# Sunefei/PathNet

Measured on AMD Instinct MI355X. Metric: paths aggregated/sec (PAGG fwd+bwd, one training step incl. on-GPU MERW sampling + Adam), higher is better.
Workload: dtype f32; 1 GPU; Cora-shaped synthetic (configs[1]): N=2708 F=1433 C=7 hid=128 path_num=40 path_len=4, 1299 masked nodes = 51960 paths/step, PathNet_homo, dropout 0.7, Adam; nodes=2708, parallelism=node-shard x1

## Files before the change

include/pathnet_hip.h:

```cpp
#ifndef PATHNET_HIP_H_
#define PATHNET_HIP_H_

#include <stdint.h>

#ifdef __cplusplus
extern "C" {
#endif

#define PN_ABI_VERSION 12

#define PN_OK 0
#define PN_ERR_ARG (-1)
#define PN_ERR_IO (-2)
#define PN_ERR_FORMAT (-3)
#define PN_ERR_HIP (-4)
#define PN_ERR_EMPTY_TABLE (-5)
#define PN_ERR_NOMEM (-6)
#define PN_ERR_CAPACITY (-7)

int pn_abi_version(void);
const char *pn_last_error(void);

typedef struct pn_device_info {
    char name[128];
    char arch[64];
    int32_t compute_units;
    int32_t lds_bytes_per_block;
    int64_t hbm_bytes;
    int32_t clock_khz;
} pn_device_info;
int pn_device_query(pn_device_info *out);

typedef struct pn_context pn_context;
int pn_context_create(pn_context **out);
int pn_context_destroy(pn_context *ctx);
int pn_context_set_knob(pn_context *ctx, const char *name, int32_t value);
int pn_context_get_knob(const pn_context *ctx, const char *name, int32_t *value);

typedef struct pn_step_state {
    int64_t epoch;
    uint64_t seed;
    int64_t adam_step;
    int64_t reserved;
} pn_step_state;
int pn_step_state_advance(pn_step_state *dev_state, void *stream);

int pn_clock_probe(double *mhz, void *stream);


int pn_edges_read_text(const char *path, int32_t *n, int64_t *m, int32_t *u, int32_t *v, double *p, int64_t cap);

int pn_pairs_read_text(const char *path, int32_t *n, int64_t *m, int32_t *u, int32_t *v, int64_t cap);

int pn_uniform_build(int32_t n, int64_t m, const int32_t *u, const int32_t *v, int64_t *off, int32_t *packed,
                     int32_t *src, int32_t *nbr, int64_t cap, int64_t *total);

int pn_alias_build(int32_t n, int64_t m, const int32_t *u, const int32_t *v, const double *p, int64_t *off,
                   int32_t *A, int32_t *B, double *S, uint32_t *thr, int64_t cap, int64_t *total);

int pn_hops_dense(int32_t n, int64_t m, const int32_t *u, const int32_t *v, int32_t seq_len, uint8_t *dis);

int pn_csr_build(int32_t n, int64_t m, const int32_t *u, const int32_t *v, int32_t reverse, int64_t *off,
                 int32_t *adj, int64_t cap, int64_t *count);

int pn_glibc_draws(uint32_t seed, uint64_t first, int64_t count, int32_t *out);


#define PN_DRAW_GLIBC_REPLAY 0
#define PN_DRAW_PHILOX 1

typedef struct pn_sampler_tables {
    int32_t n;
    int64_t total;
    const int64_t *off;
    const int32_t *triples;
    const uint8_t *dis;
    const int64_t *adj_off;
    const int32_t *adj;
    const int64_t *radj_off;
    const int32_t *radj;
    int32_t draws_per_step;
    const uint32_t *node_ref;
} pn_sampler_tables;

int pn_node_ref_pack(int32_t n, const int64_t *off, uint32_t *ref);

int pn_alias_pack(int64_t total, const int32_t *A, const int32_t *B, const uint32_t *thr, int32_t *dst);

int pn_tables_workspace_bytes(int32_t n, int64_t m, int64_t *bytes);

int pn_alias_build_device(int32_t n, int64_t m, const int32_t *u, const int32_t *v, const double *p, int64_t *off,
                          int32_t *triples, uint32_t *node_ref, double *S, int64_t cap, int64_t *total, void *workspace,
                          int64_t workspace_bytes, void *stream);

int pn_csr_build_device(int32_t n, int64_t m, const int32_t *u, const int32_t *v, int32_t reverse, int64_t *off,
                        int32_t *adj, int64_t cap, int64_t *count, void *workspace, int64_t workspace_bytes, void *stream);

int pn_hops_dense_device(int32_t n, const int64_t *off, const int32_t *adj, int32_t seq_len, uint8_t *dis, void *stream);

int pn_sample_workspace_bytes(int32_t W, int32_t L, int32_t draw_source, int64_t epoch_count, int32_t node_count,
                              int64_t *bytes);

int pn_sample_paths(pn_context *ctx, const pn_sampler_tables *tables, int32_t W, int32_t L, int32_t draw_source, uint64_t seed,
                    int64_t epoch_begin, int64_t epoch_count, int32_t node_begin, int32_t node_count, int32_t *ids,
                    uint8_t *codes, void *workspace, int64_t workspace_bytes, int32_t *status_flag,
                    const pn_step_state *step_state ,
                    const int32_t *node_list , void *stream);

typedef struct pn_path_report {
    int64_t out_of_range;
    int64_t non_edges;
    int64_t far;
    int64_t first_bad;
} pn_path_report;

int pn_path_codes_workspace_bytes(const pn_sampler_tables *tables, int32_t W, int32_t L, int32_t rows, int64_t *bytes);
int pn_path_codes(pn_context *ctx, const pn_sampler_tables *tables, int32_t W, int32_t L, int32_t rows,
                  const int32_t *ids , const int32_t *sources ,
                  uint8_t *codes , pn_path_report *report ,
                  void *workspace, int64_t workspace_bytes, void *stream);

#define PN_BIAS_MAX_TRIALS 64
int pn_bias_thresholds(double p, double q, uint64_t thr[3]);
int pn_sample_paths_biased_workspace_bytes(const pn_sampler_tables *tables, int32_t W, int32_t L, int64_t epoch_count,
                                           int32_t node_count, int64_t *bytes);
int pn_sample_paths_biased(pn_context *ctx, const pn_sampler_tables *tables, int32_t W, int32_t L, uint64_t seed,
                           int64_t epoch_begin, int64_t epoch_count, int32_t node_begin, int32_t node_count, double p,
                           double q, int32_t *ids, uint8_t *codes, int64_t *exhausted , void *workspace,
                           int64_t workspace_bytes, int32_t *status_flag, const pn_step_state *step_state,
                           const int32_t *node_list, void *stream);

int pn_census_lists_workspace_bytes(int32_t n, int64_t m, int64_t *bytes);
int pn_census_lists(pn_context *ctx, int32_t n, int64_t m, const int32_t *u, const int32_t *v, int64_t *off, int32_t *adj,
                    void *workspace, int64_t workspace_bytes, void *stream);

int pn_pattern_census_workspace_bytes(int32_t n, int32_t num_symbols, int32_t walk_len, int64_t *bytes);
int pn_pattern_census(pn_context *ctx, int32_t n, const int64_t *off, const int32_t *adj,
                      const uint8_t *symbols , int32_t num_symbols, int32_t walk_len,
                      int64_t *counts , int64_t *labels , void *workspace,
                      int64_t workspace_bytes, void *stream);

typedef struct pn_walk_stats_out {
    int64_t *step_code;
    int64_t *label_pairs;
    int64_t *unlabeled;
    int64_t *stay;
    int64_t *back;
    int64_t *distinct_hist;
    int32_t *unique_paths;
    int32_t *cover;
    int64_t *visits;
    int64_t *counters;
} pn_walk_stats_out;

int pn_walk_stats_workspace_bytes(int32_t n, int32_t W, int32_t L, int64_t rows, int32_t C, int64_t *bytes);
int pn_walk_stats(pn_context *ctx, int32_t n, int32_t W, int32_t L, int64_t rows,
                  const int32_t *ids , const uint8_t *codes ,
                  const int32_t *sources , const int32_t *labels , int32_t C,
                  int32_t accumulate, const pn_walk_stats_out *out, void *workspace, int64_t workspace_bytes,
                  void *stream);

typedef struct pn_path_prob_out {
    int64_t *num;
    int64_t *mass;
    uint8_t *cls;
    int64_t *counters;
} pn_path_prob_out;

int pn_path_prob_workspace_bytes(const pn_sampler_tables *tables, int32_t W, int32_t L, int64_t rows, int32_t second_order,
                                 int64_t *bytes);
int pn_path_prob(pn_context *ctx, const pn_sampler_tables *tables, int32_t W, int32_t L, int64_t rows,
                 const int32_t *ids , int32_t second_order, const pn_path_prob_out *out,
                 void *workspace, int64_t workspace_bytes, void *stream);

int pn_paths_write_text(const char *path, const int32_t *ids, const uint8_t *codes, int64_t npaths, int32_t L,
                        int32_t append);
int pn_paths_read_text(const char *path, int32_t L, int32_t *ids, uint8_t *codes, int64_t cap, int64_t *npaths);

int pn_paths_write_bin(const char *path, const int32_t *ids, const uint8_t *codes, int64_t npaths, int32_t L);
int pn_paths_read_bin(const char *path, int32_t *L_out, int32_t *ids, uint8_t *codes, int64_t cap, int64_t *npaths);

#define PN_VARIANT_HETERO 0
#define PN_VARIANT_HOMO 1
#define PN_VARIANT_PAGG 2

typedef struct pn_pagg_shape {
    int32_t variant;
    int32_t N, F, H, C;
    int32_t S, W, L;
    int32_t S_total, group_begin;
    int32_t batch_groups;
    int32_t cell;
    int32_t deterministic;
    int32_t compact;
    int32_t seq_math;
} pn_pagg_shape;
#define PN_SEQ_MATH_DEFAULT 0
#define PN_SEQ_MATH_BF16X3 1
#define PN_SEQ_MATH_F16X2 2
#define PN_COMPACT_AUTO 0
#define PN_COMPACT_ON 1
#define PN_COMPACT_OFF 2
#define PN_CELL_DEFAULT 0
#define PN_CELL_LSTM 1
#define PN_CELL_RNN 2
#define PN_CELL_GRU 3
#define PN_CELL_MEAN 4
#define PN_CELL_SUM 5

typedef struct pn_pagg_args {
    pn_pagg_shape shape;
    const float *X;
    const int32_t *ids;
    const uint8_t *codes;
    const int32_t *sel;
    const float *fc0_w, *fc0_b;
    const float *bank_w, *bank_b;
    const float *w_ih, *w_hh;
    const float *b_ih, *b_hh;
    const float *att_w, *att_b;
    const float *fc2_w, *fc2_b;
    float p_seq, p_cls;
    uint64_t seed;
    const float *mask_seq;
    const float *mask_cls;
    float *out;
    void *workspace;
    int64_t workspace_bytes;
    const float *g_out;
    float *g_X;
    float *g_fc0_w, *g_fc0_b, *g_bank_w, *g_bank_b, *g_w_ih, *g_w_hh, *g_b_ih, *g_b_hh, *g_att_w, *g_att_b,
        *g_fc2_w, *g_fc2_b;
    const float *Xh_in;
    float *g_Xh;
    void *Xh_ready;
    void *g_Xh_ready;
    int32_t no_save;
    int32_t reuse_tables;
    int32_t index_rows_local;
    const pn_step_state *step_state;
    float *out_embed;
    float *out_path_weight;
    float *out_path_state;
    const float *g_embed;
} pn_pagg_args;

int pn_pagg_workspace_bytes(const pn_pagg_shape *shape, int64_t *bytes);
int pn_pagg_shape_info(const pn_pagg_shape *shape, int64_t out[4]);
typedef struct pn_seq_range {
    uint32_t x_bits;
    int32_t x_esum;
    uint32_t x_cnt;
    uint32_t w_ih_bits, w_hh_bits, dg_bits;
} pn_seq_range;
int pn_pagg_range_offset(const pn_pagg_shape *shape, int64_t *offset);
int pn_pagg_paths_stream(pn_context *ctx, const pn_pagg_shape *shape, void *stream, void **out);
int pn_pagg_forward(pn_context *ctx, const pn_pagg_args *args, void *stream);
int pn_pagg_backward(pn_context *ctx, const pn_pagg_args *args, void *stream);
int pn_pagg_train_step(pn_context *ctx, const pn_pagg_args *args, const int64_t *target, float grad_scale, float *loss,
                       void *stream);

int pn_pagg_gather(pn_context *ctx, const pn_pagg_shape *shape, const float *table , const int32_t *ids,
                   const uint8_t *codes, float *rows , void *stream);

int pn_gemm_f32(const float *A, int64_t sAm, int64_t sAk, const float *B, int64_t sBn, int64_t sBk, float *C,
                int64_t ldc, const float *bias, int32_t M, int32_t N, int32_t K, int32_t relu, void *stream);

#define PN_LINEAR_SPLIT_MAX 8
int pn_linear_forward(pn_context *ctx, const float *X, const float *W, const float *b, int32_t rows, int32_t in_f, int32_t out_f,
                      int32_t relu, float *Y, void *workspace, int64_t workspace_bytes, void *stream);

#define PN_LINEAR_BWD_SPLIT_MAX 32
int pn_linear_backward(pn_context *ctx, const float *dY, const float *gate, const float *X, const float *W, int32_t rows, int32_t in_f,
                       int32_t out_f, float *g_W, float *g_b, float *g_X, void *workspace, int64_t workspace_bytes, void *stream);

int pn_merw_workspace_bytes(int32_t n, int64_t *bytes);
int pn_merw_probabilities(int32_t n, int64_t nnz, const int64_t *row_off, const int32_t *col, const double *val,
                          double *p, double *psi, double *lambda, int32_t max_iter, double tol, int32_t *iters,
                          void *workspace, int64_t workspace_bytes, void *stream);

int pn_cross_entropy(const float *logits, const int64_t *target, int32_t rows, int32_t classes, float *loss,
                     float *g_logits, void *stream);

#define PN_ADAM_MAX_TENSORS 32
typedef struct pn_adam_tensor {
    float *param;
    const float *grad;
    float *exp_avg;
    float *exp_avg_sq;
    int64_t count;
} pn_adam_tensor;
int pn_adam_step(const pn_adam_tensor *tensors, int32_t n_tensors, float lr, float beta1, float beta2, float eps,
                 float weight_decay, int64_t step, const pn_step_state *step_state ,
                 void *stream);
int pn_adam_step_advance(const pn_adam_tensor *tensors, int32_t n_tensors, float lr, float beta1, float beta2, float eps,
                         float weight_decay, pn_step_state *step_state , void *stream);

int pn_pagg_debug_offsets(const pn_pagg_shape *shape, int64_t out[4]);

int pn_profile_configure(pn_context *ctx, int32_t mode, int32_t stage);
int pn_profile_stage_count(void);
const char *pn_profile_stage_name(int32_t stage);
int pn_profile_read(pn_context *ctx, double *ms_sum, int64_t *count);

#ifdef __cplusplus
}
#endif
#endif
```

pathnet_amd/_lib.py:

```python
import ctypes
import os

HERE = os.path.dirname(os.path.abspath(__file__))
LIB_PATH = os.environ.get("PN_LIB_PATH", os.path.join(HERE, "csrc", "libpathnet_hip.so"))

PN_OK = 0
PN_ERR_ARG, PN_ERR_IO, PN_ERR_FORMAT, PN_ERR_HIP, PN_ERR_EMPTY_TABLE, PN_ERR_NOMEM, PN_ERR_CAPACITY = (
    -1, -2, -3, -4, -5, -6, -7)
DRAW_GLIBC_REPLAY, DRAW_PHILOX = 0, 1
ABI_VERSION = 12
VARIANT_HETERO, VARIANT_HOMO, VARIANT_PAGG = 0, 1, 2
CELL_DEFAULT, CELL_LSTM, CELL_RNN, CELL_GRU, CELL_MEAN, CELL_SUM = 0, 1, 2, 3, 4, 5
SEQ_MATH_DEFAULT, SEQ_MATH_BF16X3, SEQ_MATH_F16X2 = 0, 1, 2
COMPACT_AUTO, COMPACT_ON, COMPACT_OFF = 0, 1, 2
LINEAR_SPLIT_MAX = 8
LINEAR_BWD_SPLIT_MAX = 32

c_i32p = ctypes.POINTER(ctypes.c_int32)
c_i64p = ctypes.POINTER(ctypes.c_int64)
c_u32p = ctypes.POINTER(ctypes.c_uint32)
c_u8p = ctypes.POINTER(ctypes.c_uint8)
c_f64p = ctypes.POINTER(ctypes.c_double)
vp = ctypes.c_void_p


class PnError(RuntimeError):
    def __init__(self, code, msg):
        super().__init__("libpathnet_hip error %d: %s" % (code, msg))
        self.code = code


class DeviceInfo(ctypes.Structure):
    _fields_ = [("name", ctypes.c_char * 128), ("arch", ctypes.c_char * 64), ("compute_units", ctypes.c_int32),
                ("lds_bytes_per_block", ctypes.c_int32), ("hbm_bytes", ctypes.c_int64), ("clock_khz", ctypes.c_int32)]


class SamplerTables(ctypes.Structure):
    _fields_ = [("n", ctypes.c_int32), ("total", ctypes.c_int64), ("off", vp), ("triples", vp), ("dis", vp),
                ("adj_off", vp), ("adj", vp), ("radj_off", vp), ("radj", vp), ("draws_per_step", ctypes.c_int32),
                ("node_ref", vp)]


class PaggShape(ctypes.Structure):
    _fields_ = [("variant", ctypes.c_int32), ("N", ctypes.c_int32), ("F", ctypes.c_int32), ("H", ctypes.c_int32),
                ("C", ctypes.c_int32), ("S", ctypes.c_int32), ("W", ctypes.c_int32), ("L", ctypes.c_int32),
                ("S_total", ctypes.c_int32), ("group_begin", ctypes.c_int32), ("batch_groups", ctypes.c_int32),
                ("cell", ctypes.c_int32), ("deterministic", ctypes.c_int32), ("compact", ctypes.c_int32),
                ("seq_math", ctypes.c_int32)]


class PaggArgs(ctypes.Structure):
    _fields_ = ([("shape", PaggShape), ("X", vp), ("ids", vp), ("codes", vp), ("sel", vp)] +
                [(k, vp) for k in ("fc0_w", "fc0_b", "bank_w", "bank_b", "w_ih", "w_hh", "b_ih", "b_hh", "att_w",
                                   "att_b", "fc2_w", "fc2_b")] +
                [("p_seq", ctypes.c_float), ("p_cls", ctypes.c_float), ("seed", ctypes.c_uint64), ("mask_seq", vp),
                 ("mask_cls", vp), ("out", vp), ("workspace", vp), ("workspace_bytes", ctypes.c_int64),
                 ("g_out", vp), ("g_X", vp)] +
                [("g_" + k, vp) for k in ("fc0_w", "fc0_b", "bank_w", "bank_b", "w_ih", "w_hh", "b_ih", "b_hh", "att_w",
                                          "att_b", "fc2_w", "fc2_b")] +
                [("Xh_in", vp), ("g_Xh", vp), ("Xh_ready", vp), ("g_Xh_ready", vp), ("no_save", ctypes.c_int32),
                 ("reuse_tables", ctypes.c_int32),
                 ("index_rows_local", ctypes.c_int32), ("step_state", vp),
                 ("out_embed", vp), ("out_path_weight", vp), ("out_path_state", vp), ("g_embed", vp)])


class WalkStatsOut(ctypes.Structure):
    FIELDS = ("step_code", "label_pairs", "unlabeled", "stay", "back", "distinct_hist", "unique_paths", "cover", "visits",
              "counters")
    _fields_ = [(k, vp) for k in FIELDS]


class PathProbOut(ctypes.Structure):
    FIELDS = ("num", "mass", "cls", "counters")
    _fields_ = [(k, vp) for k in FIELDS]


class AdamTensor(ctypes.Structure):
    _fields_ = [("param", ctypes.c_void_p), ("grad", ctypes.c_void_p), ("exp_avg", ctypes.c_void_p),
                ("exp_avg_sq", ctypes.c_void_p), ("count", ctypes.c_int64)]


SIGNATURES = {
    "pn_abi_version": (ctypes.c_int, []),
    "pn_last_error": (ctypes.c_char_p, []),
    "pn_device_query": (ctypes.c_int, [ctypes.POINTER(DeviceInfo)]),
    "pn_context_create": (ctypes.c_int, [ctypes.POINTER(vp)]),
    "pn_context_destroy": (ctypes.c_int, [vp]),
    "pn_context_set_knob": (ctypes.c_int, [vp, ctypes.c_char_p, ctypes.c_int32]),
    "pn_context_get_knob": (ctypes.c_int, [vp, ctypes.c_char_p, c_i32p]),
    "pn_clock_probe": (ctypes.c_int, [c_f64p, vp]),
    "pn_step_state_advance": (ctypes.c_int, [vp, vp]),
    "pn_edges_read_text": (ctypes.c_int, [ctypes.c_char_p, c_i32p, c_i64p, c_i32p, c_i32p, c_f64p, ctypes.c_int64]),
    "pn_pairs_read_text": (ctypes.c_int, [ctypes.c_char_p, c_i32p, c_i64p, c_i32p, c_i32p, ctypes.c_int64]),
    "pn_uniform_build": (ctypes.c_int, [ctypes.c_int32, ctypes.c_int64, c_i32p, c_i32p, c_i64p, c_i32p, c_i32p, c_i32p,
                                        ctypes.c_int64, c_i64p]),
    "pn_alias_build": (ctypes.c_int, [ctypes.c_int32, ctypes.c_int64, c_i32p, c_i32p, c_f64p, c_i64p, c_i32p, c_i32p,
                                      c_f64p, c_u32p, ctypes.c_int64, c_i64p]),
    "pn_alias_pack": (ctypes.c_int, [ctypes.c_int64, c_i32p, c_i32p, c_u32p, c_i32p]),
    "pn_node_ref_pack": (ctypes.c_int, [ctypes.c_int32, c_i64p, c_u32p]),
    "pn_hops_dense": (ctypes.c_int, [ctypes.c_int32, ctypes.c_int64, c_i32p, c_i32p, ctypes.c_int32, c_u8p]),
    "pn_csr_build": (ctypes.c_int, [ctypes.c_int32, ctypes.c_int64, c_i32p, c_i32p, ctypes.c_int32, c_i64p, c_i32p,
                                    ctypes.c_int64, c_i64p]),
    "pn_glibc_draws": (ctypes.c_int, [ctypes.c_uint32, ctypes.c_uint64, ctypes.c_int64, c_i32p]),
    "pn_tables_workspace_bytes": (ctypes.c_int, [ctypes.c_int32, ctypes.c_int64, c_i64p]),
    "pn_alias_build_device": (ctypes.c_int, [ctypes.c_int32, ctypes.c_int64, vp, vp, vp, vp, vp, vp, vp, ctypes.c_int64,
                                             c_i64p, vp, ctypes.c_int64, vp]),
    "pn_csr_build_device": (ctypes.c_int, [ctypes.c_int32, ctypes.c_int64, vp, vp, ctypes.c_int32, vp, vp,
                                           ctypes.c_int64, c_i64p, vp, ctypes.c_int64, vp]),
    "pn_hops_dense_device": (ctypes.c_int, [ctypes.c_int32, vp, vp, ctypes.c_int32, vp, vp]),
    "pn_sample_workspace_bytes": (ctypes.c_int, [ctypes.c_int32, ctypes.c_int32, ctypes.c_int32, ctypes.c_int64,
                                                 ctypes.c_int32, c_i64p]),
    "pn_sample_paths": (ctypes.c_int, [vp, ctypes.POINTER(SamplerTables), ctypes.c_int32, ctypes.c_int32, ctypes.c_int32,
                                       ctypes.c_uint64, ctypes.c_int64, ctypes.c_int64, ctypes.c_int32, ctypes.c_int32,
                                       vp, vp, vp, ctypes.c_int64, vp, vp, vp, vp]),
    "pn_path_codes_workspace_bytes": (ctypes.c_int, [ctypes.POINTER(SamplerTables), ctypes.c_int32, ctypes.c_int32,
                                                     ctypes.c_int32, c_i64p]),
    "pn_path_codes": (ctypes.c_int, [vp, ctypes.POINTER(SamplerTables), ctypes.c_int32, ctypes.c_int32, ctypes.c_int32, vp, vp,
                                     vp, vp, vp, ctypes.c_int64, vp]),
    "pn_bias_thresholds": (ctypes.c_int, [ctypes.c_double, ctypes.c_double, ctypes.POINTER(ctypes.c_uint64)]),
    "pn_sample_paths_biased_workspace_bytes": (ctypes.c_int, [ctypes.POINTER(SamplerTables), ctypes.c_int32, ctypes.c_int32,
                                                              ctypes.c_int64, ctypes.c_int32, c_i64p]),
    "pn_sample_paths_biased": (ctypes.c_int, [vp, ctypes.POINTER(SamplerTables), ctypes.c_int32, ctypes.c_int32,
                                              ctypes.c_uint64, ctypes.c_int64, ctypes.c_int64, ctypes.c_int32,
                                              ctypes.c_int32, ctypes.c_double, ctypes.c_double, vp, vp, vp, vp,
                                              ctypes.c_int64, vp, vp, vp, vp]),
    "pn_census_lists_workspace_bytes": (ctypes.c_int, [ctypes.c_int32, ctypes.c_int64, c_i64p]),
    "pn_census_lists": (ctypes.c_int, [vp, ctypes.c_int32, ctypes.c_int64, vp, vp, vp, vp, vp, ctypes.c_int64, vp]),
    "pn_pattern_census_workspace_bytes": (ctypes.c_int, [ctypes.c_int32, ctypes.c_int32, ctypes.c_int32, c_i64p]),
    "pn_pattern_census": (ctypes.c_int, [vp, ctypes.c_int32, vp, vp, vp, ctypes.c_int32, ctypes.c_int32, vp, vp, vp,
                                         ctypes.c_int64, vp]),
    "pn_walk_stats_workspace_bytes": (ctypes.c_int, [ctypes.c_int32, ctypes.c_int32, ctypes.c_int32, ctypes.c_int64,
                                                     ctypes.c_int32, c_i64p]),
    "pn_walk_stats": (ctypes.c_int, [vp, ctypes.c_int32, ctypes.c_int32, ctypes.c_int32, ctypes.c_int64, vp, vp, vp, vp,
                                     ctypes.c_int32, ctypes.c_int32, ctypes.POINTER(WalkStatsOut), vp, ctypes.c_int64, vp]),
    "pn_path_prob_workspace_bytes": (ctypes.c_int, [ctypes.POINTER(SamplerTables), ctypes.c_int32, ctypes.c_int32,
                                                    ctypes.c_int64, ctypes.c_int32, c_i64p]),
    "pn_path_prob": (ctypes.c_int, [vp, ctypes.POINTER(SamplerTables), ctypes.c_int32, ctypes.c_int32, ctypes.c_int64, vp,
                                    ctypes.c_int32, ctypes.POINTER(PathProbOut), vp, ctypes.c_int64, vp]),
    "pn_paths_write_text": (ctypes.c_int, [ctypes.c_char_p, c_i32p, c_u8p, ctypes.c_int64, ctypes.c_int32,
                                           ctypes.c_int32]),
    "pn_paths_read_text": (ctypes.c_int, [ctypes.c_char_p, ctypes.c_int32, c_i32p, c_u8p, ctypes.c_int64, c_i64p]),
    "pn_paths_write_bin": (ctypes.c_int, [ctypes.c_char_p, c_i32p, c_u8p, ctypes.c_int64, ctypes.c_int32]),
    "pn_paths_read_bin": (ctypes.c_int, [ctypes.c_char_p, c_i32p, c_i32p, c_u8p, ctypes.c_int64, c_i64p]),
    "pn_pagg_workspace_bytes": (ctypes.c_int, [ctypes.POINTER(PaggShape), c_i64p]),
    "pn_pagg_shape_info": (ctypes.c_int, [ctypes.POINTER(PaggShape), c_i64p]),
    "pn_pagg_forward": (ctypes.c_int, [vp, ctypes.POINTER(PaggArgs), vp]),
    "pn_pagg_backward": (ctypes.c_int, [vp, ctypes.POINTER(PaggArgs), vp]),
    "pn_pagg_gather": (ctypes.c_int, [vp, ctypes.POINTER(PaggShape), vp, vp, vp, vp, vp]),
    "pn_gemm_f32": (ctypes.c_int, [vp, ctypes.c_int64, ctypes.c_int64, vp, ctypes.c_int64, ctypes.c_int64, vp,
                                   ctypes.c_int64, vp, ctypes.c_int32, ctypes.c_int32, ctypes.c_int32, ctypes.c_int32,
                                   vp]),
    "pn_profile_configure": (ctypes.c_int, [vp, ctypes.c_int32, ctypes.c_int32]),
    "pn_profile_stage_count": (ctypes.c_int, []),
    "pn_profile_stage_name": (ctypes.c_char_p, [ctypes.c_int32]),
    "pn_profile_read": (ctypes.c_int, [vp, c_f64p, c_i64p]),
    "pn_linear_forward": (ctypes.c_int, [vp, vp, vp, vp, ctypes.c_int32, ctypes.c_int32, ctypes.c_int32, ctypes.c_int32, vp,
                                         vp, ctypes.c_int64, vp]),
    "pn_linear_backward": (ctypes.c_int, [vp, vp, vp, vp, vp, ctypes.c_int32, ctypes.c_int32, ctypes.c_int32, vp, vp,
                                          vp, vp, ctypes.c_int64, vp]),
    "pn_pagg_train_step": (ctypes.c_int, [vp, ctypes.POINTER(PaggArgs), vp, ctypes.c_float, vp, vp]),
    "pn_pagg_debug_offsets": (ctypes.c_int, [ctypes.POINTER(PaggShape), c_i64p]),
    "pn_pagg_range_offset": (ctypes.c_int, [ctypes.POINTER(PaggShape), c_i64p]),
    "pn_pagg_paths_stream": (ctypes.c_int, [vp, ctypes.POINTER(PaggShape), vp, ctypes.POINTER(ctypes.c_void_p)]),
    "pn_merw_workspace_bytes": (ctypes.c_int, [ctypes.c_int32, c_i64p]),
    "pn_merw_probabilities": (ctypes.c_int, [ctypes.c_int32, ctypes.c_int64, vp, vp, vp, vp, vp, c_f64p, ctypes.c_int32,
                                             ctypes.c_double, c_i32p, vp, ctypes.c_int64, vp]),
    "pn_cross_entropy": (ctypes.c_int, [vp, vp, ctypes.c_int32, ctypes.c_int32, vp, vp, vp]),
    "pn_adam_step": (ctypes.c_int, [ctypes.POINTER(AdamTensor), ctypes.c_int32, ctypes.c_float, ctypes.c_float,
                                    ctypes.c_float, ctypes.c_float, ctypes.c_float, ctypes.c_int64, vp, vp]),
    "pn_adam_step_advance": (ctypes.c_int, [ctypes.POINTER(AdamTensor), ctypes.c_int32, ctypes.c_float, ctypes.c_float,
                                            ctypes.c_float, ctypes.c_float, ctypes.c_float, vp, vp]),
}

_lib = None


def load():
    global _lib
    if _lib is None:
        if not os.path.exists(LIB_PATH):
            raise ImportError("pathnet_amd: %s is missing -- build the HIP extension first "
                              "(python -c 'import __graft_entry__ as g; g.build()'); there is no CPU fallback"
                              % LIB_PATH)
        lib = ctypes.CDLL(LIB_PATH)
        for name, (res, args) in SIGNATURES.items():
            fn = getattr(lib, name)
            fn.restype = res
            fn.argtypes = args
        if lib.pn_abi_version() != ABI_VERSION:
            raise ImportError("libpathnet_hip.so ABI version mismatch")
        _lib = lib
    return _lib


_contexts = {}


def context(device):
    import torch
    dev = torch.device(device)
    idx = dev.index if dev.index is not None else torch.cuda.current_device()
    ctx = _contexts.get(idx)
    if ctx is None:
        lib = load()
        h = vp()
        with torch.cuda.device(idx):
            check(lib.pn_context_create(ctypes.byref(h)))
        ctx = _contexts[idx] = vp(h.value)
        if len(_contexts) == 1:
            import atexit
            atexit.register(_destroy_contexts)
    return ctx


def set_knob(name, value, device="cuda"):
    old = get_knob(name, device)
    check(load().pn_context_set_knob(context(device), name.encode(), int(value)))
    return old


def get_knob(name, device="cuda"):
    v = ctypes.c_int32()
    check(load().pn_context_get_knob(context(device), name.encode(), ctypes.byref(v)))
    return v.value


def _destroy_contexts():
    if _lib is None:
        return
    for h in _contexts.values():
        try:
            _lib.pn_context_destroy(h)
        except Exception:
            pass
    _contexts.clear()


def stream_ptr(device):
    import torch
    return vp(torch.cuda.current_stream(device).cuda_stream)


def check(rc):
    if rc != PN_OK:
        raise PnError(rc, load().pn_last_error().decode(errors="replace"))


def ptr(t):
    if t is None:
        return None
    if hasattr(t, "data_ptr"):
        return ctypes.c_void_p(t.data_ptr())
    return ctypes.c_void_p(t.ctypes.data)


def np_ptr(a, ctype):
    return a.ctypes.data_as(ctypes.POINTER(ctype))
```

pathnet_amd/csrc/pn_context.hip:

```cpp
#include <hip/hip_runtime.h>

#include <cstdlib>
#include <cstring>
#include <map>
#include <new>
#include <tuple>
#include <vector>

#include "pn_internal.h"

struct pn_context {
    int device = 0;
    hipStream_t side = nullptr;
    hipEvent_t fork = nullptr, join = nullptr;
    int prof_mode = 0, prof_stage = -1;
    struct Rec {
        int stage;
        hipEvent_t a, b;
    };
    std::vector<Rec> recs;
    std::vector<hipEvent_t> free_events;
    std::map<const void *, int> lds_attr;
    std::map<std::tuple<const void *, size_t, int>, int> slots;
    int cus = 0;
    pn::Knobs knobs;
};

namespace {

__global__ void warm_kernel() {}

__global__ void step_state_advance_kernel(pn_step_state *s) {
    if (threadIdx.x != 0 || blockIdx.x != 0) return;
    s->epoch += 1;
    s->adam_step += 1;
    uint64_t z = (s->seed += 0x9E3779B97F4A7C15ull);
    z = (z ^ (z >> 30)) * 0xBF58476D1CE4E5B9ull;
    z = (z ^ (z >> 27)) * 0x94D049BB133111EBull;
    s->seed = z ^ (z >> 31);
}

__global__ void clock_probe_kernel(long long spin_ticks, long long *out) {
    const long long w0 = wall_clock64();
    const long long c0 = (long long)__builtin_readcyclecounter();
    long long w1 = w0;
    while (w1 - w0 < spin_ticks) {
        __builtin_amdgcn_s_sleep(8);
        w1 = wall_clock64();
    }
    const long long c1 = (long long)__builtin_readcyclecounter();
    out[0] = c1 - c0;
    out[1] = w1 - w0;
}

hipEvent_t take_event(pn_context *ctx) {
    if (!ctx->free_events.empty()) {
        hipEvent_t e = ctx->free_events.back();
        ctx->free_events.pop_back();
        return e;
    }
    hipEvent_t e = nullptr;
    (void)hipEventCreateWithFlags(&e, ctx->knobs.event_dev ? hipEventDisableSystemFence : hipEventDefault);
    return e;
}

}

namespace {

struct KnobName {
    const char *name;
    int pn::Knobs::*field;
};
const KnobName kKnobs[] = {{"PN_NODE_GEMM3", &pn::Knobs::node_gemm3}, {"PN_EVAL_ZW", &pn::Knobs::eval_zw},
                           {"PN_POOL_STEP", &pn::Knobs::pool_step}, {"PN_EVENT_DEVICE_SCOPE", &pn::Knobs::event_dev},
                           {"PN_NODE_RGRAD", &pn::Knobs::node_rgrad}, {"PN_SAMPLER_STAGE", &pn::Knobs::sampler_stage},
                           {"PN_SEQ4", &pn::Knobs::seq4}, {"PN_SEQH_TAIL", &pn::Knobs::seqh_tail}};

}

namespace pn {

const Knobs &knobs_of(const pn_context *ctx) {
    static const Knobs defaults;
    return ctx ? ctx->knobs : defaults;
}

bool profiling_every_stage(const pn_context *ctx) { return ctx && ctx->prof_mode == 1; }

int resident_slots(pn_context *ctx, const void *kernel, int threads, size_t lds_bytes, int *slots, int *cus) {
    if (ctx) {
        auto it = ctx->slots.find(std::make_tuple(kernel, lds_bytes, threads));
        if (it != ctx->slots.end() && ctx->cus > 0) {
            *slots = it->second * ctx->cus;
            *cus = ctx->cus;
            return PN_OK;
        }
    }
    int dev = 0, n_cu = 0, per_cu = 0;
    PN_CHECK_HIP(hipGetDevice(&dev));
    PN_CHECK_HIP(hipDeviceGetAttribute(&n_cu, hipDeviceAttributeMultiprocessorCount, dev));
    PN_CHECK_HIP(hipOccupancyMaxActiveBlocksPerMultiprocessor(&per_cu, kernel, threads, lds_bytes));
    if (ctx) {
        ctx->slots[std::make_tuple(kernel, lds_bytes, threads)] = per_cu;
        ctx->cus = n_cu;
    }
    *slots = per_cu * n_cu;
    *cus = n_cu;
    return PN_OK;
}

int context_check_device(const pn_context *ctx) {
    if (!ctx) return PN_OK;
    int dev = -1;
    PN_CHECK_HIP(hipGetDevice(&dev));
    if (dev != ctx->device)
        PN_FAIL(PN_ERR_ARG, "pn_context belongs to device %d, the current device is %d", ctx->device, dev);
    return PN_OK;
}

int ensure_dynamic_lds(pn_context *ctx, const void *kernel, int bytes) {
    if (ctx) {
        auto it = ctx->lds_attr.find(kernel);
        if (it != ctx->lds_attr.end() && it->second >= bytes) return PN_OK;
    }
    PN_CHECK_HIP(hipFuncSetAttribute(kernel, hipFuncAttributeMaxDynamicSharedMemorySize, bytes));
    if (ctx) ctx->lds_attr[kernel] = bytes;
    return PN_OK;
}

void *context_side_stream(pn_context *ctx) { return ctx ? (void *)ctx->side : nullptr; }
void *context_fork(pn_context *ctx, void *stream) {
    if (!ctx || !ctx->side) return nullptr;
    if (hipEventRecord(ctx->fork, (hipStream_t)stream) != hipSuccess) return nullptr;
    if (hipStreamWaitEvent(ctx->side, ctx->fork, 0) != hipSuccess) return nullptr;
    return ctx->side;
}
int context_record_join(pn_context *ctx) {
    PN_CHECK_HIP(hipEventRecord(ctx->join, ctx->side));
    return PN_OK;
}
int context_join(pn_context *ctx, void *stream) {
    PN_CHECK_HIP(hipStreamWaitEvent((hipStream_t)stream, ctx->join, 0));
    return PN_OK;
}
int context_wait_side(pn_context *ctx, void *stream) {
    if (!ctx || !ctx->side || (hipStream_t)stream == ctx->side) return PN_OK;
    hipStreamCaptureStatus cs = hipStreamCaptureStatusNone, ss = hipStreamCaptureStatusNone;
    PN_CHECK_HIP(hipStreamIsCapturing((hipStream_t)stream, &cs));
    PN_CHECK_HIP(hipStreamIsCapturing(ctx->side, &ss));
    if ((cs == hipStreamCaptureStatusActive) != (ss == hipStreamCaptureStatusActive)) return PN_OK;
    if (int rc = context_record_join(ctx)) return rc;
    return context_join(ctx, stream);
}

StageTimer::StageTimer(pn_context *ctx_, int stage, void *stream_) : ctx(ctx_), slot(-1), stream(stream_) {
    if (!ctx || ctx->prof_mode == 0 || (ctx->prof_mode == 2 && stage != ctx->prof_stage)) return;
    pn_context::Rec r{stage, take_event(ctx), take_event(ctx)};
    (void)hipEventRecord(r.a, (hipStream_t)stream);
    slot = (int)ctx->recs.size();
    ctx->recs.push_back(r);
}
StageTimer::~StageTimer() {
    if (slot >= 0) (void)hipEventRecord(ctx->recs[(size_t)slot].b, (hipStream_t)stream);
}

}

extern "C" {

int pn_context_create(pn_context **out) try {
    if (!out) PN_FAIL(PN_ERR_ARG, "pn_context_create: null");
    *out = nullptr;
    pn_context *c = new (std::nothrow) pn_context();
    if (!c) PN_FAIL(PN_ERR_NOMEM, "pn_context_create: out of memory");
    auto fail = [&](hipError_t e, const char *what) {
        pn::set_error("%s failed: %s", what, hipGetErrorString(e));
        (void)pn_context_destroy(c);
        return PN_ERR_HIP;
    };
    for (const KnobName &k : kKnobs)
        if (const char *v = std::getenv(k.name)) c->knobs.*(k.field) = std::atoi(v);
    hipError_t e = hipGetDevice(&c->device);
    if (e != hipSuccess) return fail(e, "hipGetDevice");
    if ((e = hipStreamCreateWithFlags(&c->side, hipStreamNonBlocking)) != hipSuccess) return fail(e, "hipStreamCreate");
    const unsigned ev_flags = hipEventDisableTiming | (c->knobs.event_dev ? hipEventDisableSystemFence : 0u);
    if ((e = hipEventCreateWithFlags(&c->fork, ev_flags)) != hipSuccess) return fail(e, "hipEventCreate");
    if ((e = hipEventCreateWithFlags(&c->join, ev_flags)) != hipSuccess) return fail(e, "hipEventCreate");
    hipLaunchKernelGGL(warm_kernel, dim3(1), dim3(64), 0, c->side);
    if ((e = hipGetLastError()) != hipSuccess) return fail(e, "first launch on the context's stream");
    *out = c;
    return PN_OK;
} catch (...) {
    PN_FAIL(PN_ERR_NOMEM, "pn_context_create: exception");
}

int pn_context_destroy(pn_context *c) {
    if (!c) return PN_OK;
    int rc = PN_OK;
    if (c->side) {
        if (hipStreamSynchronize(c->side) != hipSuccess) rc = PN_ERR_HIP;
        (void)hipStreamDestroy(c->side);
    }
    if (c->fork) (void)hipEventDestroy(c->fork);
    if (c->join) (void)hipEventDestroy(c->join);
    for (auto &r : c->recs) {
        (void)hipEventDestroy(r.a);
        (void)hipEventDestroy(r.b);
    }
    for (hipEvent_t e : c->free_events) (void)hipEventDestroy(e);
    delete c;
    if (rc != PN_OK) pn::set_error("pn_context_destroy: the context's stream reported an error");
    return rc;
}

int pn_context_set_knob(pn_context *ctx, const char *name, int32_t value) {
    if (!ctx || !name) PN_FAIL(PN_ERR_ARG, "pn_context_set_knob: null");
    for (const KnobName &k : kKnobs)
        if (std::strcmp(k.name, name) == 0) {
            const bool events_change = k.field == &pn::Knobs::event_dev && (ctx->knobs.event_dev != 0) != (value != 0);
            ctx->knobs.*(k.field) = value;
            if (events_change) {
                PN_CHECK_HIP(hipDeviceSynchronize());
                const unsigned ev_flags = hipEventDisableTiming | (value ? hipEventDisableSystemFence : 0u);
                hipEvent_t fork = nullptr, join = nullptr;
                PN_CHECK_HIP(hipEventCreateWithFlags(&fork, ev_flags));
                PN_CHECK_HIP(hipEventCreateWithFlags(&join, ev_flags));
                (void)hipEventDestroy(ctx->fork);
                (void)hipEventDestroy(ctx->join);
                ctx->fork = fork;
                ctx->join = join;
                for (hipEvent_t e : ctx->free_events) (void)hipEventDestroy(e);
                ctx->free_events.clear();
            }
            return PN_OK;
        }
    PN_FAIL(PN_ERR_ARG, "pn_context_set_knob: no knob named %s", name);
}
int pn_context_get_knob(const pn_context *ctx, const char *name, int32_t *value) {
    if (!name || !value) PN_FAIL(PN_ERR_ARG, "pn_context_get_knob: null");
    for (const KnobName &k : kKnobs)
        if (std::strcmp(k.name, name) == 0) {
            *value = pn::knobs_of(ctx).*(k.field);
            return PN_OK;
        }
    PN_FAIL(PN_ERR_ARG, "pn_context_get_knob: no knob named %s", name);
}

int pn_profile_configure(pn_context *ctx, int32_t mode, int32_t stage) {
    if (!ctx) PN_FAIL(PN_ERR_ARG, "pn_profile_configure: null context");
    if (mode < 0 || mode > 2) PN_FAIL(PN_ERR_ARG, "profile mode %d", mode);
    ctx->prof_mode = mode;
    ctx->prof_stage = stage;
    return PN_OK;
}
int pn_profile_stage_count(void) { return pn::ST_COUNT; }
const char *pn_profile_stage_name(int32_t stage) {
    static const char *const names[pn::ST_COUNT] = {"sampler_glibc_fill", "sampler_walk", "gather",    "fc0",      "bank",
                                                    "plan_pack",          "seq_fwd",      "pool_fwd",  "fc2_grad", "pool_bwd",
                                                    "seq_bwd",            "wgrad",        "bias_grad", "bank_bwd", "fc0_bwd", "zero_fill"};
    return (stage >= 0 && stage < pn::ST_COUNT) ? names[stage] : "?";
}
int pn_profile_read(pn_context *ctx, double *ms_sum, int64_t *count) try {
    if (!ctx || !ms_sum || !count) PN_FAIL(PN_ERR_ARG, "pn_profile_read: null");
    for (auto &r : ctx->recs) {
        PN_CHECK_HIP(hipEventSynchronize(r.b));
        float ms = 0.0f;
        PN_CHECK_HIP(hipEventElapsedTime(&ms, r.a, r.b));
        ms_sum[r.stage] += ms;
        count[r.stage] += 1;
        ctx->free_events.push_back(r.a);
        ctx->free_events.push_back(r.b);
    }
    ctx->recs.clear();
    return PN_OK;
} catch (...) {
    PN_FAIL(PN_ERR_NOMEM, "pn_profile_read: exception");
}

int pn_device_query(pn_device_info *out) {
    if (!out) PN_FAIL(PN_ERR_ARG, "pn_device_query: null");
    int dev = 0;
    PN_CHECK_HIP(hipGetDevice(&dev));
    hipDeviceProp_t prop;
    PN_CHECK_HIP(hipGetDeviceProperties(&prop, dev));
    std::snprintf(out->name, sizeof out->name, "%s", prop.name);
    std::snprintf(out->arch, sizeof out->arch, "%s", prop.gcnArchName);
    out->compute_units = prop.multiProcessorCount;
    out->lds_bytes_per_block = (int32_t)prop.sharedMemPerBlock;
    out->hbm_bytes = (int64_t)prop.totalGlobalMem;
    out->clock_khz = prop.clockRate;
    return PN_OK;
}

int pn_step_state_advance(pn_step_state *dev_state, void *stream_) {
    if (!dev_state) PN_FAIL(PN_ERR_ARG, "pn_step_state_advance: null");
    hipLaunchKernelGGL(step_state_advance_kernel, dim3(1), dim3(64), 0, (hipStream_t)stream_, dev_state);
    PN_CHECK_HIP(hipGetLastError());
    return PN_OK;
}

int pn_clock_probe(double *mhz, void *stream_) {
    if (!mhz) PN_FAIL(PN_ERR_ARG, "pn_clock_probe: null");
    hipStream_t stream = (hipStream_t)stream_;
    long long *buf = nullptr;
    PN_CHECK_HIP(hipHostMalloc(reinterpret_cast<void **>(&buf), 2 * sizeof(long long), hipHostMallocDefault));
    buf[0] = buf[1] = 0;
    hipLaunchKernelGGL(clock_probe_kernel, dim3(1), dim3(64), 0, stream, 200000LL , buf);
    hipError_t e = hipGetLastError();
    if (e == hipSuccess) e = hipStreamSynchronize(stream);
    const long long cyc = buf[0], ticks = buf[1];
    (void)hipHostFree(buf);
    if (e != hipSuccess) PN_FAIL(PN_ERR_HIP, "clock probe failed: %s", hipGetErrorString(e));
    if (ticks <= 0) PN_FAIL(PN_ERR_HIP, "clock probe: the wall clock did not advance");
    *mhz = (double)cyc / (double)ticks * 100.0;
    return PN_OK;
}

}
```

pathnet_amd/csrc/pn_internal.h:

```cpp
#pragma once
#include <cstdarg>
#include <cstdint>
#include <cstdio>

#include "../../include/pathnet_hip.h"

namespace pn {

void set_error(const char *fmt, ...) __attribute__((format(printf, 1, 2)));

#define PN_FAIL(code, ...)          \
    do {                            \
        ::pn::set_error(__VA_ARGS__); \
        return (code);              \
    } while (0)

#define PN_CHECK_HIP(expr)                                                                      \
    do {                                                                                        \
        hipError_t e_ = (expr);                                                                 \
        if (e_ != hipSuccess) PN_FAIL(PN_ERR_HIP, "%s failed: %s", #expr, hipGetErrorString(e_)); \
    } while (0)

struct GlibcPoly {
    uint32_t c[31];
};
struct GlibcState {
    uint32_t s[31];
};
GlibcPoly glibc_poly_one();
GlibcPoly glibc_poly_mul(const GlibcPoly &a, const GlibcPoly &b);
GlibcPoly glibc_poly_xpow(uint64_t d);
GlibcState glibc_apply(const GlibcPoly &p, const GlibcState &st);
GlibcState glibc_seed_state(uint32_t seed);

#ifndef PN_SEQH_TAIL_DEFAULT
#define PN_SEQH_TAIL_DEFAULT 0
#endif
struct Knobs {
    int node_gemm3 = 7;
    int eval_zw = 1;
    int event_dev = 1;
    int pool_step = 1;
    int node_rgrad = 1;
    int sampler_stage = -1;
    int seq4 = 4;
    int seqh_tail = PN_SEQH_TAIL_DEFAULT;
};
const Knobs &knobs_of(const pn_context *ctx);

enum Stage {
    ST_SAMPLER_FILL = 0, ST_SAMPLER_WALK, ST_GATHER, ST_FC0, ST_BANK, ST_PLAN_PACK, ST_SEQ_FWD, ST_POOL_FWD,
    ST_FC2_GRAD, ST_POOL_BWD, ST_SEQ_BWD, ST_WGRAD, ST_BIAS_GRAD, ST_BANK_BWD, ST_FC0_BWD, ST_ZERO_FILL, ST_COUNT
};
bool profiling_every_stage(const pn_context *ctx);
int context_check_device(const pn_context *ctx);
void *context_fork(pn_context *ctx, void *stream);
void *context_side_stream(pn_context *ctx);
int context_record_join(pn_context *ctx);
int context_join(pn_context *ctx, void *stream);
int context_wait_side(pn_context *ctx, void *stream);
int ensure_dynamic_lds(pn_context *ctx, const void *kernel, int bytes);
int resident_slots(pn_context *ctx, const void *kernel, int threads, size_t lds_bytes, int *slots, int *cus);
struct StageTimer {
    StageTimer(pn_context *ctx, int stage, void *stream);
    ~StageTimer();
    pn_context *ctx;
    int slot;
    void *stream;
};

struct ZeroList {
    float *ptr[12];
    unsigned long long count[12];
    int n;
};
struct ZeroFill {
    pn_context *ctx;
    ZeroList zl{};
    int add(float *ptr, size_t count) {
        if (!ptr || !count) return PN_OK;
        if (zl.n >= (int)(sizeof zl.ptr / sizeof zl.ptr[0])) PN_FAIL(PN_ERR_ARG, "internal: zero list overflow");
        zl.ptr[zl.n] = ptr;
        zl.count[zl.n] = count;
        zl.n++;
        return PN_OK;
    }
    int flush(void *stream, bool timed = true);
};

int launch_cross_entropy(const float *logits, const int64_t *target, int rows, int classes, float scale, float *loss,
                         float *g_logits, void *stream, bool overwrite = false);

size_t sort_temp_reserve(int64_t n);
int sort_pairs_i32(void *tmp, size_t tmp_bytes, const int32_t *keys_in, int32_t *keys_out, const int32_t *vals_in,
                   int32_t *vals_out, int64_t n, int key_bits, void *stream);

}
```

pathnet_amd/csrc/pn_pagg.hip:

```cpp
#include <hip/hip_runtime.h>

#include <algorithm>
#include <cstdlib>
#include <cstring>
#include <type_traits>

#include "pn_gemm.h"
#include "pn_internal.h"
#include "pn_kernels.h"
#include "pn_seq.h"

using namespace pn;

namespace {

struct PlanDims {
    int S_total, W, L, N;
    int64_t P_total;
    int64_t row_base;
};
__device__ __forceinline__ void plan_entry(int variant, const int32_t *ids, const uint8_t *codes, const PlanDims &d,
                                           int64_t slot, int t, int64_t &q, int &node, int &code) {
    if (variant == PN_VARIANT_HETERO) {
        const int64_t g = slot / d.W, mem = slot - g * d.W;
        q = mem * d.S_total + g;
        const int64_t r = q * d.L + t;
        node = ids[(r % d.P_total) * d.L + (d.L - 1 - (int)(r / d.P_total))];
    } else {
        q = slot;
        node = ids[(q - d.row_base) * d.L + t];
    }
    code = codes[(q - d.row_base) * d.L + t];
}

__global__ void plan_kernel(int variant, const int32_t *__restrict__ ids, const uint8_t *__restrict__ codes, PlanDims d,
                            int64_t slot_begin, int64_t count, const int32_t *__restrict__ rank, int32_t *__restrict__ rowidx,
                            int32_t *__restrict__ egoidx, int32_t *__restrict__ slotof) {
    const int64_t i = (int64_t)blockIdx.x * blockDim.x + threadIdx.x;
    if (i >= count * d.L) return;
    const int64_t ls = i / d.L;
    const int t = (int)(i - ls * d.L);
    int64_t q;
    int node, code;
    plan_entry(variant, ids, codes, d, slot_begin + ls, t, q, node, code);
    node = min(max(node, 0), d.N - 1);
    code = min(code, d.L - 1);
    const int32_t row = rank ? rank[(int64_t)code * d.N + node] : node * d.L + code;
    rowidx[i] = row;
    if (t == 0) {
        slotof[ls] = (int32_t)q;
        egoidx[ls] = variant == PN_VARIANT_HETERO ? min(max(ids[(q - d.row_base) * d.L], 0), d.N - 1) : row;
    }
}

__global__ void mark_rows_kernel(int variant, const int32_t *__restrict__ ids, const uint8_t *__restrict__ codes, PlanDims d,
                                 int64_t slot_begin, int64_t count, uint8_t *__restrict__ flags) {
    const int64_t i = (int64_t)blockIdx.x * blockDim.x + threadIdx.x;
    if (i >= count * d.L) return;
    const int64_t ls = i / d.L;
    int64_t q;
    int node, code;
    plan_entry(variant, ids, codes, d, slot_begin + ls, (int)(i - ls * d.L), q, node, code);
    flags[(int64_t)min(code, d.L - 1) * d.N + min(max(node, 0), d.N - 1)] = 1;
}
constexpr int SCAN_BLOCK = 256 * 16;
__global__ __launch_bounds__(256) void scan_count_kernel(const uint8_t *__restrict__ flags, int64_t n, int32_t *__restrict__ bsum) {
    __shared__ int red[4];
    const int64_t base = (int64_t)blockIdx.x * SCAN_BLOCK + threadIdx.x * 16;
    int c = 0;
    if (base + 16 <= n) {
        const uint4 v = *reinterpret_cast<const uint4 *>(flags + base);
        c = __popc(v.x) + __popc(v.y) + __popc(v.z) + __popc(v.w);
    } else {
        for (int k = 0; k < 16; k++) c += base + k < n ? flags[base + k] : 0;
    }
    c = (int)wave_sum((float)c);
    if ((threadIdx.x & 63) == 0) red[threadIdx.x >> 6] = c;
    __syncthreads();
    if (threadIdx.x == 0) bsum[blockIdx.x] = red[0] + red[1] + red[2] + red[3];
}
__global__ __launch_bounds__(1024) void scan_blocks_kernel(int32_t *__restrict__ bsum, int nb, int32_t *__restrict__ total) {
    __shared__ int part[1024];
    const int per = (nb + 1023) / 1024, lo = threadIdx.x * per, hi = min(nb, lo + per);
    int s = 0;
    for (int i = lo; i < hi; i++) s += bsum[i];
    part[threadIdx.x] = s;
    __syncthreads();
    if (threadIdx.x == 0) {
        int run = 0;
        for (int i = 0; i < 1024; i++) {
            const int v = part[i];
            part[i] = run;
            run += v;
        }
        *total = run;
    }
    __syncthreads();
    int run = part[threadIdx.x];
    for (int i = lo; i < hi; i++) {
        const int v = bsum[i];
        bsum[i] = run;
        run += v;
    }
}
__global__ __launch_bounds__(256) void scan_rank_kernel(const uint8_t *__restrict__ flags, int64_t n, int N, int L,
                                                        const int32_t *__restrict__ bsum, int32_t *__restrict__ rank,
                                                        int32_t *__restrict__ list, int32_t *__restrict__ seg) {
    __shared__ int wsum[4];
    const int64_t base = (int64_t)blockIdx.x * SCAN_BLOCK + threadIdx.x * 16;
    uint8_t f[16];
    int c = 0;
#pragma unroll
    for (int k = 0; k < 16; k++) {
        f[k] = base + k < n ? flags[base + k] : 0;
        c += f[k];
    }
    const int lane = threadIdx.x & 63, wave = threadIdx.x >> 6;
    int inc = c;
#pragma unroll
    for (int o = 1; o < 64; o <<= 1) {
        const int up = __shfl_up(inc, o, 64);
        if (lane >= o) inc += up;
    }
    if (lane == 63) wsum[wave] = inc;
    __syncthreads();
    int run = bsum[blockIdx.x] + inc - c;
    for (int w = 0; w < wave; w++) run += wsum[w];
#pragma unroll
    for (int k = 0; k < 16; k++) {
        const int64_t i = base + k;
        if (i < n) {
            rank[i] = run;
            const int code = (int)(i / N), node = (int)(i - (int64_t)code * N);
            if (node == 0) seg[code] = run;
            if (f[k]) list[run] = node;
            run += f[k];
        }
    }
}

template <int VEC>
__global__ __launch_bounds__(256) void gather_kernel(int variant, const float *__restrict__ table,
                                                     const int32_t *__restrict__ ids,
                                                     const uint8_t *__restrict__ codes, PlanDims d, int64_t slot_begin,
                                                     int64_t count, int H, float *__restrict__ rows) {
    const int hv = H / VEC;
    const int64_t total = count * d.L * hv;
    for (int64_t i = (int64_t)blockIdx.x * blockDim.x + threadIdx.x; i < total; i += (int64_t)gridDim.x * blockDim.x) {
        const int64_t row = i / hv;
        const int c = (int)(i - row * hv);
        const int64_t ls = row / d.L;
        const int t = (int)(row - ls * d.L);
        int64_t q;
        int node, code;
        plan_entry(variant, ids, codes, d, slot_begin + ls, t, q, node, code);
        node = min(max(node, 0), d.N - 1);
        code = min(code, d.L - 1);
        const int64_t src = ((int64_t)node * d.L + code) * hv + c;
        if (VEC == 4)
            reinterpret_cast<float4 *>(rows)[i] = reinterpret_cast<const float4 *>(table)[src];
        else
            rows[i] = table[src];
    }
}

struct SeqReduceParams {
    const float *Z;
    const int32_t *rowidx;
    const int32_t *slotof;
    float *hn;
    const float *dhn;
    float *dZ;
    int P, L, H;
    int64_t Pmask;
    float scale;
    float p_drop;
    uint64_t seed;
    const pn_step_state *dyn;
    const float *mask;
};

template <bool BACKWARD>
__global__ __launch_bounds__(256) void seq_reduce_kernel(SeqReduceParams p) {
    const int hv = p.H / 4;
    const int64_t i = (int64_t)blockIdx.x * blockDim.x + threadIdx.x;
    if (i >= (int64_t)p.P * hv) return;
    const int q = (int)(i / hv), c4 = (int)(i - (int64_t)q * hv);
    const uint64_t seed = p.dyn ? p.dyn->seed : p.seed;
    const int64_t slot = p.slotof[q];
    float4 acc = make_float4(0.f, 0.f, 0.f, 0.f);
    float4 g = make_float4(0.f, 0.f, 0.f, 0.f);
    if (BACKWARD) {
        g = reinterpret_cast<const float4 *>(p.dhn)[i];
        g.x *= p.scale; g.y *= p.scale; g.z *= p.scale; g.w *= p.scale;
    }
    for (int t = 0; t < p.L; t++) {
        float4 m = make_float4(1.f, 1.f, 1.f, 1.f);
        if (p.mask)
            m = reinterpret_cast<const float4 *>(p.mask)[((int64_t)t * p.Pmask + slot) * hv + c4];
        else if (p.p_drop > 0.0f)
            m = dropout4(seed, ((uint64_t)t * p.Pmask + slot) * hv + c4, 1u, p.p_drop);
        const size_t row = (size_t)(uint32_t)p.rowidx[(int64_t)q * p.L + t];
        if (BACKWARD) {
            float *d = p.dZ + row * p.H + 4 * c4;
            atomicAdd(d + 0, g.x * m.x); atomicAdd(d + 1, g.y * m.y); atomicAdd(d + 2, g.z * m.z); atomicAdd(d + 3, g.w * m.w);
        } else {
            const float4 v = reinterpret_cast<const float4 *>(p.Z)[row * hv + c4];
            acc.x += v.x * m.x; acc.y += v.y * m.y; acc.z += v.z * m.z; acc.w += v.w * m.w;
        }
    }
    if (!BACKWARD) {
        acc.x *= p.scale; acc.y *= p.scale; acc.z *= p.scale; acc.w *= p.scale;
        reinterpret_cast<float4 *>(p.hn)[i] = acc;
    }
}


struct GenParams {
    const float *Z;
    const int32_t *rowidx;
    const int32_t *slotof;
    float *xh;
    float *pre;
    float *saved;
    float *state;
    float *hn;
    float *dh;
    const float *gx;
    float *dZ;
    const float *biasc;
    int P, L, H, G, cell, t;
    int64_t Pmask;
    float p_drop;
    uint64_t seed;
    const pn_step_state *dyn;
    const float *mask;
};

__device__ __forceinline__ float4 gen_mask(const GenParams &p, uint64_t seed, int t, int64_t slot, int c4) {
    const int hv = p.H / 4;
    if (p.mask) return reinterpret_cast<const float4 *>(p.mask)[((int64_t)t * p.Pmask + slot) * hv + c4];
    if (p.p_drop > 0.0f) return dropout4(seed, ((uint64_t)t * p.Pmask + slot) * hv + c4, 1u, p.p_drop);
    return make_float4(1.f, 1.f, 1.f, 1.f);
}

__global__ __launch_bounds__(256) void gen_x_kernel(GenParams p) {
    const int hv = p.H / 4;
    const int64_t i = (int64_t)blockIdx.x * blockDim.x + threadIdx.x;
    if (i >= (int64_t)p.P * hv) return;
    const int q = (int)(i / hv), c4 = (int)(i - (int64_t)q * hv);
    const uint64_t seed = p.dyn ? p.dyn->seed : p.seed;
    const float4 m = gen_mask(p, seed, p.t, p.slotof[q], c4);
    const size_t row = (size_t)(uint32_t)p.rowidx[(int64_t)q * p.L + p.t];
    float4 v = reinterpret_cast<const float4 *>(p.Z)[row * hv + c4];
    v.x *= m.x; v.y *= m.y; v.z *= m.z; v.w *= m.w;
    float4 *dst = reinterpret_cast<float4 *>(p.xh) + ((size_t)q * p.L + p.t) * (2 * hv) + c4;
    dst[0] = v;
    if (p.t == 0) dst[hv] = make_float4(0.f, 0.f, 0.f, 0.f);
}

__global__ __launch_bounds__(256) void gen_cell_fwd_kernel(GenParams p) {
    const int64_t i = (int64_t)blockIdx.x * blockDim.x + threadIdx.x;
    if (i >= (int64_t)p.P * p.H) return;
    const int H = p.H, q = (int)(i / H), j = (int)(i - (int64_t)q * H);
    const float *pre = p.pre + ((size_t)q * p.L + p.t) * ((size_t)p.G * H) + j;
    const int SV = p.G == 4 ? 5 : 1;
    float *sv = p.saved ? p.saved + (((size_t)q * p.L + p.t) * SV) * H + j : nullptr;
    float h;
    if (p.cell == 3) {
        const float rg = sigmoidf_(pre[0]), zg = sigmoidf_(pre[H]), nh = pre[3 * (size_t)H];
        const float ng = tanhf_(pre[2 * (size_t)H] + rg * nh);
        const float hp = p.t > 0 ? p.state[i] : 0.0f;
        h = (1.0f - zg) * ng + zg * hp;
        p.state[i] = h;
        if (sv) { sv[0] = rg; sv[H] = zg; sv[2 * (size_t)H] = ng; sv[3 * (size_t)H] = nh; sv[4 * (size_t)H] = hp; }
    } else if (p.G == 4) {
        const float ig = sigmoidf_(pre[0]), fg = sigmoidf_(pre[H]), gg = tanhf_(pre[2 * (size_t)H]), og = sigmoidf_(pre[3 * (size_t)H]);
        const float c = fg * (p.t > 0 ? p.state[i] : 0.0f) + ig * gg;
        p.state[i] = c;
        h = og * tanhf_(c);
        if (sv) { sv[0] = ig; sv[H] = fg; sv[2 * (size_t)H] = gg; sv[3 * (size_t)H] = og; sv[4 * (size_t)H] = c; }
    } else {
        h = tanhf_(pre[0]);
        if (sv) sv[0] = h;
    }
    if (p.t == p.L - 1)
        p.hn[i] = h;
    else
        p.xh[((size_t)q * p.L + p.t + 1) * (2 * (size_t)H) + H + j] = h;
}

__global__ __launch_bounds__(256) void gen_cell_bwd_kernel(GenParams p) {
    const int64_t i = (int64_t)blockIdx.x * blockDim.x + threadIdx.x;
    if (i >= (int64_t)p.P * p.H) return;
    const int H = p.H, q = (int)(i / H), j = (int)(i - (int64_t)q * H);
    const int SV = p.G == 4 ? 5 : 1;
    const float *sv = p.saved + (((size_t)q * p.L + p.t) * SV) * H + j;
    float *d = p.pre + ((size_t)q * p.L + p.t) * ((size_t)p.G * H) + j;
    const float dhv = p.dh[i];
    if (p.cell == 3) {
        const float rg = sv[0], zg = sv[H], ng = sv[2 * (size_t)H], nh = sv[3 * (size_t)H], hp = sv[4 * (size_t)H];
        const float dnp = dhv * (1.0f - zg) * (1.0f - ng * ng);
        d[0] = dnp * nh * rg * (1.0f - rg);
        d[H] = dhv * (hp - ng) * zg * (1.0f - zg);
        d[2 * (size_t)H] = dnp;
        d[3 * (size_t)H] = dnp * rg;
        p.state[i] = dhv * zg;
    } else if (p.G == 4) {
        const float ig = sv[0], fg = sv[H], gg = sv[2 * (size_t)H], og = sv[3 * (size_t)H], c = sv[4 * (size_t)H];
        const float cprev = p.t > 0 ? sv[-(ptrdiff_t)H] : 0.0f;
        const float tc = tanhf_(c);
        const float dct = (p.t < p.L - 1 ? p.state[i] : 0.0f) + dhv * og * (1.0f - tc * tc);
        d[0] = dct * gg * ig * (1.0f - ig);
// ... 677 lines not shown
        gab += ds;
    }
    PTRACE(9);
    if (!has_att) return;
    float *red = part4;
    if (one_row) {
#pragma unroll
        for (int i = 0; i < HI; i++) {
            const int j = lane + 64 * i;
            if (j < H) red[wave * H + j] = ego_acc[i];
        }
        __syncthreads();
        if (tid < H) atomicAdd(&b.dego[(int64_t)e0 * H + tid], (red[tid] + red[H + tid]) + (red[2 * H + tid] + red[3 * H + tid]));
        __syncthreads();
    }
#pragma unroll
    for (int i = 0; i < HI; i++) {
        const int j = lane + 64 * i;
        if (j < H) {
            red[wave * 2 * H + j] = gaw_h[i];
            red[wave * 2 * H + H + j] = gaw_e[i];
        }
    }
    __syncthreads();
    float *out = b.det_att + (int64_t)g * (2 * H + 4);
    for (int j = tid; j < 2 * H; j += 256) out[j] = red[j] + red[2 * H + j] + red[4 * H + j] + red[6 * H + j];
    if (lane == 0) out[2 * H + wave] = gab;
    PTRACE(10);
}
inline size_t pool_step2_lds_bytes(int MM, int H, int C) { return (size_t)(12 * MM + 8 * H + 2 * H + H + 2 * C + 8) * sizeof(float); }

__global__ __launch_bounds__(1024) void loss_sum_kernel(const float *__restrict__ lossg, int rows, float scale,
                                                        float *__restrict__ loss, int store) {
    __shared__ float part[16];
    float mine = 0.0f;
    for (int r = threadIdx.x; r < rows; r += 1024) mine += lossg[r];
#pragma unroll
    for (int o = 32; o > 0; o >>= 1) mine += __shfl_xor(mine, o, 64);
    if ((threadIdx.x & 63) == 0) part[threadIdx.x >> 6] = mine;
    __syncthreads();
    if (threadIdx.x == 0) {
        float t = 0.0f;
        for (int w = 0; w < 16; w++) t += part[w];
        if (store)
            *loss = t * scale;
        else
            atomicAdd(loss, t * scale);
    }
}

constexpr int DET_CHUNK = 32;
struct DetScatterParams {
    const int32_t *skey, *ssrc;
    int32_t kmask;
    int64_t K, chunk0;
    const float *rows;
    const float *scal, *vec;
    float *dst;
    float *cpart;
    int H;
};

struct DetScatterPair {
    DetScatterParams s[2];
};

template <int PASS>
__global__ __launch_bounds__(256) void det_scatter_kernel(DetScatterPair pp) {
    const DetScatterParams &p = pp.s[blockIdx.y];
    const int hv = p.H / 4, gpb = 256 / hv;
    const int grp = threadIdx.x / hv, ln = threadIdx.x - grp * hv;
    if (grp >= gpb) return;
    const int64_t c = (int64_t)blockIdx.x * gpb + grp, b = c * DET_CHUNK;
    if (b >= p.K) return;
    const int64_t e = min(p.K, b + (int64_t)DET_CHUNK);
    float4 *dst = reinterpret_cast<float4 *>(p.dst);
    float4 *cpart = reinterpret_cast<float4 *>(p.cpart) + p.chunk0 * 2 * hv;
    const int32_t km = p.kmask;
    auto add_to = [&](float4 *d, const float4 &a) {
        float4 v = *d;
        v.x += a.x; v.y += a.y; v.z += a.z; v.w += a.w;
        *d = v;
    };
    if (PASS == 1) {
        const float4 vec = p.rows ? make_float4(0.f, 0.f, 0.f, 0.f) : reinterpret_cast<const float4 *>(p.vec)[ln];
        int key = p.skey[b] & km;
        bool lead = b > 0 && (p.skey[b - 1] & km) == key;
        float4 acc = make_float4(0.f, 0.f, 0.f, 0.f);
        constexpr int DU = 4;
        for (int64_t i0 = b; i0 < e; i0 += DU) {
            int kk[DU];
            float4 vv[DU];
#pragma unroll
            for (int j = 0; j < DU; j++) {
                const int64_t i = min(i0 + j, e - 1);
                kk[j] = p.skey[i] & km;
                const int64_t src = p.ssrc[i];
                if (p.rows) {
                    vv[j] = reinterpret_cast<const float4 *>(p.rows)[src * hv + ln];
                } else {
                    const float sc = p.scal[src];
                    vv[j] = make_float4(sc * vec.x, sc * vec.y, sc * vec.z, sc * vec.w);
                }
            }
#pragma unroll
            for (int j = 0; j < DU; j++) {
                if (i0 + j >= e) break;
                const int k = kk[j];
                if (k != key) {
                    if (lead)
                        cpart[(c * 2 + 0) * hv + ln] = acc;
                    else
                        add_to(dst + (int64_t)key * hv + ln, acc);
                    lead = false;
                    key = k;
                    acc = make_float4(0.f, 0.f, 0.f, 0.f);
                }
                acc.x += vv[j].x; acc.y += vv[j].y; acc.z += vv[j].z; acc.w += vv[j].w;
            }
        }
        const bool cont = e < p.K && (p.skey[e] & km) == key;
        if (lead)
            cpart[(c * 2 + 0) * hv + ln] = acc;
        else if (cont)
            cpart[(c * 2 + 1) * hv + ln] = acc;
        else
            add_to(dst + (int64_t)key * hv + ln, acc);
    } else {
        const int key = p.skey[e - 1] & km;
        if (!(e < p.K && (p.skey[e] & km) == key)) return;
        if ((p.skey[b] & km) == key && b > 0 && (p.skey[b - 1] & km) == key) return;
        float4 acc = cpart[(c * 2 + 1) * hv + ln];
        for (int64_t c2 = c + 1;; c2++) {
            const int64_t e2 = min(p.K, (c2 + 1) * (int64_t)DET_CHUNK);
            const float4 v = cpart[(c2 * 2 + 0) * hv + ln];
            acc.x += v.x; acc.y += v.y; acc.z += v.z; acc.w += v.w;
            if ((p.skey[e2 - 1] & km) != key || !(e2 < p.K && (p.skey[e2] & km) == key)) break;
        }
        add_to(dst + (int64_t)key * hv + ln, acc);
    }
}

struct DetKeys3 {
    const int32_t *keys[3];
    int64_t n[3];
    int32_t hi[3];
    int shift;
};
__global__ __launch_bounds__(256) void det_keys3_kernel(DetKeys3 q, int32_t *__restrict__ keys, int32_t *__restrict__ pos) {
    int64_t i = (int64_t)blockIdx.x * blockDim.x + threadIdx.x;
    const int64_t at = i;
    int seg = 0;
    while (seg < 3 && i >= q.n[seg]) i -= q.n[seg], seg++;
    if (seg >= 3) return;
    keys[at] = min(max(q.keys[seg][i], 0), q.hi[seg]) | (seg << q.shift);
    pos[at] = (int32_t)i;
}

__global__ __launch_bounds__(256) void det_iota_kernel(int32_t *__restrict__ iota, int64_t n) {
    const int64_t i = (int64_t)blockIdx.x * blockDim.x + threadIdx.x;
    if (i < n) iota[i] = (int32_t)i;
}

__global__ __launch_bounds__(1024) void det_att_reduce_kernel(const float *__restrict__ part, int nblk, int H,
                                                              float *__restrict__ g_att_w, float *__restrict__ g_att_b) {
    __shared__ float red[16][64];
    const int lane = threadIdx.x & 63, rg = threadIdx.x >> 6, stride = 2 * H + 4;
    const int col = blockIdx.x * 64 + lane;
    float v = 0.0f;
    if (col < stride) {
        const float *src = part + col;
#pragma unroll 8
        for (int b = rg; b < nblk; b += 16) v += src[(int64_t)b * stride];
    }
    red[rg][lane] = v;
    __syncthreads();
    if (rg != 0) return;
    float t = 0.0f;
#pragma unroll
    for (int r = 0; r < 16; r++) t += red[r][lane];
    if (col < 2 * H) {
        g_att_w[col] += t;
    } else if (col < stride) {
        red[0][lane] = t;
        __builtin_amdgcn_fence(__ATOMIC_RELEASE, "wavefront");
        __builtin_amdgcn_wave_barrier();
        __builtin_amdgcn_fence(__ATOMIC_ACQUIRE, "wavefront");
        if (col == 2 * H) *g_att_b += (red[0][lane] + red[0][lane + 1]) + (red[0][lane + 2] + red[0][lane + 3]);
    }
}

__global__ __launch_bounds__(256) void pad_rows_kernel(const float *__restrict__ in, int64_t R, int F, int F4, float *__restrict__ out) {
    const int q4 = F4 / 4;
    const int64_t i = (int64_t)blockIdx.x * 256 + threadIdx.x;
    if (i >= R * q4) return;
    const int64_t r = i / q4;
    const int c = (int)(i - r * q4) * 4;
    const float *src = in + r * F + c;
    float4 v;
    v.x = src[0];
    v.y = c + 1 < F ? src[1] : 0.0f;
    v.z = c + 2 < F ? src[2] : 0.0f;
    v.w = c + 3 < F ? src[3] : 0.0f;
    reinterpret_cast<float4 *>(out)[i] = v;
}

__global__ __launch_bounds__(256) void zero_kernel(ZeroList z) {
    for (int b = 0; b < z.n; b++) {
        float *p = z.ptr[b];
        const unsigned long long cnt = z.count[b];
        const unsigned long long head = min(cnt, (unsigned long long)((16 - (reinterpret_cast<uintptr_t>(p) & 15)) & 15) / 4);
        const unsigned long long body4 = (cnt - head) / 4;
        float4 *p4 = reinterpret_cast<float4 *>(p + head);
        for (unsigned long long i = (unsigned long long)blockIdx.x * blockDim.x + threadIdx.x; i < body4;
             i += (unsigned long long)gridDim.x * blockDim.x)
            p4[i] = make_float4(0.f, 0.f, 0.f, 0.f);
        if (blockIdx.x == 0) {
            for (unsigned long long i = threadIdx.x; i < head; i += blockDim.x) p[i] = 0.0f;
            for (unsigned long long i = head + body4 * 4 + threadIdx.x; i < cnt; i += blockDim.x) p[i] = 0.0f;
        }
    }
}

enum { CELL_LSTM = 1, CELL_RNN = 2, CELL_GRU = 3, CELL_MEAN = 4, CELL_SUM = 5 };
struct Dims {
    int variant, N, F, H, C, S, W, L, G, SV;
    int cell, Gw;
    int gru;
    bool generic;
    int S_total, group_begin;
    int Sb;
    int nb;
    int64_t P_total;
    bool det;
    bool compact;
    int64_t ZR;
    int math;
};

int make_dims(const pn_pagg_shape &s, Dims &d) {
    if (s.variant < 0 || s.variant > 2) PN_FAIL(PN_ERR_ARG, "unknown variant %d", s.variant);
    if (s.H < 32 || s.H > 1024 || s.H % 32 != 0)
        PN_FAIL(PN_ERR_ARG, "hidden size %d not supported (multiples of 32 up to 1024; fused kernels up to 256)", s.H);
    if (s.N < 1 || s.F < 1 || s.C < 1 || s.S < 0 || s.W < 1 || s.L < 1 || s.L > 64)
        PN_FAIL(PN_ERR_ARG, "bad aggregator shape N=%d F=%d C=%d S=%d W=%d L=%d", s.N, s.F, s.C, s.S, s.W, s.L);
    if (64 * (int64_t)s.W + 48 * s.H > 64 * 1024)
        PN_FAIL(PN_ERR_ARG, "W=%d walks per node exceed the pooling kernels' LDS budget (W <= %d at H=%d)", s.W,
                (64 * 1024 - 48 * s.H) / 64, s.H);
    if (s.variant == PN_VARIANT_PAGG && s.L != 4)
        PN_FAIL(PN_ERR_ARG, "PAGG has exactly four distance layers nei0..nei3 (copy.py:310-313); L=%d", s.L);
    if (s.cell < 0 || s.cell > CELL_SUM) PN_FAIL(PN_ERR_ARG, "unknown cell %d", s.cell);
    const int S_total = s.S_total > 0 ? s.S_total : s.S;
    if (s.group_begin < 0 || (int64_t)s.group_begin + s.S > S_total || s.batch_groups < 0)
        PN_FAIL(PN_ERR_ARG, "bad slice: groups [%d, +%d) of a batch of %d, batch_groups=%d", s.group_begin, s.S,
                S_total, s.batch_groups);
    if ((int64_t)S_total * s.W > 2000000000LL || (int64_t)s.N * s.L > 2000000000LL)
        PN_FAIL(PN_ERR_ARG, "index space exceeds int32 (S_total*W = %lld paths, N*L = %lld rows)",
                (long long)S_total * s.W, (long long)s.N * s.L);
    d.variant = s.variant;
    d.N = s.N, d.F = s.F, d.H = s.H, d.C = s.C, d.S = s.S, d.W = s.W, d.L = s.L;
    d.cell = s.cell ? s.cell : (s.variant == PN_VARIANT_PAGG ? CELL_RNN : CELL_LSTM);
    d.G = d.cell == CELL_RNN ? 1 : (d.cell == CELL_LSTM || d.cell == CELL_GRU) ? 4 : 0;
    d.gru = d.cell == CELL_GRU ? 1 : 0;
    d.Gw = d.gru ? 3 : d.G;
    d.SV = d.G == 4 ? 5 : 1;
    d.generic = s.H > 256 && d.G > 0;
    d.S_total = S_total;
    d.group_begin = s.group_begin;
    d.Sb = (s.batch_groups > 0 && s.batch_groups < s.S) ? s.batch_groups : s.S;
    d.nb = d.Sb > 0 ? (s.S + d.Sb - 1) / d.Sb : 1;
    d.P_total = (int64_t)S_total * s.W;
    d.det = s.deterministic != 0;
    {
        const int64_t steps = (int64_t)(d.variant == PN_VARIANT_HETERO ? S_total : s.S) * s.W * s.L, rows = (int64_t)s.N * s.L;
        if (s.compact < 0 || s.compact > PN_COMPACT_OFF) PN_FAIL(PN_ERR_ARG, "unknown compact mode %d", s.compact);
        d.compact = s.S > 0 && (s.compact == PN_COMPACT_AUTO ? 2 * steps < rows : s.compact == PN_COMPACT_ON);
        d.ZR = d.compact ? std::min(rows, steps) : rows;
    }
    if (s.seq_math < 0 || s.seq_math > PN_SEQ_MATH_F16X2) PN_FAIL(PN_ERR_ARG, "unknown seq_math %d", s.seq_math);
    d.math = (d.G > 0 && !d.generic) ? (s.seq_math == PN_SEQ_MATH_BF16X3 ? PN_SEQ_MATH_BF16X3 : PN_SEQ_MATH_F16X2) : 0;
    if ((int64_t)d.Sb * s.W * s.L > 2000000000LL)
        PN_FAIL(PN_ERR_ARG, "%lld path steps in one micro-batch exceed int32: set batch_groups", (long long)d.Sb * s.W * s.L);
    return PN_OK;
}

#ifndef PN_WGRAD_CUS_SHARED
#define PN_WGRAD_CUS_SHARED 224
#endif
constexpr int WGRAD_CUS_SHARED = PN_WGRAD_CUS_SHARED;
inline size_t xpad_floats(const Dims &d) {
    if (d.F % 4 == 0 || d.N < 2048 || d.det) return 0;
    const size_t f4 = (size_t)(d.F + 3) / 4 * 4, n = (size_t)d.N * f4;
    return n * 4 <= ((size_t)256 << 20) ? n : 0;
}

struct WsLayout {
    size_t Xh, Z, range, wmax;
    size_t Wp, biasc, WpT, wpart, gpart, dZ, dXh;
    size_t rowidx, egoidx, slotof, hn, saved, coef, rawsc, layer1, outb;
    size_t xh, keep, dG, dhn, dl1, gx, gout, bankT, xpad;
    size_t flags, rank, list, seg, bsum;
    size_t dx, keys, iota, skey, stmp, cpart, dsel, dds, datt, dgemm;
    size_t okey, osrc;
    size_t stmp_bytes;
    int wgrad_split, wgrad_tiles;
    size_t total;
};

inline size_t align256(size_t x) { return (x + 255) / 256 * 256; }

WsLayout ws_layout(const Dims &d) {
    WsLayout w{};
    const size_t N = d.N, H = d.H, L = d.L, G = d.G, SV = d.SV, Sb = d.Sb, Pb = (size_t)d.Sb * d.W;
    size_t at = 0;
    auto take = [&](size_t bytes) {
        size_t o = at;
        at = align256(at + bytes);
        return o;
    };
    w.Xh = take(N * H * 4);
    w.Z = take((size_t)d.ZR * H * 4);
    w.range = take(sizeof(SeqRange));
    w.wmax = take(64 * 4);
    w.Wp = take(G * H * 3 * H * 4);
    w.biasc = take(G * H * 4);
    w.WpT = take(G * H * 3 * H * 4);
    {
        const size_t rows = Pb * L, tiles = std::max<size_t>(1, ((G * H + WG_BM - 1) / WG_BM) * ((2 * H + WG_BN - 1) / WG_BN));
        const double wg_flops = 2.0 * (double)rows * (double)(G * H) * (double)(2 * H);
        size_t cus = wg_flops <= 1.2e11 ? WGRAD_CUS_SHARED : 256;
        size_t nz = (cus + tiles - 1) / tiles;
        const size_t max_nz = (rows + 4 * WG_KT - 1) / (4 * WG_KT);
        if (nz > max_nz) nz = max_nz;
        if (nz < 1) nz = 1;
        w.wgrad_split = (int)nz;
        w.wgrad_tiles = (int)tiles;
        w.wpart = take(nz * (G * H * 2 * H + G * H) * 4);
    }
    {
        const int nz = std::max(gemm_split_count(d.N, d.H, d.F), gemm_split_count(d.N, d.H, d.L * d.H));
        w.gpart = take(nz > 1 ? (size_t)nz * N * H * 4 : 0);
    }
    w.dZ = take((size_t)d.ZR * H * 4);
    w.dXh = take(N * H * 4);
    w.rowidx = take(Pb * L * 4);
    w.egoidx = take(Pb * 4);
    w.slotof = take(Pb * 4);
    w.hn = take(Pb * H * 4);
    w.saved = take(Pb * L * SV * H * 4);
    w.coef = take(Pb * 4);
    w.rawsc = take(Pb * 4);
    w.layer1 = take(Sb * 2 * H * 4);
    w.outb = take(Sb * (size_t)d.C * 4);
    w.xh = take(Pb * L * 2 * H * 4);
    w.keep = take(Pb * L * (H / 4));
    w.dG = take(Pb * L * G * H * 4);
    w.dhn = take(Pb * H * 4);
    w.dl1 = take(Sb * 2 * H * 4 + 1024);
    w.gx = take(d.generic ? Pb * 2 * H * 4 : 0);
    w.gout = take(Sb * (size_t)d.C * 4);
    w.datt = take(Sb * (2 * H + 4) * 4);
    w.bankT = take(L * H * H * 4);
    w.xpad = take(xpad_floats(d) * 4);
    w.flags = take(d.compact ? N * L + 16 : 0);
    w.rank = take(d.compact ? N * L * 4 : 0);
    w.list = take(d.compact ? (size_t)d.ZR * 4 : 0);
    w.seg = take(d.compact ? (L + 2) * 4 : 0);
    w.bsum = take(d.compact ? ((N * L + SCAN_BLOCK - 1) / SCAN_BLOCK + 1) * 4 : 0);
    if (d.det) {
        const size_t K = std::max(Pb * L, Sb), C = d.C, F = d.F;
        w.dx = take(Pb * L * H * 4);
        const size_t ord[3] = {Sb, Pb, Pb * L};
        const size_t Kt = ord[0] + ord[1] + ord[2];
        w.keys = take(Kt * 4);
        w.iota = take(K * 4);
        w.skey = take(Kt * 4);
        w.okey = take(Kt * 4);
        w.osrc = take(Kt * 4);
        w.stmp_bytes = sort_temp_reserve((int64_t)Kt);
        w.stmp = take(w.stmp_bytes);
        w.cpart = take((Kt / DET_CHUNK + 4) * 2 * H * 4);
        w.dsel = take(Sb * H * 4);
        w.dds = take(Pb * 4);
        w.dgemm = take(std::max({det_gemm_floats(C, 2 * H), det_gemm_floats(d.compact ? H : L * H, H), det_gemm_floats(H, F)}) * 4);
    }
    w.total = at;
    return w;
}

struct JoinGuard {
    pn_context *ctx;
    hipStream_t stream;
    bool pending = false;
    int mark() {
        if (int rc = context_record_join(ctx)) return rc;
        pending = true;
        return PN_OK;
    }
    int join() {
        if (!pending) return PN_OK;
        pending = false;
        return context_join(ctx, stream);
    }
    ~JoinGuard() { (void)join(); }
};

struct Call {
    pn_context *ctx;
    hipStream_t stream;
    const pn_pagg_args *a;
    Dims d;
    WsLayout w;
    char *ws;
    const float *Xh;
    float *Z;
    template <class T>
    T *at(size_t off) const { return reinterpret_cast<T *>(ws + off); }
    int groups(int b) const { return std::min(d.Sb, d.S - b * d.Sb); }
    int64_t group0(int b) const { return (int64_t)d.group_begin + (int64_t)b * d.Sb; }
    const int32_t *sel(int b) const { return a->sel + (a->index_rows_local ? (int64_t)b * d.Sb : group0(b)); }
};

int resolve_call(Call &c, pn_context *ctx, const pn_pagg_args *a, hipStream_t stream, const char *who) {
    if (!a) PN_FAIL(PN_ERR_ARG, "%s: null args", who);
    if (int rc = context_check_device(ctx)) return rc;
    if (int rc = make_dims(a->shape, c.d)) return rc;
    c.ctx = ctx;
    c.stream = stream;
    c.a = a;
    c.w = ws_layout(c.d);
    if (!a->workspace) PN_FAIL(PN_ERR_ARG, "%s: null workspace", who);
    if (a->workspace_bytes < (int64_t)c.w.total)
        PN_FAIL(PN_ERR_CAPACITY, "aggregator workspace holds %lld bytes, need %lld", (long long)a->workspace_bytes,
                (long long)c.w.total);
    c.ws = reinterpret_cast<char *>(a->workspace);
    c.Xh = a->Xh_in ? a->Xh_in : c.at<const float>(c.w.Xh);
    c.Z = c.at<float>(c.w.Z);
    if (a->index_rows_local && c.d.variant == PN_VARIANT_HETERO && (c.d.group_begin != 0 || c.d.S != c.d.S_total))
        PN_FAIL(PN_ERR_ARG, "%s: the hetero class reads paths of the whole batch (PathNet_run.py:196-197): "
                "index_rows_local needs the whole batch's ids / codes", who);
    return PN_OK;
}

inline PlanDims plan_dims(const Call &c) {
    const Dims &d = c.d;
    return PlanDims{d.S_total, d.W, d.L, d.N, d.P_total, c.a->index_rows_local ? (int64_t)d.group_begin * d.W : 0};
}

int run_plan(const Call &c, hipStream_t s, int b) {
    const Dims &d = c.d;
    const int64_t count = (int64_t)c.groups(b) * d.W, n = count * d.L;
    const PlanDims pd = plan_dims(c);
    hipLaunchKernelGGL(plan_kernel, dim3((unsigned)((n + 255) / 256)), dim3(256), 0, s, d.variant, c.a->ids, c.a->codes,
                       pd, c.group0(b) * d.W, count, d.compact ? c.at<const int32_t>(c.w.rank) : nullptr,
                       c.at<int32_t>(c.w.rowidx), c.at<int32_t>(c.w.egoidx), c.at<int32_t>(c.w.slotof));
    PN_CHECK_HIP(hipGetLastError());
    return PN_OK;
}

int run_compact_rows(const Call &c, hipStream_t s) {
    const Dims &d = c.d;
    const bool het = d.variant == PN_VARIANT_HETERO;
    const int64_t slot0 = het ? 0 : (int64_t)d.group_begin * d.W, count = (int64_t)(het ? d.S_total : d.S) * d.W, n = count * d.L;
    const int64_t rows = (int64_t)d.N * d.L;
    const PlanDims pd = plan_dims(c);
    uint8_t *flags = c.at<uint8_t>(c.w.flags);
    PN_CHECK_HIP(hipMemsetAsync(flags, 0, (size_t)rows, s));
    hipLaunchKernelGGL(mark_rows_kernel, dim3((unsigned)((n + 255) / 256)), dim3(256), 0, s, d.variant, c.a->ids, c.a->codes, pd,
                       slot0, count, flags);
    const int nb = (int)((rows + SCAN_BLOCK - 1) / SCAN_BLOCK);
    int32_t *seg = c.at<int32_t>(c.w.seg), *bsum = c.at<int32_t>(c.w.bsum);
    hipLaunchKernelGGL(scan_count_kernel, dim3(nb), dim3(256), 0, s, flags, rows, bsum);
    hipLaunchKernelGGL(scan_blocks_kernel, dim3(1), dim3(1024), 0, s, bsum, nb, seg + d.L);
    hipLaunchKernelGGL(scan_rank_kernel, dim3(nb), dim3(256), 0, s, flags, rows, d.N, d.L, bsum, c.at<int32_t>(c.w.rank),
                       c.at<int32_t>(c.w.list), seg);
    PN_CHECK_HIP(hipGetLastError());
    return PN_OK;
}

GenParams gen_params(const Call &c, int b) {
    const Dims &d = c.d;
    const pn_pagg_args *a = c.a;
    GenParams gp{};
    gp.Z = c.Z;
    gp.rowidx = c.at<int32_t>(c.w.rowidx);
    gp.slotof = c.at<int32_t>(c.w.slotof);
    gp.xh = c.at<float>(c.w.xh);
    gp.pre = c.at<float>(c.w.dG);
    gp.hn = c.at<float>(c.w.hn);
    gp.gx = c.at<float>(c.w.gx);
    gp.dZ = c.at<float>(c.w.dZ);
    gp.biasc = c.at<float>(c.w.biasc);
    gp.P = c.groups(b) * d.W;
    gp.L = d.L;
    gp.H = d.H;
    gp.G = d.G;
    gp.cell = d.cell;
    gp.Pmask = d.P_total;
    gp.p_drop = a->p_seq;
    gp.seed = a->seed;
    gp.dyn = a->step_state;
    gp.mask = a->mask_seq;
    return gp;
}

int run_seq_fwd_generic(const Call &c, int b, bool save) {
    const Dims &d = c.d;
    GenParams gp = gen_params(c, b);
    gp.saved = save ? c.at<float>(c.w.saved) : nullptr;
    gp.state = c.at<float>(c.w.dhn);
    const int H = d.H, GH = d.G * H, P = gp.P;
    const float *Wcat = c.at<const float>(c.w.Wp);
    const unsigned bx = (unsigned)(((int64_t)P * (H / 4) + 255) / 256), be = (unsigned)(((int64_t)P * H + 255) / 256);
    StageTimer tm(c.ctx, ST_SEQ_FWD, c.stream);
    for (int t = 0; t < d.L; t++) {
        gp.t = t;
        hipLaunchKernelGGL(gen_x_kernel, dim3(bx), dim3(256), 0, c.stream, gp);
        PN_CHECK_HIP(hipGetLastError());
        GemmParams g = gemm_linear_fwd(gp.xh + (size_t)t * 2 * H, (int64_t)d.L * 2 * H, Wcat, 2 * H, gp.pre + (size_t)t * GH,
                                       (int64_t)d.L * GH, P, t == 0 ? H : 2 * H, GH);
        g.bias = gp.biasc;
        if (int rc = launch_gemm3(c.stream, gemm3_of(g))) return rc;
        hipLaunchKernelGGL(gen_cell_fwd_kernel, dim3(be), dim3(256), 0, c.stream, gp);
        PN_CHECK_HIP(hipGetLastError());
    }
    return PN_OK;
}

int run_seq_bwd_generic(const Call &c, int b) {
    const Dims &d = c.d;
    GenParams gp = gen_params(c, b);
    gp.saved = c.at<float>(c.w.saved);
    if (d.det) gp.rowidx = c.at<int32_t>(c.w.iota), gp.dZ = c.at<float>(c.w.dx);
    gp.dh = c.at<float>(c.w.dhn);
    gp.state = c.at<float>(c.w.hn);
    const int H = d.H, GH = d.G * H, P = gp.P;
    const float *WcatT = c.at<const float>(c.w.WpT);
    float *gx = c.at<float>(c.w.gx);
    const unsigned bx = (unsigned)(((int64_t)P * (H / 4) + 255) / 256), be = (unsigned)(((int64_t)P * H + 255) / 256);
    {
        StageTimer tm(c.ctx, ST_SEQ_BWD, c.stream);
        for (int t = d.L - 1; t >= 0; t--) {
            gp.t = t;
            hipLaunchKernelGGL(gen_cell_bwd_kernel, dim3(be), dim3(256), 0, c.stream, gp);
            PN_CHECK_HIP(hipGetLastError());
            const GemmParams g = gemm_linear_fwd(gp.pre + (size_t)t * GH, (int64_t)d.L * GH, WcatT, GH, gx, 2 * H, P, GH,
                                                 t == 0 ? H : 2 * H);
            if (int rc = launch_gemm3(c.stream, gemm3_of(g))) return rc;
            hipLaunchKernelGGL(gen_scatter_kernel, dim3(bx), dim3(256), 0, c.stream, gp);
            PN_CHECK_HIP(hipGetLastError());
        }
    }
    return PN_OK;
}

inline bool bank_epilogue_range(const Call &c) {
    const Dims &d = c.d;
    const pn_pagg_args *a = c.a;
    return d.math == PN_SEQ_MATH_F16X2 && d.G > 0 && !d.generic && !d.compact && a->reuse_tables == 0 && !a->Xh_in &&
           !gemm3_pays(c.ctx, d.N, d.H, d.F, G3_FC0) && !gemm3_pays(c.ctx, d.N, d.L * d.H, d.H, G3_BANK);
}

int run_pack_fwd(const Call &c, hipStream_t s) {
    const Dims &d = c.d;
    if (d.G == 0) return PN_OK;
    if (d.generic) {
        const int64_t n = (int64_t)d.G * d.H * 2 * d.H;
        hipLaunchKernelGGL(gen_pack_kernel, dim3((unsigned)((n + 255) / 256)), dim3(256), 0, s, c.a->w_ih, c.a->w_hh,
                           c.a->b_ih, c.a->b_hh, d.H, d.G, d.gru, c.at<float>(c.w.Wp),
                           c.at<float>(c.w.WpT), c.at<float>(c.w.biasc));
        PN_CHECK_HIP(hipGetLastError());
        return PN_OK;
    }
    if (d.math == PN_SEQ_MATH_F16X2) {
        SeqRange *rg = c.at<SeqRange>(c.w.range);
        return launch_pack_fb(s, c.a->w_ih, c.a->w_hh, c.a->b_ih, c.a->b_hh, d.H, d.G, d.Gw, d.gru,
                              (d.compact || c.a->reuse_tables != 1) && !bank_epilogue_range(c), rg, c.at<void>(c.w.wmax),
                              c.at<void>(c.w.Wp), c.at<float>(c.w.biasc), c.a->no_save ? nullptr : c.at<void>(c.w.WpT));
    }
    return launch_pack_fwd3(s, c.a->w_ih, c.a->w_hh, c.a->b_ih, c.a->b_hh, d.H, d.G, d.gru, c.at<void>(c.w.Wp),
                            c.at<float>(c.w.biasc));
}

int run_seq_reduce(const Call &c, int b, bool backward) {
    const Dims &d = c.d;
    const pn_pagg_args *a = c.a;
    SeqReduceParams rp{};
    rp.Z = c.Z;
    rp.rowidx = c.at<int32_t>(c.w.rowidx);
    rp.slotof = c.at<int32_t>(c.w.slotof);
    rp.hn = c.at<float>(c.w.hn);
    rp.dhn = c.at<float>(c.w.dhn);
    rp.dZ = c.at<float>(c.w.dZ);
    rp.P = c.groups(b) * d.W;
    rp.L = d.L;
    rp.H = d.H;
    rp.Pmask = d.P_total;
    rp.scale = d.cell == CELL_MEAN ? 1.0f / (float)d.L : 1.0f;
    rp.p_drop = a->p_seq;
    rp.seed = a->seed;
    rp.dyn = a->step_state;
    rp.mask = a->mask_seq;
    if (backward && d.det) rp.rowidx = c.at<int32_t>(c.w.iota), rp.dZ = c.at<float>(c.w.dx);
    const int64_t n = (int64_t)rp.P * (d.H / 4);
    StageTimer tm(c.ctx, backward ? ST_SEQ_BWD : ST_SEQ_FWD, c.stream);
    if (backward)
        hipLaunchKernelGGL(seq_reduce_kernel<true>, dim3((unsigned)((n + 255) / 256)), dim3(256), 0, c.stream, rp);
    else
        hipLaunchKernelGGL(seq_reduce_kernel<false>, dim3((unsigned)((n + 255) / 256)), dim3(256), 0, c.stream, rp);
    PN_CHECK_HIP(hipGetLastError());
    return PN_OK;
}

inline bool use_zw(const Call &c) {
    const Dims &d = c.d;
    const pn_pagg_args *a = c.a;
    if (d.math != PN_SEQ_MATH_F16X2 || !a->no_save || a->p_seq > 0.0f || a->mask_seq) return false;
    if (knobs_of(c.ctx).eval_zw == 0) return false;
    const size_t need = (size_t)d.ZR * d.G * d.H * 4, have = (size_t)d.Sb * d.W * d.L * d.SV * d.H * 4;
    return need <= have && need <= ((size_t)2 << 30);
}

inline float seq_xmul(const pn_pagg_args *a) {
    return a->mask_seq ? 16.0f : a->p_seq > 0.0f ? 1.0f / (1.0f - a->p_seq) : 1.0f;
}

int run_seq_fwd(const Call &c, int b, bool save) {
    const Dims &d = c.d;
    const pn_pagg_args *a = c.a;
    if (d.G == 0) return run_seq_reduce(c, b, false);
    if (d.generic) return run_seq_fwd_generic(c, b, save);
    SeqFwdParams sp{};
    sp.Z = c.Z;
    sp.rowidx = c.at<int32_t>(c.w.rowidx);
    sp.slotof = c.at<int32_t>(c.w.slotof);
    sp.Wp = c.at<float>(c.w.Wp);
    sp.biasc = c.at<float>(c.w.biasc);
    sp.hn = c.at<float>(c.w.hn);
    sp.saved = save ? c.at<float>(c.w.saved) : nullptr;
    sp.xh = save ? c.at<float>(c.w.xh) : nullptr;
    sp.keep = (!save || a->mask_seq || !(a->p_seq > 0.0f)) ? nullptr : c.at<uint8_t>(c.w.keep);
    sp.P = c.groups(b) * d.W;
    sp.L = d.L;
    sp.Pmask = d.P_total;
    sp.p_drop = a->p_seq;
    sp.seed = a->seed;
    sp.dyn = a->step_state;
    sp.mask = a->mask_seq;
    StageTimer tm(c.ctx, ST_SEQ_FWD, c.stream);
    if (!save && use_zw(c)) {
        sp.range = c.at<SeqRange>(c.w.range);
        sp.ZW = c.at<const float>(c.w.saved);
        return launch_seq_fwdzw(c.ctx, c.stream, d.H, d.Gw, sp);
    }
    if (d.math == PN_SEQ_MATH_F16X2) {
        sp.range = c.at<SeqRange>(c.w.range);
        sp.xmul = seq_xmul(a);
        return launch_seq_fwdh(c.ctx, c.stream, d.H, d.Gw, sp);
    }
    return launch_seq_fwd3(c.ctx, c.stream, d.H, d.Gw, sp);
}

PoolParams pool_fwd_params(const Call &c, int b, float *out) {
    const Dims &d = c.d;
    const pn_pagg_args *a = c.a;
    const int homo = d.variant == PN_VARIANT_HOMO;
    PoolParams pp{};
    pp.variant = d.variant;
    pp.S = c.groups(b);
    pp.W = d.W;
    pp.H = d.H;
    pp.C = d.C;
    pp.N = d.N;
    pp.goff = c.group0(b);
    pp.hn = c.at<float>(c.w.hn);
    pp.ego_tab = homo ? c.Z : c.Xh;
    pp.egoidx = c.at<int32_t>(c.w.egoidx);
    pp.Xh = c.Xh;
    pp.sel = c.sel(b);
    pp.att_w = a->att_w;
    pp.att_b = a->att_b;
    pp.fc2_w = a->fc2_w;
    pp.fc2_b = a->fc2_b;
    pp.p_drop = a->p_cls;
    pp.seed = a->seed;
    pp.dyn = a->step_state;
    pp.mask = a->mask_cls;
    pp.coef = c.at<float>(c.w.coef);
    pp.rawsc = c.at<float>(c.w.rawsc);
    pp.layer1 = c.at<float>(c.w.layer1);
    pp.out = out;
    return pp;
}
inline size_t pool_fwd_lds_bytes(const Dims &d) { return (size_t)(2 * d.W + 6 * d.H) * sizeof(float); }
int run_pool_fwd(const Call &c, int b, float *out, bool outputs = false) {
    PoolParams pp = pool_fwd_params(c, b, out);
    if (outputs) {
        const pn_pagg_args *a = c.a;
        const int64_t r0 = (int64_t)b * c.d.Sb;
        if (a->out_embed) pp.embed = a->out_embed + r0 * 2 * c.d.H;
        if (a->out_path_weight) pp.path_weight = a->out_path_weight + r0 * c.d.W;
        if (a->out_path_state) pp.path_state = a->out_path_state + r0 * c.d.W * c.d.H;
    }
    StageTimer tm(c.ctx, ST_POOL_FWD, c.stream);
    hipLaunchKernelGGL(pool_fwd_kernel, dim3(pp.S), dim3(256), pool_fwd_lds_bytes(c.d), c.stream, pp);
    PN_CHECK_HIP(hipGetLastError());
    return PN_OK;
}

int check_forward_args(const Call &c, const char *who) {
    const pn_pagg_args *a = c.a;
    const Dims &d = c.d;
    if (!a->ids || !a->codes || !a->sel || !a->bank_w || !a->bank_b || !a->fc2_w || !a->fc2_b || !a->out)
        PN_FAIL(PN_ERR_ARG, "%s: null tensor", who);
    if (d.G > 0 && (!a->w_ih || !a->w_hh || !a->b_ih || !a->b_hh)) PN_FAIL(PN_ERR_ARG, "%s: recurrent weights missing", who);
    if (!a->Xh_in && !a->reuse_tables && (!a->X || !a->fc0_w || !a->fc0_b)) PN_FAIL(PN_ERR_ARG, "%s: X / fc0 missing", who);
    if (d.variant != PN_VARIANT_PAGG && (!a->att_w || !a->att_b)) PN_FAIL(PN_ERR_ARG, "%s: attention weights missing", who);
    if (reinterpret_cast<uintptr_t>(a->out_path_state) % 16 != 0)
        PN_FAIL(PN_ERR_ARG, "%s: out_path_state must be 16-byte aligned", who);
    return PN_OK;
}

int run_tables(const Call &c, JoinGuard &joiner, ZeroFill *zero_fill = nullptr) {
    pn_context *ctx = c.ctx;
    hipStream_t stream = c.stream;
    const pn_pagg_args *a = c.a;
    const Dims &d = c.d;
    const int H = d.H, L = d.L;
    const int homo = d.variant == PN_VARIANT_HOMO;
    const bool epi_range = bank_epilogue_range(c);
    if (d.compact) {
        if (int rc = context_wait_side(ctx, stream)) return rc;
        StageTimer tm(ctx, ST_PLAN_PACK, stream);
        if (int rc = run_compact_rows(c, stream)) return rc;
    }
    hipStream_t pstream = stream;
    if (!profiling_every_stage(ctx))
        if (void *side = context_fork(ctx, stream)) pstream = (hipStream_t)side;
    {
        StageTimer tm(ctx, ST_PLAN_PACK, pstream);
        if (int rc = run_plan(c, pstream, 0)) return rc;
        if (int rc = run_pack_fwd(c, pstream)) return rc;
    }
    if (zero_fill)
        if (int rc = zero_fill->flush(pstream)) return rc;
    if (pstream != stream)
        if (int rc = joiner.mark()) return rc;
    if (!a->reuse_tables) {
        if (!a->Xh_in) {
            StageTimer tm(ctx, ST_FC0, stream);
            GemmParams g = gemm_linear_fwd(a->X, d.F, a->fc0_w, d.F, c.at<float>(c.w.Xh), H, d.N, d.F, H);
            g.bias = a->fc0_b;
            g.relu = homo;
            g.clear_word = epi_range ? &c.at<SeqRange>(c.w.range)->x : nullptr;
            if (gemm3_pays(c.ctx, d.N, H, d.F, G3_FC0)) {
                if (int rc = launch_gemm3(stream, gemm3_of(g))) return rc;
            } else if (int rc = launch_gemm_split(stream, g, c.at<float>(c.w.gpart)))
                return rc;
        }
    }
    if (a->Xh_in && a->Xh_ready) PN_CHECK_HIP(hipStreamWaitEvent(stream, (hipEvent_t)a->Xh_ready, 0));
    if (d.compact) {
        StageTimer tm(ctx, ST_BANK, stream);
        const int mmax = (int)std::min<int64_t>(d.N, d.ZR);
        for (int code = 0; code < L; code++) {
            GemmParams g = gemm_linear_fwd(c.Xh, H, a->bank_w + (size_t)code * H * H, H, c.Z, H, mmax, H, H);
            g.bias = a->bank_b + (size_t)code * H;
            g.relu = homo;
            g.ind = GEMM_IND_A_ROWS;
            g.seg = c.at<const int32_t>(c.w.seg) + code;
            g.list = c.at<const int32_t>(c.w.list);
            if (gemm3_pays(c.ctx, mmax, H, H, G3_BANK)) {
                if (int rc = launch_gemm3(stream, gemm3_of(g), g.ind)) return rc;
            } else if (int rc = launch_gemm(stream, g))
                return rc;
        }
    } else if (a->reuse_tables != 1) {
        StageTimer tm(ctx, ST_BANK, stream);
        GemmParams g = gemm_linear_fwd(c.Xh, H, a->bank_w, H, c.Z, (int64_t)L * H, d.N, H, L * H);
        g.bias = a->bank_b;
        g.relu = homo;
        g.absmax = epi_range ? &c.at<SeqRange>(c.w.range)->x : nullptr;
        if (gemm3_pays(c.ctx, d.N, L * H, H, G3_BANK)) {
            if (int rc = launch_gemm3(stream, gemm3_of(g))) return rc;
        } else if (int rc = launch_gemm(stream, g))
            return rc;
    }
    if (int rc = joiner.join()) return rc;
    if (d.math == PN_SEQ_MATH_F16X2 && (d.compact || a->reuse_tables != 1) && !epi_range) {
        StageTimer tm(ctx, ST_BANK, stream);
        if (int rc = launch_range_rows(stream, c.Z, d.ZR, H, d.compact ? c.at<const int32_t>(c.w.seg) + L : nullptr,
                                       c.at<SeqRange>(c.w.range)))
            return rc;
    }
    if (use_zw(c)) {
        StageTimer tm(ctx, ST_BANK, stream);
        const int GH = d.G * H;
        const int64_t n = (int64_t)GH * 2 * H;
        float *Wcat = c.at<float>(c.w.WpT);
        hipLaunchKernelGGL(gen_pack_kernel, dim3((unsigned)((n + 255) / 256)), dim3(256), 0, stream, a->w_ih, a->w_hh, a->b_ih,
                           a->b_hh, H, d.G, d.gru, Wcat, (float *)nullptr, c.at<float>(c.w.biasc));
        PN_CHECK_HIP(hipGetLastError());
        const int M = (int)d.ZR;
        const bool g3 = H % G3_KT == 0 && (int64_t)((M + G3_BM - 1) / G3_BM) * ((GH + G3_BN - 1) / G3_BN) >= 256;
        GemmParams g = gemm_linear_fwd(c.Z, H, Wcat, 2 * H, c.at<float>(c.w.saved), GH, M, H, GH);
        g.bias = c.at<float>(c.w.biasc);
        if (g3) {
            if (int rc = launch_gemm3(stream, gemm3_of(g))) return rc;
        } else if (int rc = launch_gemm(stream, g))
            return rc;
    }
    return PN_OK;
}

enum { DET_SEL = 0, DET_EGO = 1, DET_ROW = 2 };
struct DetOrder {
    const int32_t *keys;
    int64_t K, max_key;
};
inline DetOrder det_order(const Call &c, int which, int b) {
    const Dims &d = c.d;
    const int64_t Sb = c.groups(b), Pb = Sb * d.W;
    const bool homo = d.variant == PN_VARIANT_HOMO;
    switch (which) {
        case DET_SEL: return DetOrder{c.sel(b), Sb, (int64_t)d.N - 1};
        case DET_EGO: return DetOrder{c.at<const int32_t>(c.w.egoidx), Pb, homo ? d.ZR - 1 : (int64_t)d.N - 1};
        default: return DetOrder{c.at<const int32_t>(c.w.rowidx), Pb * d.L, d.ZR - 1};
    }
}

struct DetSegments {
    DetOrder o[3];
    int64_t n[3], off[3], total, max_key;
    int bits;
};
DetSegments det_segments(const Call &c, int b) {
    const bool has_att = c.d.variant != PN_VARIANT_PAGG;
    DetSegments g{};
    for (int which = 0; which < 3; which++) {
        g.o[which] = det_order(c, which, b);
        g.n[which] = (which == DET_EGO && !has_att) ? 0 : std::max<int64_t>(g.o[which].K, 0);
        g.off[which] = g.total;
        g.total += g.n[which];
        if (g.n[which]) g.max_key = std::max(g.max_key, g.o[which].max_key);
    }
    g.bits = 1;
    while (g.bits < 31 && (g.max_key >> g.bits) != 0) g.bits++;
    return g;
}

int prepare_det_orders(const Call &c, hipStream_t s, int b) {
    const DetSegments g = det_segments(c, b);
    if (g.total <= 0) return PN_OK;
    if (g.bits + 2 > 31)
        PN_FAIL(PN_ERR_ARG, "deterministic mode: %lld table rows leave no room for the scatters' segment bits", (long long)g.max_key + 1);
    DetKeys3 q{};
    for (int which = 0; which < 3; which++) {
        q.keys[which] = g.o[which].keys;
        q.n[which] = g.n[which];
        q.hi[which] = (int32_t)g.o[which].max_key;
    }
    q.shift = g.bits;
    int32_t *ck = c.at<int32_t>(c.w.keys), *pos = c.at<int32_t>(c.w.skey);
    hipLaunchKernelGGL(det_keys3_kernel, dim3((unsigned)((g.total + 255) / 256)), dim3(256), 0, s, q, ck, pos);
    PN_CHECK_HIP(hipGetLastError());
    return sort_pairs_i32(c.at<void>(c.w.stmp), c.w.stmp_bytes, ck, c.at<int32_t>(c.w.okey), pos, c.at<int32_t>(c.w.osrc),
                          g.total, g.bits + 2, s);
}

int fork_det_orders(const Call &c, JoinGuard &joiner, int b) {
    hipStream_t s = c.stream;
    if (!profiling_every_stage(c.ctx))
        if (void *side = context_fork(c.ctx, c.stream)) s = (hipStream_t)side;
    if (int rc = prepare_det_orders(c, s, b)) return rc;
    if (s != c.stream) return joiner.mark();
    return PN_OK;
}

DetScatterParams det_params(const Call &c, int which, int b, const float *rows, const float *scal, const float *vec, float *dst) {
    const DetSegments g = det_segments(c, b);
    const int64_t off = g.off[which];
    return DetScatterParams{c.at<int32_t>(c.w.okey) + off, c.at<int32_t>(c.w.osrc) + off, (int32_t)((1u << g.bits) - 1u),
                            g.n[which], off / DET_CHUNK + which, rows, scal, vec, dst, c.at<float>(c.w.cpart), c.d.H};
}

int run_det_scatters(const Call &c, const DetScatterParams *list, int count) {
    DetScatterPair pp{};
    int64_t kmax = 0;
    for (int i = 0; i < count; i++) pp.s[i] = list[i], kmax = std::max(kmax, list[i].K);
    if (kmax <= 0) return PN_OK;
    const int gpb = 256 / (c.d.H / 4);
    const int64_t chunks = (kmax + DET_CHUNK - 1) / DET_CHUNK;
    const dim3 grid((unsigned)((chunks + gpb - 1) / gpb), (unsigned)count);
    hipLaunchKernelGGL(det_scatter_kernel<1>, grid, dim3(256), 0, c.stream, pp);
    hipLaunchKernelGGL(det_scatter_kernel<2>, grid, dim3(256), 0, c.stream, pp);
    PN_CHECK_HIP(hipGetLastError());
    return PN_OK;
}

int run_det_scatter(const Call &c, int which, int b, const float *rows, const float *scal, const float *vec, float *dst) {
    const DetScatterParams p = det_params(c, which, b, rows, scal, vec, dst);
    return run_det_scatters(c, &p, 1);
}

inline float *grad_xh(const Call &c) { return c.a->Xh_in ? c.a->g_Xh : c.at<float>(c.w.dXh); }

inline hipStream_t fork_if(const Call &c, bool fork) {
    if (fork)
        if (void *side = context_fork(c.ctx, c.stream)) return (hipStream_t)side;
    return c.stream;
}

int run_fc2_grad(const Call &c, int b, JoinGuard &joiner, hipStream_t s, const float *g_out, float *loss, float grad_scale) {
    const Dims &d = c.d;
    const pn_pagg_args *a = c.a;
    const int H = d.H, Sb = c.groups(b);
    if (loss) {
        hipLaunchKernelGGL(loss_sum_kernel, dim3(1), dim3(1024), 0, s, c.at<const float>(c.w.outb), Sb, grad_scale, loss,
                           d.nb == 1 ? 1 : 0);
        PN_CHECK_HIP(hipGetLastError());
    }
    if (g_out) {
        StageTimer tm(c.ctx, ST_FC2_GRAD, s);
        GemmParams g = gemm_weight_grad(g_out, d.C, c.at<float>(c.w.layer1), 2 * H, a->g_fc2_w, 2 * H, Sb, 2 * H, d.C);
        g.rowsum = a->g_fc2_b;
        g.mode = GEMM_ATOMIC;
        if (a->g_fc2_w && d.det) {
            if (int rc = launch_gemm_det(s, g, (Sb + 127) / 128, c.at<float>(c.w.dgemm))) return rc;
        } else if (a->g_fc2_w) {
            if (int rc = launch_gemm(s, g, (Sb + 127) / 128)) return rc;
        } else if (a->g_fc2_b) {
            if (int rc = launch_colsum(s, g_out, nullptr, d.C, Sb, d.C, a->g_fc2_b, d.det)) return rc;
        }
    }
    return s != c.stream ? joiner.mark() : PN_OK;
}

PoolBwdParams pool_bwd_params(const Call &c, int b, const float *g_out) {
    const Dims &d = c.d;
    const pn_pagg_args *a = c.a;
    const int homo = d.variant == PN_VARIANT_HOMO;
    float *dXh = grad_xh(c), *scratch = c.at<float>(c.w.dl1);
    PoolBwdParams pp{};
    pp.variant = d.variant;
    pp.S = c.groups(b);
    pp.W = d.W;
    pp.H = d.H;
    pp.C = d.C;
    pp.N = d.N;
    pp.goff = c.group0(b);
    pp.hn = c.at<float>(c.w.hn);
    pp.ego_tab = homo ? c.Z : c.Xh;
    pp.egoidx = c.at<int32_t>(c.w.egoidx);
    pp.sel = c.sel(b);
    pp.att_w = a->att_w;
    pp.fc2_w = a->fc2_w;
    pp.g_out = g_out;
    pp.coef = c.at<float>(c.w.coef);
    pp.rawsc = c.at<float>(c.w.rawsc);
    pp.p_drop = a->p_cls;
    pp.seed = a->seed;
    pp.dyn = a->step_state;
    pp.mask = a->mask_cls;
    pp.dhn = c.at<float>(c.w.dhn);
    pp.dXh = dXh;
    pp.dego = homo ? c.at<float>(c.w.dZ) : dXh;
    pp.g_att_w = a->g_att_w ? a->g_att_w : scratch;
    pp.g_att_b = a->g_att_b ? a->g_att_b : scratch + 2 * d.H;
    pp.det_att = c.at<float>(c.w.datt);
    if (d.det) {
        pp.det_sel = c.at<float>(c.w.dsel);
        pp.det_ds = c.at<float>(c.w.dds);
    }
    return pp;
}
inline size_t pool_bwd_lds_bytes(const Dims &d) { return (size_t)(4 * (2 * d.W + d.H) + 8 * d.H + 8 * d.W) * sizeof(float); }

int run_pool_step(const Call &c, int b, const PoolBwdParams &pp, const int64_t *target, float grad_scale) {
    const Dims &d = c.d;
    const int H = d.H, Sb = pp.S, knob = knobs_of(c.ctx).pool_step;
    PoolStepParams ps{};
    ps.f = pool_fwd_params(c, b, c.a->out + (size_t)b * d.Sb * d.C);
    ps.b = pp;
    ps.target = target + (size_t)b * d.Sb;
    ps.scale = grad_scale;
    ps.gout = c.at<float>(c.w.gout);
    ps.b.g_out = ps.gout;
    ps.lossg = c.at<float>(c.w.outb);
    const size_t lds_step = std::max(pool_bwd_lds_bytes(d), pool_fwd_lds_bytes(d));
    StageTimer tm(c.ctx, ST_POOL_FWD, c.stream);
    const size_t lds_step2 = pool_step2_lds_bytes(10, H, d.C);
    if (d.W <= 40 && H <= 128 && H >= 32 && lds_step2 <= 64 * 1024 && knob >= 1 && knob != 2) {
        hipLaunchKernelGGL((pool_step2_kernel<10, 2>), dim3(Sb), dim3(256), lds_step2, c.stream, ps);
    } else if (H <= 256) {
        hipLaunchKernelGGL(pool_step_kernel<4>, dim3(Sb), dim3(256), lds_step, c.stream, ps);
    } else {
        if (int rc = ensure_dynamic_lds(c.ctx, reinterpret_cast<const void *>(pool_step_kernel<16>), (int)lds_step)) return rc;
        hipLaunchKernelGGL(pool_step_kernel<16>, dim3(Sb), dim3(256), lds_step, c.stream, ps);
    }
    PN_CHECK_HIP(hipGetLastError());
    return PN_OK;
}

int run_pool_bwd(const Call &c, const PoolBwdParams &pp, bool pool_step) {
    StageTimer tm(c.ctx, ST_POOL_BWD, c.stream);
    if (pool_step) return PN_OK;
    const size_t lds_bytes = pool_bwd_lds_bytes(c.d);
    if (pp.H <= 256) {
        hipLaunchKernelGGL(pool_bwd_wg_kernel<4>, dim3(pp.S), dim3(256), lds_bytes, c.stream, pp);
    } else {
        if (int rc = ensure_dynamic_lds(c.ctx, reinterpret_cast<const void *>(pool_bwd_wg_kernel<16>), (int)lds_bytes)) return rc;
        hipLaunchKernelGGL(pool_bwd_wg_kernel<16>, dim3(pp.S), dim3(256), lds_bytes, c.stream, pp);
    }
    PN_CHECK_HIP(hipGetLastError());
    return PN_OK;
}

int run_att_reduce(const Call &c, JoinGuard &joiner, hipStream_t s, const PoolBwdParams &pp) {
    if (c.d.variant != PN_VARIANT_PAGG) {
        hipLaunchKernelGGL(det_att_reduce_kernel, dim3((2 * pp.H + 4 + 63) / 64), dim3(1024), 0, s, pp.det_att, pp.S, pp.H,
                           pp.g_att_w, pp.g_att_b);
        PN_CHECK_HIP(hipGetLastError());
    }
    return s != c.stream ? joiner.mark() : PN_OK;
}

int run_pool_scatters(const Call &c, int b, const PoolBwdParams &pp) {
    const bool has_att = c.d.variant != PN_VARIANT_PAGG;
    const DetScatterParams two[2] = {det_params(c, DET_SEL, b, pp.det_sel, nullptr, nullptr, pp.dXh),
                                     det_params(c, DET_EGO, b, nullptr, pp.det_ds, c.a->att_w + c.d.H, pp.dego)};
    if (has_att && pp.dego != pp.dXh) return run_det_scatters(c, two, 2);
    if (int rc = run_det_scatters(c, two, 1)) return rc;
    return has_att ? run_det_scatters(c, two + 1, 1) : PN_OK;
}

int run_seq_bwd(const Call &c, int b) {
    const Dims &d = c.d;
    const pn_pagg_args *a = c.a;
    const bool f16 = d.math == PN_SEQ_MATH_F16X2;
    const int64_t Pb = (int64_t)c.groups(b) * d.W;
    float *dZ = c.at<float>(c.w.dZ);
    if (d.det && !f16) PN_CHECK_HIP(hipMemsetAsync(c.at<float>(c.w.dx), 0, (size_t)Pb * d.L * d.H * sizeof(float), c.stream));
    if (d.G == 0) {
        if (int rc = run_seq_reduce(c, b, true)) return rc;
    } else if (d.generic) {
        if (int rc = run_seq_bwd_generic(c, b)) return rc;
    } else {
        StageTimer tm(c.ctx, ST_SEQ_BWD, c.stream);
        SeqBwdParams sp{};
        sp.saved = c.at<float>(c.w.saved);
        sp.keep = (a->mask_seq || !(a->p_seq > 0.0f)) ? nullptr : c.at<const uint8_t>(c.w.keep);
        sp.dhn = c.at<float>(c.w.dhn);
        sp.rowidx = c.at<int32_t>(c.w.rowidx);
        sp.slotof = c.at<int32_t>(c.w.slotof);
        sp.WpT = c.at<float>(c.w.WpT);
        sp.dG = c.at<float>(c.w.dG);
        sp.dZ = dZ;
        sp.P = (int)Pb;
        sp.L = d.L;
        sp.Pmask = d.P_total;
        sp.p_drop = a->p_seq;
        sp.seed = a->seed;
        sp.mask = a->mask_seq;
        sp.merge0 = d.variant != PN_VARIANT_HETERO && !d.det;
        if (d.det) sp.rowidx = c.at<int32_t>(c.w.iota), sp.dZ = c.at<float>(c.w.dx);
        sp.range = c.at<SeqRange>(c.w.range);
        sp.store_dx = d.det && f16;
        if (int rc = f16 ? launch_seq_bwdh(c.ctx, c.stream, d.H, d.Gw, sp) : launch_seq_bwd3(c.ctx, c.stream, d.H, d.Gw, sp))
            return rc;
    }
    if (d.det) {
        StageTimer tm(c.ctx, ST_SEQ_BWD, c.stream);
        return run_det_scatter(c, DET_ROW, b, c.at<float>(c.w.dx), nullptr, nullptr, dZ);
    }
    return PN_OK;
}

int run_wgrad(const Call &c, int b, JoinGuard &joiner) {
    const Dims &d = c.d;
    const pn_pagg_args *a = c.a;
    const int H = d.H, GH = d.G * H;
    const hipStream_t ws = fork_if(c, !profiling_every_stage(c.ctx));
    WgradParams wp{};
    wp.dG = c.at<float>(c.w.dG);
    wp.xh = c.at<const float>(c.w.xh);
    wp.R = (int64_t)c.groups(b) * d.W * d.L;
    wp.GH = GH;
    wp.H2 = 2 * H;
    int nz = c.w.wgrad_split;
    if (a->Xh_in && a->g_Xh_ready) nz = std::min(nz, std::max(1, (WGRAD_CUS_SHARED + c.w.wgrad_tiles - 1) / c.w.wgrad_tiles));
    int64_t rps = (wp.R + nz - 1) / nz;
    rps = (rps + WG_KT - 1) / WG_KT * WG_KT;
    wp.rows_per_split = rps;
    const int64_t ntiles = (wp.R + WG_KT - 1) / WG_KT;
    const int nz_used = (int)(ntiles < nz ? ntiles : nz);
    wp.part_w = c.at<float>(c.w.wpart);
    wp.part_b = wp.part_w + (size_t)nz * GH * 2 * H;
    {
        StageTimer tm(c.ctx, ST_WGRAD, ws);
        int nz_red = nz_used;
        wp.range = c.at<SeqRange>(c.w.range);
        wp.xmul = seq_xmul(a);
        if (d.math == PN_SEQ_MATH_F16X2) {
            const int64_t nt16 = (wp.R + 15) / 16;
            nz_red = (int)(nt16 < nz ? nt16 : nz);
            if (int rc = launch_wgradh(c.ctx, ws, wp, H, nz_red)) return rc;
        } else if (seq4_select(c.ctx, H, d.G, d.L) & SEQ4_WGRAD) {
            const int64_t nt16 = (wp.R + 15) / 16;
            nz_red = (int)(nt16 < nz ? nt16 : nz);
            if (int rc = launch_wgrad4(c.ctx, ws, wp, nz_red)) return rc;
        } else {
            if (int rc = launch_wgrad3(c.ctx, ws, wp, nz_used)) return rc;
        }
        if (int rc = launch_wgrad_reduce(ws, wp.part_w, wp.part_b, nz_red, GH, H, b > 0 ? 1 : 0, d.gru,
                                         a->g_w_ih, a->g_w_hh, a->g_b_ih, a->g_b_hh))
            return rc;
    }
    return ws != c.stream ? joiner.mark() : PN_OK;
}

int run_bank_bwd(const Call &c, float *dXh, const float *dZ) {
    pn_context *ctx = c.ctx;
    hipStream_t stream = c.stream;
    const pn_pagg_args *a = c.a;
    const Dims &d = c.d;
    const int H = d.H, L = d.L;
    const float *Xh = c.Xh, *zgate = d.variant == PN_VARIANT_HOMO ? c.Z : nullptr;
    float *dgemm = d.det ? c.at<float>(c.w.dgemm) : nullptr;
    StageTimer tm(ctx, ST_BANK_BWD, stream);
    if (d.compact) {
        if (a->g_bank_b && !a->g_bank_w) PN_FAIL(PN_ERR_ARG, "pn_pagg_backward: compact rows need g_bank_w with g_bank_b");
        const int mmax = (int)std::min<int64_t>(d.N, d.ZR);
        const int32_t *seg = c.at<const int32_t>(c.w.seg), *list = c.at<const int32_t>(c.w.list);
        const bool g3 = (knobs_of(ctx).node_gemm3 & 8) && gemm3_pays(ctx, mmax, H, H, G3_BANK_DX);
        float *bankT = c.at<float>(c.w.bankT);
        if (g3)
            for (int code = 0; code < L; code++)
                launch_transpose(stream, a->bank_w + (size_t)code * H * H, H, H, bankT + (size_t)code * H * H);
        for (int code = 0; code < L; code++) {
            GemmParams g = g3 ? gemm_linear_fwd(dZ, H, bankT + (size_t)code * H * H, H, dXh, H, mmax, H, H)
                              : gemm_input_grad(dZ, H, a->bank_w + (size_t)code * H * H, H, dXh, H, mmax, H, H);
            g.gateA = zgate;
            g.mode = GEMM_ADD;
            g.ind = GEMM_IND_C_ROWS;
            g.seg = seg + code;
            g.list = list;
            if (g3) {
                if (int rc = launch_gemm3(stream, gemm3_of(g), g.ind)) return rc;
            } else if (int rc = launch_gemm(stream, g))
                return rc;
        }
        if (a->Xh_in && a->g_Xh_ready) PN_CHECK_HIP(hipEventRecord((hipEvent_t)a->g_Xh_ready, stream));
        for (int code = 0; code < L; code++) {
            GemmParams g = gemm_weight_grad(dZ, H, Xh, H, a->g_bank_w ? a->g_bank_w + (size_t)code * H * H : nullptr, H, mmax, H, H);
            g.gateA = zgate;
            g.rowsum = a->g_bank_b ? a->g_bank_b + (size_t)code * H : nullptr;
            g.mode = GEMM_ATOMIC;
            g.ind = GEMM_IND_K;
            g.seg = seg + code;
            g.list = list;
            if (a->g_bank_w && d.det) {
                if (int rc = launch_gemm_det(stream, g, (mmax + 255) / 256, dgemm)) return rc;
            } else if (a->g_bank_w && rgrad_pays(ctx, mmax, H, H)) {
                const RgradParams rp{dZ, zgate, Xh, H, H, mmax, H, H, a->g_bank_w + (size_t)code * H * H, H,
                                     a->g_bank_b ? a->g_bank_b + (size_t)code * H : nullptr, seg + code, list};
                if (int rc = launch_rgrad(ctx, stream, rp)) return rc;
            } else if (a->g_bank_w)
                if (int rc = launch_gemm(stream, g, (mmax + 255) / 256)) return rc;
        }
        return PN_OK;
    }
    if (gemm3_pays(ctx, d.N, H, L * H, G3_BANK_DX)) {
        float *bankT = c.at<float>(c.w.bankT);
        launch_transpose(stream, a->bank_w, L * H, H, bankT);
        GemmParams g = gemm_linear_fwd(dZ, (int64_t)L * H, bankT, (int64_t)L * H, dXh, H, d.N, L * H, H);
        g.gateA = zgate;
        g.mode = GEMM_ADD;
        if (int rc = launch_gemm3(stream, gemm3_of(g))) return rc;
    } else {
        GemmParams g = gemm_input_grad(dZ, (int64_t)L * H, a->bank_w, H, dXh, H, d.N, H, L * H);
        g.gateA = zgate;
        g.mode = GEMM_ADD;
        if (int rc = launch_gemm_split(stream, g, c.at<float>(c.w.gpart))) return rc;
    }
    if (a->Xh_in && a->g_Xh_ready) PN_CHECK_HIP(hipEventRecord((hipEvent_t)a->g_Xh_ready, stream));
    GemmParams g = gemm_weight_grad(dZ, (int64_t)L * H, Xh, H, a->g_bank_w, H, d.N, H, L * H);
    g.gateA = zgate;
    g.rowsum = a->g_bank_b;
    g.mode = GEMM_ATOMIC;
    if (a->g_bank_w && d.det) {
        if (int rc = launch_gemm_det(stream, g, (d.N + 255) / 256, dgemm)) return rc;
    } else if (a->g_bank_w && rgrad_pays(ctx, d.N, L * H, H)) {
        const RgradParams rp{dZ, zgate, Xh, (int64_t)L * H, H, d.N, L * H, H, a->g_bank_w, H, a->g_bank_b, nullptr, nullptr};
        if (int rc = launch_rgrad(ctx, stream, rp)) return rc;
    } else if (a->g_bank_w) {
        if (int rc = launch_gemm(stream, g, (d.N + 255) / 256)) return rc;
    } else if (a->g_bank_b) {
        if (int rc = launch_colsum(stream, dZ, zgate, (int64_t)L * H, d.N, L * H, a->g_bank_b, d.det)) return rc;
    }
    return PN_OK;
}

int run_fc0_bwd(const Call &c, const float *dXh) {
    pn_context *ctx = c.ctx;
    hipStream_t stream = c.stream;
    const pn_pagg_args *a = c.a;
    const Dims &d = c.d;
    const int H = d.H;
    const float *xgate = d.variant == PN_VARIANT_HOMO ? c.Xh : nullptr;
    StageTimer tm(ctx, ST_FC0_BWD, stream);
    GemmParams g = gemm_weight_grad(dXh, H, a->X, d.F, a->g_fc0_w, d.F, d.N, d.F, H);
    g.gateA = xgate;
    g.rowsum = a->g_fc0_b;
    g.mode = GEMM_ATOMIC;
    if (a->g_fc0_w && d.det) {
        if (int rc = launch_gemm_det(stream, g, (d.N + 255) / 256, c.at<float>(c.w.dgemm))) return rc;
    } else if (a->g_fc0_w && d.F % 4 == 0 && rgrad_pays(ctx, d.N, H, d.F)) {
        const RgradParams rp{dXh, xgate, a->X, H, d.F, d.N, H, d.F, a->g_fc0_w, d.F, a->g_fc0_b, nullptr, nullptr};
        if (int rc = launch_rgrad(ctx, stream, rp)) return rc;
    } else if (a->g_fc0_w && xpad_floats(d) > 0 && rgrad_pays(ctx, d.N, H, (d.F + 3) / 4 * 4)) {
        const int F4 = (d.F + 3) / 4 * 4;
        float *Xp = c.at<float>(c.w.xpad);
        const int64_t n4 = (int64_t)d.N * (F4 / 4);
        hipLaunchKernelGGL(pad_rows_kernel, dim3((unsigned)((n4 + 255) / 256)), dim3(256), 0, stream, a->X, (int64_t)d.N, d.F, F4, Xp);
        PN_CHECK_HIP(hipGetLastError());
        const RgradParams rp{dXh, xgate, Xp, H, F4, d.N, H, d.F, a->g_fc0_w, d.F, a->g_fc0_b, nullptr, nullptr};
        if (int rc = launch_rgrad(ctx, stream, rp)) return rc;
    } else if (a->g_fc0_w) {
        if (int rc = launch_gemm(stream, g, (d.N + 255) / 256)) return rc;
    } else if (a->g_fc0_b) {
        if (int rc = launch_colsum(stream, dXh, xgate, H, d.N, H, a->g_fc0_b, d.det)) return rc;
    }
    if (a->g_X) {
        GemmParams gx = gemm_input_grad(dXh, H, a->fc0_w, d.F, a->g_X, d.F, d.N, d.F, H);
        gx.gateA = xgate;
        if (int rc = launch_gemm(stream, gx)) return rc;
    }
    return PN_OK;
}

}

int pn::ZeroFill::flush(void *stream, bool timed) {
    if (!zl.n) return PN_OK;
    StageTimer tm(timed ? ctx : nullptr, ST_ZERO_FILL, stream);
    hipLaunchKernelGGL(zero_kernel, dim3(512), dim3(256), 0, (hipStream_t)stream, zl);
    PN_CHECK_HIP(hipGetLastError());
    zl.n = 0;
    return PN_OK;
}

extern "C" {

int pn_pagg_workspace_bytes(const pn_pagg_shape *shape, int64_t *bytes) {
    if (!shape || !bytes) PN_FAIL(PN_ERR_ARG, "pn_pagg_workspace_bytes: null");
    Dims d;
    if (int rc = make_dims(*shape, d)) return rc;
    *bytes = (int64_t)ws_layout(d).total;
    return PN_OK;
}

int pn_pagg_shape_info(const pn_pagg_shape *shape, int64_t out[4]) {
    if (!shape || !out) PN_FAIL(PN_ERR_ARG, "pn_pagg_shape_info: null");
    Dims d;
    if (int rc = make_dims(*shape, d)) return rc;
    out[0] = d.compact ? 1 : 0;
    out[1] = d.ZR;
    out[2] = d.nb;
    out[3] = d.math;
    return PN_OK;
}

int pn_pagg_paths_stream(pn_context *ctx, const pn_pagg_shape *shape, void *stream, void **out) {
    if (!shape || !out) PN_FAIL(PN_ERR_ARG, "pn_pagg_paths_stream: null");
    Dims d;
    if (int rc = make_dims(*shape, d)) return rc;
    void *side = (ctx && d.nb == 1 && !profiling_every_stage(ctx)) ? context_side_stream(ctx) : nullptr;
    *out = side ? side : stream;
    return PN_OK;
}

int pn_pagg_range_offset(const pn_pagg_shape *shape, int64_t *offset) {
    if (!shape || !offset) PN_FAIL(PN_ERR_ARG, "pn_pagg_range_offset: null");
    Dims d;
    if (int rc = make_dims(*shape, d)) return rc;
    static_assert(sizeof(SeqRange) == sizeof(pn_seq_range), "pn_seq_range is the public face of SeqRange");
    *offset = (d.math == PN_SEQ_MATH_F16X2 && d.G > 0 && !d.generic) ? (int64_t)ws_layout(d).range : -1;
    return PN_OK;
}

int pn_pagg_debug_offsets(const pn_pagg_shape *shape, int64_t out[4]) {
    if (!shape || !out) PN_FAIL(PN_ERR_ARG, "pn_pagg_debug_offsets: null");
    Dims d;
    if (int rc = make_dims(*shape, d)) return rc;
    const WsLayout w = ws_layout(d);
    out[0] = (int64_t)w.Xh;
    out[1] = (int64_t)w.Z;
    out[2] = (int64_t)w.hn;
    out[3] = (int64_t)w.layer1;
    return PN_OK;
}

int pn_pagg_gather(pn_context *ctx, const pn_pagg_shape *shape, const float *table, const int32_t *ids,
                   const uint8_t *codes, float *rows, void *stream_) {
    hipStream_t stream = (hipStream_t)stream_;
    if (!shape || !table || !ids || !codes || !rows) PN_FAIL(PN_ERR_ARG, "pn_pagg_gather: null");
    if (int rc = context_check_device(ctx)) return rc;
    const pn_pagg_shape &s = *shape;
    if (s.S < 0 || s.W < 1 || s.L < 1 || s.H < 1 || s.N < 1) PN_FAIL(PN_ERR_ARG, "pn_pagg_gather: bad shape");
    const int S_total = s.S_total > 0 ? s.S_total : s.S;
    if (s.group_begin < 0 || (int64_t)s.group_begin + s.S > S_total) PN_FAIL(PN_ERR_ARG, "pn_pagg_gather: bad slice");
    const int64_t count = (int64_t)s.S * s.W, rowsn = count * s.L;
    if (rowsn == 0) return PN_OK;
    const bool vec = (s.H % 4 == 0) && ((reinterpret_cast<uintptr_t>(table) | reinterpret_cast<uintptr_t>(rows)) % 16 == 0);
    const int64_t work = rowsn * (vec ? s.H / 4 : s.H);
    const int blocks = (int)std::min<int64_t>((work + 255) / 256, 256 * 32);
    const PlanDims pd{S_total, s.W, s.L, s.N, (int64_t)S_total * s.W, 0};
    const int64_t slot_begin = (int64_t)s.group_begin * s.W;
    StageTimer tm(ctx, ST_GATHER, stream);
    if (vec)
        hipLaunchKernelGGL(gather_kernel<4>, dim3(blocks), dim3(256), 0, stream, s.variant, table, ids, codes, pd,
                           slot_begin, count, s.H, rows);
    else
        hipLaunchKernelGGL(gather_kernel<1>, dim3(blocks), dim3(256), 0, stream, s.variant, table, ids, codes, pd,
                           slot_begin, count, s.H, rows);
    PN_CHECK_HIP(hipGetLastError());
    return PN_OK;
}

int pn_pagg_forward(pn_context *ctx, const pn_pagg_args *a, void *stream_) {
    hipStream_t stream = (hipStream_t)stream_;
    Call c;
    if (int rc = resolve_call(c, ctx, a, stream, "pn_pagg_forward")) return rc;
    const Dims &d = c.d;
    if (int rc = check_forward_args(c, "pn_pagg_forward")) return rc;
    if (d.S == 0) return PN_OK;
    JoinGuard joiner{ctx, stream};
    if (int rc = run_tables(c, joiner)) return rc;
    const bool save = d.nb == 1 && !a->no_save;
    if (save && d.det)
        if (int rc = fork_det_orders(c, joiner, 0)) return rc;
    for (int b = 0; b < d.nb; b++) {
        if (b > 0) {
            StageTimer tm(ctx, ST_PLAN_PACK, stream);
            if (int rc = run_plan(c, stream, b)) return rc;
        }
        if (int rc = run_seq_fwd(c, b, save)) return rc;
        if (int rc = run_pool_fwd(c, b, a->out + (size_t)b * d.Sb * d.C, true)) return rc;
    }
    return PN_OK;
}

static int pagg_backward_impl(pn_context *ctx, const pn_pagg_args *a, void *stream_, const int64_t *target, float grad_scale,
                              float *loss) {
    hipStream_t stream = (hipStream_t)stream_;
    const bool fused = target != nullptr;
    Call c;
    if (int rc = resolve_call(c, ctx, a, stream, fused ? "pn_pagg_train_step" : "pn_pagg_backward")) return rc;
    const Dims &d = c.d;
    if (fused) {
        if (d.S > 0)
            if (int rc = check_forward_args(c, "pn_pagg_train_step")) return rc;
        if (d.nb > 1 || d.S == 0) PN_CHECK_HIP(hipMemsetAsync(loss, 0, sizeof(float), stream));
    }
    if (!a->bank_w || !a->fc2_w || (d.S > 0 && (!a->ids || !a->codes || !a->sel || (!fused && !a->g_out && !a->g_embed))))
        PN_FAIL(PN_ERR_ARG, "pn_pagg_backward: null tensor");
    if (d.G > 0 && (!a->w_ih || !a->w_hh)) PN_FAIL(PN_ERR_ARG, "pn_pagg_backward: recurrent weights missing");
    if (!a->Xh_in && (!a->X || !a->fc0_w)) PN_FAIL(PN_ERR_ARG, "pn_pagg_backward: X / fc0 missing");
    if (a->Xh_in && !a->g_Xh) PN_FAIL(PN_ERR_ARG, "pn_pagg_backward: g_Xh is required with Xh_in");
    if (d.nb > 1 && !fused && ((d.G > 0 && (!a->b_ih || !a->b_hh)) || !a->fc2_b || (d.variant != PN_VARIANT_PAGG && !a->att_b)))
        PN_FAIL(PN_ERR_ARG, "pn_pagg_backward: micro-batches re-run the forward and need every forward tensor");
    const int H = d.H, L = d.L, GwH = d.Gw * H;
    const bool has_att = d.variant != PN_VARIANT_PAGG;
    float *dZ = c.at<float>(c.w.dZ), *dXh = grad_xh(c);
    ZeroFill zf{ctx};
    if (int rc = zf.add(dZ, (size_t)d.ZR * H)) return rc;
    if (int rc = zf.add(dXh, (size_t)d.N * H)) return rc;
    if (int rc = zf.add(a->g_att_w, has_att ? (size_t)2 * H : 0)) return rc;
    if (int rc = zf.add(a->g_att_b, has_att ? 1 : 0)) return rc;
    if (has_att && (!a->g_att_w || !a->g_att_b))
        if (int rc = zf.add(c.at<float>(c.w.dl1), (size_t)2 * H + 1)) return rc;
    if (int rc = zf.add(a->g_fc2_b, (size_t)d.C)) return rc;
    if (int rc = zf.add(a->g_fc2_w, (size_t)d.C * 2 * H)) return rc;
    if (int rc = zf.add(a->g_bank_w, (size_t)L * H * H)) return rc;
    if (int rc = zf.add(a->g_bank_b, (size_t)L * H)) return rc;
    if (!a->Xh_in) {
        if (int rc = zf.add(a->g_fc0_w, (size_t)H * d.F)) return rc;
        if (int rc = zf.add(a->g_fc0_b, (size_t)H)) return rc;
    }
    if (d.S == 0) {
        if (int rc = zf.flush(stream)) return rc;
        if (int rc = zf.add(a->g_w_ih, (size_t)GwH * H)) return rc;
        if (int rc = zf.add(a->g_w_hh, (size_t)GwH * H)) return rc;
        if (int rc = zf.add(a->g_b_ih, (size_t)GwH)) return rc;
        if (int rc = zf.add(a->g_b_hh, (size_t)GwH)) return rc;
        if (int rc = zf.add(a->g_X, (size_t)d.N * d.F)) return rc;
        if (int rc = zf.flush(stream)) return rc;
        if (a->Xh_in && a->g_Xh_ready) PN_CHECK_HIP(hipEventRecord((hipEvent_t)a->g_Xh_ready, stream));
        return PN_OK;
    }
    JoinGuard joiner{ctx, stream};
    if (int rc = fused ? run_tables(c, joiner, &zf) : zf.flush(stream)) return rc;
    const bool side_ok = !profiling_every_stage(ctx) && !d.det;
    const bool pool_step = fused && !d.det && knobs_of(ctx).pool_step != 0;
    if (d.det) {
        const int64_t n = std::max<int64_t>((int64_t)d.Sb * d.W * L, d.Sb);
        hipLaunchKernelGGL(det_iota_kernel, dim3((unsigned)((n + 255) / 256)), dim3(256), 0, stream, c.at<int32_t>(c.w.iota), n);
        PN_CHECK_HIP(hipGetLastError());
    }
    if (d.G > 0 && !d.generic) {
        StageTimer tm(ctx, ST_PLAN_PACK, stream);
        if (d.math != PN_SEQ_MATH_F16X2)
            if (int rc = launch_pack_bwd3(stream, a->w_ih, a->w_hh, H, d.G, d.gru, c.at<void>(c.w.WpT))) return rc;
    }
    const bool wgrad_wanted = d.G > 0 && (a->g_w_ih || a->g_w_hh || a->g_b_ih || a->g_b_hh);
    const bool small_behind_pool = side_ok && wgrad_wanted && ctx != nullptr;
    const bool rerun = fused || d.nb > 1;
    for (int b = 0; b < d.nb; b++) {
        const float *g_out = fused ? c.at<const float>(c.w.gout) : a->g_out ? a->g_out + (size_t)b * d.Sb * d.C : nullptr;
        float *loss_sum = pool_step ? loss : nullptr;
        if (rerun) {
            if (!(fused && b == 0)) {
                StageTimer tm(ctx, ST_PLAN_PACK, stream);
                if (int rc = run_plan(c, stream, b)) return rc;
            }
            if (d.det)
                if (int rc = fork_det_orders(c, joiner, b)) return rc;
            if (int rc = run_seq_fwd(c, b, true)) return rc;
            if (!pool_step) {
                float *out_b = fused ? a->out + (size_t)b * d.Sb * d.C : c.at<float>(c.w.outb);
                if (int rc = run_pool_fwd(c, b, out_b)) return rc;
                if (fused)
                    if (int rc = launch_cross_entropy(out_b, target + (size_t)b * d.Sb, c.groups(b), d.C, grad_scale, loss,
                                                      c.at<float>(c.w.gout), stream, d.nb == 1))
                        return rc;
            }
        }
        PoolBwdParams pp = pool_bwd_params(c, b, g_out);
        if (a->g_embed) pp.g_embed = a->g_embed + (size_t)b * d.Sb * 2 * H;
        if (pool_step)
            if (int rc = run_pool_step(c, b, pp, target, grad_scale)) return rc;
        if (!small_behind_pool)
            if (int rc = run_fc2_grad(c, b, joiner, fork_if(c, side_ok), g_out, loss_sum, grad_scale)) return rc;
        if (int rc = run_pool_bwd(c, pp, pool_step)) return rc;
        const hipStream_t small = fork_if(c, small_behind_pool);
        if (small_behind_pool)
            if (int rc = run_fc2_grad(c, b, joiner, small, g_out, loss_sum, grad_scale)) return rc;
        if (int rc = run_att_reduce(c, joiner, small, pp)) return rc;
        if (d.det) {
            if (rerun)
                if (int rc = joiner.join()) return rc;
            if (int rc = run_pool_scatters(c, b, pp)) return rc;
        }
        if (int rc = run_seq_bwd(c, b)) return rc;
        if (wgrad_wanted)
            if (int rc = run_wgrad(c, b, joiner)) return rc;
        if (b + 1 < d.nb)
            if (int rc = joiner.join()) return rc;
    }
    if (int rc = run_bank_bwd(c, dXh, dZ)) return rc;
    if (a->Xh_in) return PN_OK;
    return run_fc0_bwd(c, dXh);
}

int pn_pagg_backward(pn_context *ctx, const pn_pagg_args *a, void *stream) {
    return pagg_backward_impl(ctx, a, stream, nullptr, 0.0f, nullptr);
}

int pn_pagg_train_step(pn_context *ctx, const pn_pagg_args *a, const int64_t *target, float grad_scale, float *loss,
                       void *stream) {
    if (!a) PN_FAIL(PN_ERR_ARG, "pn_pagg_train_step: null args");
    if (a->out_embed || a->out_path_weight || a->out_path_state || a->g_embed)
        PN_FAIL(PN_ERR_ARG, "pn_pagg_train_step: out_embed / out_path_weight / out_path_state / g_embed are for pn_pagg_forward / "
                            "pn_pagg_backward");
    if (!loss || (a->shape.S > 0 && !target)) PN_FAIL(PN_ERR_ARG, "pn_pagg_train_step: null target / loss");
    if (a->shape.S == 0) {
        PN_CHECK_HIP(hipMemsetAsync(loss, 0, sizeof(float), (hipStream_t)stream));
        return pagg_backward_impl(ctx, a, stream, nullptr, 0.0f, nullptr);
    }
    return pagg_backward_impl(ctx, a, stream, target, grad_scale, loss);
}

}

#ifdef PN_POOL_TRACE
extern "C" int pn_debug_pool_trace(long long *host_out) {
    return hipMemcpyFromSymbol(host_out, HIP_SYMBOL(g_pool_trace), sizeof(long long) * 2048 * 12) == hipSuccess ? 0 : -1;
}
#endif
```

pathnet_amd/modules.py:

```python
import collections
import ctypes
import os

import numpy as np
import torch
import torch.nn as nn

from . import _lib

dropout = 0.7

_VARIANT = {"hetero": _lib.VARIANT_HETERO, "homo": _lib.VARIANT_HOMO, "pagg": _lib.VARIANT_PAGG}
_CELL = {None: _lib.CELL_DEFAULT, "lstm": _lib.CELL_LSTM, "rnn": _lib.CELL_RNN, "gru": _lib.CELL_GRU,
         "mean": _lib.CELL_MEAN, "sum": _lib.CELL_SUM}
_HEAD_PARAMS = ("fc0_w", "fc0_b", "w_ih", "w_hh", "b_ih", "b_hh", "att_w", "att_b", "fc2_w", "fc2_b")


WORKSPACE_BUDGET_BYTES = 48 << 30
MIN_BATCH_BYTES = 8 << 30


def default_budget(device=None):
    try:
        free, _ = torch.cuda.mem_get_info(device)
        return int(min(WORKSPACE_BUDGET_BYTES, max(0.6 * free, MIN_BATCH_BYTES)))
    except Exception:
        return WORKSPACE_BUDGET_BYTES


_SEQ_MATH = {None: _lib.SEQ_MATH_DEFAULT, "": _lib.SEQ_MATH_DEFAULT, "f16x2": _lib.SEQ_MATH_F16X2, "bf16x3": _lib.SEQ_MATH_BF16X3}


def compact_default():
    e = os.environ.get("PN_COMPACT")
    if e is None or e == "":
        return _lib.COMPACT_AUTO
    return _lib.COMPACT_ON if int(e) != 0 else _lib.COMPACT_OFF


RANGE_WINDOW_BITS = 18
RANGE_POLL_EVERY = 16


def seq_math_default():
    e = os.environ.get("PN_SEQ_MATH", "").strip().lower()
    if e not in _SEQ_MATH:
        raise ValueError("PN_SEQ_MATH=%r: f16x2 or bf16x3" % e)
    return _SEQ_MATH[e]


class PaggCall:
    SHAPE_FIELDS = ("variant", "N", "F", "H", "C", "S", "W", "L", "S_total", "group_begin", "batch_groups", "cell",
                    "deterministic", "compact", "seq_math")
    __slots__ = SHAPE_FIELDS + ("p_seq", "p_cls", "seed", "mask_seq", "mask_cls", "step_state", "index_rows_local", "bank_w",
                                "bank_b", "grad", "reuse_tables", "grad_scale", "path_state", "sparse_plan", "workspace",
                                "_shape", "_ws_bytes")

    def __init__(self, variant, N, F, H, C, S, W, L, S_total=0, group_begin=0, batch_groups=0, cell=None, deterministic=False,
                 compact=None, seq_math=None, *, p_seq=0.0, p_cls=0.0, seed=0, mask_seq=None, mask_cls=None, step_state=None,
                 index_rows_local=False, bank_w=None, bank_b=None, grad=True, reuse_tables=0, grad_scale=1.0,
                 path_state=False, sparse_plan=None, workspace=None):
        self.variant, self.N, self.F, self.H, self.C, self.S, self.W, self.L = variant, N, F, H, C, S, W, L
        self.S_total, self.group_begin, self.batch_groups, self.cell = S_total, group_begin, batch_groups, cell
        self.deterministic = bool(deterministic)
        self.compact = compact_default() if compact is None else int(compact)
        self.seq_math = seq_math_default() if seq_math is None else int(seq_math)
        self.p_seq, self.p_cls, self.seed, self.mask_seq, self.mask_cls = p_seq, p_cls, seed, mask_seq, mask_cls
        self.step_state, self.index_rows_local, self.bank_w, self.bank_b = step_state, index_rows_local, bank_w, bank_b
        self.grad, self.reuse_tables, self.grad_scale, self.path_state = grad, reuse_tables, grad_scale, path_state
        self.sparse_plan, self.workspace = sparse_plan, workspace
        self._shape = self._ws_bytes = None

    def get(self, name, default=None):
        return getattr(self, name)
    __getitem__ = get

    def shape(self):
        if self._shape is None:
            self._shape = _lib.PaggShape(_VARIANT[self.variant], self.N, self.F, self.H, self.C, self.S, self.W, self.L,
                                         self.S_total, self.group_begin, self.batch_groups, _CELL[self.cell],
                                         1 if self.deterministic else 0, self.compact, self.seq_math)
        return self._shape

    def set_batch_groups(self, bg):
        self.batch_groups = bg
        self._shape = self._ws_bytes = None
        return self

    def pick_batch_groups(self, budget, device=None):
        return self.set_batch_groups(pick_batch_groups(
            self.variant, self.N, self.F, self.H, self.C, self.S, self.W, self.L, budget, cell=self.cell, device=device,
            deterministic=self.deterministic, S_total=self.S_total, group_begin=self.group_begin, compact=self.compact,
            seq_math=self.seq_math))

    def workspace_bytes(self):
        if self._ws_bytes is None:
            n = ctypes.c_int64(0)
            _lib.check(_lib.load().pn_pagg_workspace_bytes(ctypes.byref(self.shape()), ctypes.byref(n)))
            self._ws_bytes = n.value
        return self._ws_bytes

    def take_workspace(self, dev, have=None):
        need = self.workspace_bytes()
        if have is not None and have.numel() >= need and have.device == dev:
            return have
        return torch.empty(max(need, 1), dtype=torch.uint8, device=dev)

    def args(self, ids, codes, sel, p, X=None, Xh=None):
        a = _lib.PaggArgs()
        a.shape = self.shape()
        if Xh is None:
            a.X, names = X.data_ptr(), _HEAD_PARAMS
        else:
            a.Xh_in, names = Xh.data_ptr(), _HEAD_PARAMS[2:]
        a.ids, a.codes, a.sel = ids.data_ptr(), codes.data_ptr(), sel.data_ptr()
        for k in names:
            if p[k] is not None:
                setattr(a, k, p[k].data_ptr())
        a.bank_w, a.bank_b = self.bank_w.data_ptr(), self.bank_b.data_ptr()
        a.p_seq, a.p_cls, a.seed = self.p_seq, self.p_cls, self.seed
        a.mask_seq = self.mask_seq.data_ptr() if self.mask_seq is not None else None
        a.mask_cls = self.mask_cls.data_ptr() if self.mask_cls is not None else None
        a.step_state = self.step_state.ptr() if self.step_state is not None else None
        a.index_rows_local = 1 if self.index_rows_local else 0
        return a

    def grad_buffers(self, a, p, X=None, flat=False):
        keys = [k for k in _HEAD_PARAMS if getattr(a, k)]
        like = [p[k] for k in keys] + [self.bank_w, self.bank_b]
        buf = None
        if flat:
            sizes = [-(-t.numel() // 4) * 4 for t in like]
            buf = torch.empty(sum(sizes), dtype=torch.float32, device=self.bank_w.device)
            pieces = [v[:t.numel()].view(t.shape) for v, t in zip(buf.split(sizes), like)]
        else:
            pieces = [torch.empty_like(t) for t in like]
        grads = dict(zip(keys + ["bank_w", "bank_b"], pieces))
        for k, g in grads.items():
            setattr(a, "g_" + k, g.data_ptr())
        gX = torch.empty_like(X) if X is not None else None
        a.g_X = gX.data_ptr() if gX is not None else None
        return grads, gX, buf


def _shape(variant, N, F, H, C, S, W, L, S_total=0, group_begin=0, batch_groups=0, cell=None, deterministic=False,
           compact=None, seq_math=None):
    return PaggCall(variant, N, F, H, C, S, W, L, S_total, group_begin, batch_groups, cell, deterministic, compact, seq_math).shape()


def shape_info(sh):
    out = (ctypes.c_int64 * 4)()
    _lib.check(_lib.load().pn_pagg_shape_info(ctypes.byref(sh), out))
    return bool(out[0]), int(out[1]), int(out[2]), int(out[3])


def deterministic_default():
    return torch.are_deterministic_algorithms_enabled() or os.environ.get("PN_DETERMINISTIC", "0") not in ("", "0")


def workspace_bytes(variant, N, F, H, C, S, W, L, S_total=0, group_begin=0, batch_groups=0, cell=None, deterministic=False,
                    compact=None, seq_math=None):
    return PaggCall(variant, N, F, H, C, S, W, L, S_total, group_begin, batch_groups, cell, deterministic, compact, seq_math).workspace_bytes()


def pick_batch_groups(variant, N, F, H, C, S, W, L, budget=None, cell=None, device=None, deterministic=False,
                      S_total=0, group_begin=0, compact=None, seq_math=None):
    call = PaggCall(variant, N, F, H, C, S, W, L, S_total, group_begin, 0, cell, deterministic, compact, seq_math)

    def ws(bg):
        return call.set_batch_groups(bg).workspace_bytes()
    need = ws(0) if S > 1 else 0
    floor = MIN_BATCH_BYTES if budget is None else 0
    if budget is None:
        if need <= MIN_BATCH_BYTES:
            return 0
        budget = default_budget(device)
    budget = int(budget)
    if S <= 1 or need <= budget:
        return 0
    step = min(1024, S - 1)
    w1 = ws(1)
    per_group = max((ws(1 + step) - w1) // step, 1) if step > 0 else max(need, 1)
    fixed = w1 - per_group
    avail = max(budget - fixed, floor)
    bg = int(max(1, min(S, avail // per_group if avail > 0 else 1)))
    if floor == 0:
        while bg > 1 and ws(bg) > budget:
            bg = max(1, min(bg - 1, int(bg * 0.98)))
        for _ in range(16):
            if bg >= S or ws(bg + 1) > budget:
                break
            bg += 1
    return bg


def _split_params(params, L):
    p = dict(zip(_HEAD_PARAMS, params[:10]))
    p["bank_ws"], p["bank_bs"] = params[10:10 + L], params[10 + L:10 + 2 * L]
    return p


def _grad_tuple(grads, L):
    return tuple(grads.get(k) for k in _HEAD_PARAMS) + tuple(grads["bank_w"][d] for d in range(L)) + tuple(
        grads["bank_b"][d] for d in range(L))


def _begin(call, ids, codes, sel, p, X=None, Xh=None):
    dev = ids.device
    out = torch.empty((call.S, call.C), dtype=torch.float32, device=dev)
    ws = call.take_workspace(dev, call.workspace)
    a = call.args(ids, codes, sel, p, X=X, Xh=Xh)
    a.out = out.data_ptr()
    a.workspace, a.workspace_bytes = ws.data_ptr(), ws.numel()
    return a, out, ws


class _PaggFunction(torch.autograd.Function):

    @staticmethod
    def _forward(ctx, call, X, ids, codes, sel, params, encode_out=None):
        p = _split_params(params, call.L)
        dev = X.device
        with torch.cuda.device(dev):
            a, out, ws = _begin(call, ids, codes, sel, p, X=X)
            a.no_save = 0 if call.grad else 1
            a.reuse_tables = int(call.reuse_tables or 0)
            if encode_out is not None:
                a.out_embed, a.out_path_weight = encode_out[0].data_ptr(), encode_out[1].data_ptr()
                a.out_path_state = encode_out[2].data_ptr() if encode_out[2] is not None else None
            if call.S > 0:
                _lib.check(_lib.load().pn_pagg_forward(_lib.context(dev), ctypes.byref(a), _lib.stream_ptr(dev)))
        ctx.call, ctx.ws = call, ws
        ctx.present = [t is not None for t in params]
        ctx.save_for_backward(X, ids, codes, sel, *[t for t in params if t is not None])
        return out

    @staticmethod
    def forward(ctx, call, X, ids, codes, sel, *params):
        return _PaggFunction._forward(ctx, call, X, ids, codes, sel, params)

    @staticmethod
    def backward(ctx, g_out):
        return _PaggFunction._backward(ctx, g_out, None)

    @staticmethod
    def _backward(ctx, g_out, g_embed):
        call = ctx.call
        saved = list(ctx.saved_tensors)
        X, ids, codes, sel = saved[:4]
        it = iter(saved[4:])
        params = [next(it) if pres else None for pres in ctx.present]
        p = _split_params(params, call.L)
        dev = X.device
        with torch.cuda.device(dev):
            g_out = g_out.contiguous().float() if g_out is not None else None
            g_embed = g_embed.contiguous().float() if g_embed is not None else None
            a = call.args(ids, codes, sel, p, X=X)
            grads, gX, _ = call.grad_buffers(a, p, X if ctx.needs_input_grad[1] else None)
            a.workspace, a.workspace_bytes = ctx.ws.data_ptr(), ctx.ws.numel()
            a.g_out = g_out.data_ptr() if g_out is not None else None
            a.g_embed = g_embed.data_ptr() if g_embed is not None else None
            if call.S > 0:
                _lib.check(_lib.load().pn_pagg_backward(_lib.context(dev), ctypes.byref(a), _lib.stream_ptr(dev)))
            else:
                for g in list(grads.values()) + [gX] * (gX is not None):
                    g.zero_()
        return (None, gX, None, None, None) + _grad_tuple(grads, call.L)


class _PaggEncodeFunction(torch.autograd.Function):

    @staticmethod
    def forward(ctx, call, X, ids, codes, sel, *params):
        S, W, H, dev = call.S, call.W, call.H, X.device
        with torch.cuda.device(dev):
            emb = torch.empty((S, 2 * H), dtype=torch.float32, device=dev)
            pw = torch.empty((S, W), dtype=torch.float32, device=dev)
            ps = torch.empty((S, W, H), dtype=torch.float32, device=dev) if call.path_state else None
        out = _PaggFunction._forward(ctx, call, X, ids, codes, sel, params, encode_out=(emb, pw, ps))
        ctx.mark_non_differentiable(*[t for t in (pw, ps) if t is not None])
        ctx.set_materialize_grads(False)
        return (out, emb, pw) if ps is None else (out, emb, pw, ps)

    @staticmethod
    def backward(ctx, g_out, g_embed, *_unused):
        if g_out is None and g_embed is None:
            return (None,) * (5 + len(ctx.present))
        return _PaggFunction._backward(ctx, g_out, g_embed)


class _PaggLossFunction(torch.autograd.Function):

    @staticmethod
    def forward(ctx, call, X, ids, codes, sel, target, *params):
        p = _split_params(params, call.L)
        dev = X.device
        with torch.cuda.device(dev):
            a, out, _ = _begin(call, ids, codes, sel, p, X=X)
            loss = (torch.empty if call.S > 0 else torch.zeros)((), dtype=torch.float32, device=dev)
            grads, gX, flat = call.grad_buffers(a, p, X if ctx.needs_input_grad[1] else None, flat=True)
            target = target.to(device=dev, dtype=torch.int64).contiguous()
            if call.S > 0:
                _lib.check(_lib.load().pn_pagg_train_step(_lib.context(dev), ctypes.byref(a), target.data_ptr(),
                                                          float(call.grad_scale), loss.data_ptr(), _lib.stream_ptr(dev)))
            else:
                flat.zero_()
                if gX is not None:
                    gX.zero_()
        ctx.grads = (gX,) + _grad_tuple(grads, call.L)
        ctx.flat = flat
        ctx.mark_non_differentiable(out)
        ctx.set_materialize_grads(False)
        return loss, out

    @staticmethod
    @torch.autograd.function.once_differentiable
    def backward(ctx, g_loss, _g_out):
        grads, flat = ctx.grads, ctx.flat
        ctx.grads = ctx.flat = None
        if grads is None:
            raise RuntimeError("forward_loss: the gradients were handed out already (backward twice)")
        from . import optim
        if g_loss is None:
            return (None,) * (6 + len(grads) - 1)
        one = optim._UNIT.get(g_loss.device)
        if one is None or g_loss.data_ptr() != one.data_ptr():
            flat.mul_(g_loss)
            if grads[0] is not None:
                grads[0].mul_(g_loss)
        return (None, grads[0], None, None, None, None) + tuple(grads[1:])


def _as_index_tensors(neis, layer_type, indices, num_w, walk_len, device, n_nodes=None):
    if isinstance(indices, np.ndarray):
        if indices.dtype == np.bool_:
            sel = torch.from_numpy(np.flatnonzero(indices).astype(np.int32))
        elif np.issubdtype(indices.dtype, np.integer):
            sel = torch.from_numpy(np.ascontiguousarray(indices).reshape(-1).astype(np.int32))
        else:
            raise TypeError("indices: bool mask or integer node ids expected, got numpy %s" % indices.dtype)
    else:
        idx = torch.as_tensor(indices)
        if idx.dtype == torch.bool:
            sel = torch.nonzero(idx, as_tuple=False).flatten().to(torch.int32)
        elif not idx.dtype.is_floating_point and not idx.dtype.is_complex:
            sel = idx.flatten().to(torch.int32)
        else:
            raise TypeError("indices: bool mask or integer node ids expected, got %s" % idx.dtype)
    S = int(sel.numel())
    ids = torch.as_tensor(neis)
    codes = torch.as_tensor(layer_type)
    if ids.numel() != S * num_w * walk_len or codes.numel() != S * num_w * walk_len:
        raise ValueError("neis / layer_type hold %d / %d entries, %d masked nodes x %d paths x %d steps = %d expected"
                         % (ids.numel(), codes.numel(), S, num_w, walk_len, S * num_w * walk_len))
    if n_nodes is not None and S and sel.device.type == "cpu":
        lo, hi = int(sel.min()), int(sel.max())
        if lo < 0 or hi >= n_nodes:
            raise IndexError("indices name node %d, the feature matrix has %d rows" % (lo if lo < 0 else hi, n_nodes))
    if ids.dtype != torch.int32:
        ids = ids.to(torch.int32)
    if codes.dtype != torch.uint8:
        codes = codes.to(torch.uint8)
    ids = ids.reshape(S, num_w, walk_len).to(device, non_blocking=True).contiguous()
    codes = codes.reshape(S, num_w, walk_len).to(device, non_blocking=True).contiguous()
    return ids, codes, sel.to(device, non_blocking=True).contiguous(), S


Encoded = collections.namedtuple("Encoded", ("logits", "embedding", "path_weight", "path_state"))


def _explicit_masks(ms, mc, H, Hk, seq_math, check_range=True):
    if ms is None and mc is None:
        return None, None
    if Hk != H:
        P = torch.nn.functional.pad
        ms = P(ms, (0, Hk - H)).contiguous() if ms is not None else None
        mc = P(mc.view(mc.shape[0], 2, H), (0, Hk - H)).reshape(mc.shape[0], 2 * Hk).contiguous() if mc is not None else None
    if ms is not None and check_range and seq_math != _lib.SEQ_MATH_BF16X3 and float(ms.abs().max()) > 16.0:
        raise ValueError("explicit sequence masks must satisfy |m| <= 16 with seq_math f16x2 (include/pathnet_hip.h); "
                         "use seq_math='bf16x3' for others")
    return ms, mc


class _Aggregator(nn.Module):
    variant = None

    def _common_init(self, feature_length, hidden_size, out_size, dropout_p, cell=None):
        _lib.load()
        if cell not in _CELL:
            raise ValueError("cell must be one of %s" % sorted(k for k in _CELL if k))
        self.cell = cell
        self.feature_length, self.hidden_size, self.out_size = feature_length, hidden_size, out_size
        self._dropout = dropout_p
        self._ws_eval = None
        self._ws_tables = None
        self.step_state = None
        self.workspace_budget = None
        self.deterministic = None
        self.seq_math = None
        self.range_guard = True
        self._range_wide = False
        self._range_calls = 0
        self._range_pending = None
        self.range_spread_bits = None
        self._mask_seq = None
        self._mask_cls = None
        self._bank_flat = (None, None)

    def dropout_p(self):
        return float(dropout if self._dropout is None else self._dropout)

    def set_dropout(self, p):
        self._dropout = p

    def _bank_layers(self):
        raise NotImplementedError

    def _tables_key(self, X, L):
        lins = [self.fc0] + list(self._bank_layers())
        return (X.data_ptr(), tuple(X.shape), int(X._version), int(L),
                tuple(int(t._version) for l in lins for t in (l.weight, l.bias)))

    def _make_cell(self, default):
        kind = self.cell or default
        H = self.hidden_size
        if kind == "lstm":
            self.LSTM = nn.LSTM(H, H)
        elif kind == "rnn":
            self.RNN = nn.RNN(H, H)
        elif kind == "gru":
            self.GRU = nn.GRU(H, H)
        self._cell_kind = kind

    def _cell(self):
        return {"lstm": getattr(self, "LSTM", None), "rnn": getattr(self, "RNN", None),
                "gru": getattr(self, "GRU", None)}.get(self._cell_kind)

    def _bank(self):
        lins = self._bank_layers()
        H = self.hidden_size
        fw, fb = self._bank_flat
        ok = (fw is not None and fw.device == lins[0].weight.device and
              all(l.weight.data_ptr() == fw.data_ptr() + d * H * H * 4 and l.bias.data_ptr() == fb.data_ptr() + d * H * 4
                  for d, l in enumerate(lins)))
        if not ok:
            with torch.no_grad():
                fw = torch.stack([l.weight.detach() for l in lins]).contiguous()
                fb = torch.stack([l.bias.detach() for l in lins]).contiguous()
                for d, l in enumerate(lins):
                    l.weight.data = fw[d]
                    l.bias.data = fb[d]
            self._bank_flat = (fw, fb)
        return fw, fb, [l.weight for l in lins], [l.bias for l in lins]

    def _padded_param_inputs(self, Hk):
        H, G = self.hidden_size, {"lstm": 4, "rnn": 1, "gru": 3}.get(self._cell_kind, 0)
        pad = Hk - H
        P = torch.nn.functional.pad

        def rows(w):
            return P(w, (0, 0) * (w.dim() - 1) + (0, pad))

        def gates(w):
            if w.dim() == 2:
                return P(w.view(G, H, H), (0, pad, 0, pad)).reshape(G * Hk, Hk)
            return P(w.view(G, H), (0, pad)).reshape(G * Hk)

        def halves(w):
            return P(w.view(w.shape[0], 2, H), (0, pad)).reshape(w.shape[0], 2 * Hk)
        lins = self._bank_layers()
        ws = [P(l.weight, (0, pad, 0, pad)) for l in lins]
        bs = [P(l.bias, (0, pad)) for l in lins]
        cell = self._cell()
        att = getattr(self, "attw", None)
        rec = tuple(gates(t) for t in (cell.weight_ih_l0, cell.weight_hh_l0, cell.bias_ih_l0, cell.bias_hh_l0)) \
            if cell is not None else (None,) * 4
        head = (rows(self.fc0.weight), P(self.fc0.bias, (0, pad))) + rec + (
            halves(att.weight) if att is not None else None, att.bias if att is not None else None,
            halves(self.fc2.weight), self.fc2.bias)
        with torch.no_grad():
            fw, fb = torch.stack([w.detach() for w in ws]).contiguous(), torch.stack([b.detach() for b in bs]).contiguous()
        return fw, fb, head + tuple(ws) + tuple(bs)

    def _param_inputs(self):
        fw, fb, ws, bs = self._bank()
        cell = self._cell()
        att = getattr(self, "attw", None)
        rec = (cell.weight_ih_l0, cell.weight_hh_l0, cell.bias_ih_l0, cell.bias_hh_l0) if cell is not None else (None,) * 4
        head = (self.fc0.weight, self.fc0.bias) + rec + (
                att.weight if att is not None else None, att.bias if att is not None else None,
                self.fc2.weight, self.fc2.bias)
        return fw, fb, head + tuple(ws) + tuple(bs)

    def forward_loss(self, X, neis, num_w, walk_len, indices, layer_type, target, indxx=None, grad_scale=None, fused=None):
        return self._run(X, neis, num_w, walk_len, indices, layer_type, target=target, grad_scale=grad_scale, fused=fused)

    def forward(self, X, neis, num_w, walk_len, indices, layer_type, indxx=None, reuse_tables=False, group_slice=None):
        return self._run(X, neis, num_w, walk_len, indices, layer_type, reuse_tables=reuse_tables, group_slice=group_slice)

    def encode(self, X, neis, num_w, walk_len, indices, layer_type, indxx=None, *, path_state=False, group_slice=None,
               reuse_tables=False, seed=None):
        res = self._run(X, neis, num_w, walk_len, indices, layer_type, reuse_tables=reuse_tables, group_slice=group_slice,
                        seed=seed, _encode=bool(path_state))
        logits, emb, pw = res[:3]
        ps = res[3] if path_state else None
        H = self.hidden_size
        Hk = emb.shape[1] // 2
        if Hk != H:
            S = emb.shape[0]
            emb = emb.view(S, 2, Hk)[:, :, :H].reshape(S, 2 * H)
            ps = ps[:, :, :H].contiguous() if ps is not None else None
        return Encoded(logits, emb, pw, ps)

    def paths_stream(self):
        cur = torch.cuda.current_stream()
        last = getattr(self, "_last_shape", None)
        if last is None or self.step_state is not None:
            prev = getattr(self, "_paths_stream_prev", None)
            if prev is not None and prev.cuda_stream != cur.cuda_stream:
                cur.wait_stream(prev)
            self._paths_stream_prev = cur
            return cur
        shape, dev = last
        out = ctypes.c_void_p()
        with torch.cuda.device(dev):
            cur = torch.cuda.current_stream(dev)
            _lib.check(_lib.load().pn_pagg_paths_stream(_lib.context(dev), ctypes.byref(shape), _lib.stream_ptr(dev), ctypes.byref(out)))
        new = cur if (not out.value or out.value == cur.cuda_stream) else torch.cuda.ExternalStream(out.value, device=dev)
        prev = getattr(self, "_paths_stream_prev", None)
        if prev is not None and prev.cuda_stream != new.cuda_stream:
            new.wait_stream(prev)
            new.wait_stream(cur)
        self._paths_stream_prev = new
        return new

    def _range_eval(self, rec):
        x_bits, esum, cnt = int(rec[0]) & 0xFFFFFFFF, int(rec[1]), int(rec[2]) & 0xFFFFFFFF
        if cnt > 0 and x_bits:
            self.range_spread_bits = ((x_bits >> 23) & 255) - esum / cnt
            if self.range_spread_bits > RANGE_WINDOW_BITS and not self._range_wide:
                self._range_wide = True
                import warnings
                warnings.warn("pathnet_amd: the distance-bank rows span %.1f bits between their largest value and the typical row "
                              "(window of the fp16 x 2 recurrent kernels: %d); this module now runs seq_math='bf16x3'"
                              % (self.range_spread_bits, RANGE_WINDOW_BITS))

    def _range_poll(self):
        if self._range_pending is not None and self._range_pending[1].query():
            rec, _ = self._range_pending
            self._range_pending = None
            self._range_eval(rec)

    def _range_read(self, call, ws, sync):
        off = ctypes.c_int64(-1)
        _lib.check(_lib.load().pn_pagg_range_offset(ctypes.byref(call.shape()), ctypes.byref(off)))
        if ws is None or off.value < 0:
            return
        rec = torch.empty(6, dtype=torch.int32, pin_memory=True)
        rec.copy_(ws[off.value:off.value + 24].view(torch.int32), non_blocking=True)
        ev = torch.cuda.Event()
        ev.record()
        if sync:
            ev.synchronize()
            self._range_eval(rec)
        else:
            self._range_pending = (rec, ev)

    def _call_modes(self):
        return (deterministic_default() if self.deterministic is None else bool(self.deterministic), compact_default(),
                seq_math_default() if self.seq_math is None else _SEQ_MATH[self.seq_math])

    def _run(self, X, neis, num_w, walk_len, indices, layer_type, reuse_tables=False, group_slice=None, target=None,
             grad_scale=None, fused=None, batch_position=None, seed=None, _math=None, _encode=None):
        dev = X.device
        if dev.type != "cuda":
            raise RuntimeError("pathnet_amd aggregators run on the GPU only (X is on %s); no CPU fallback" % dev)
        X = X.contiguous().float()
        ids, codes, sel, S = _as_index_tensors(neis, layer_type, indices, num_w, walk_len, dev, n_nodes=X.shape[0])
        H, L = self.hidden_size, int(walk_len)
        Hk = -(-H // 32) * 32
        fw, fb, params = self._param_inputs() if Hk == H else self._padded_param_inputs(Hk)
        training = self.training
        p = self.dropout_p() if training else 0.0
        det, compact, math = self._call_modes()
        if _math is not None:
            math = _math
        guard = (_math is None and self.seq_math is None and self.range_guard and math != _lib.SEQ_MATH_BF16X3 and
                 self.step_state is None)
        if guard:
            self._range_poll()
            if self._range_wide:
                math, guard = _lib.SEQ_MATH_BF16X3, False
        draws = p > 0 and self.step_state is None
        seed = (int(seed) if seed is not None else int(torch.randint(0, 2 ** 62, (1,)).item())) if draws else 0
        S_total = begin = 0
        if batch_position is not None:
            if self.variant == "hetero" or group_slice is not None:
                raise ValueError("batch_position: homo / PAGG classes, without group_slice")
            S_total, begin = int(batch_position[0]), int(batch_position[1])
            if begin < 0 or begin + S > S_total:
                raise ValueError("batch_position (%d, %d): %d rows do not fit" % (S_total, begin, S))
        if group_slice is not None:
            begin, count = int(group_slice[0]), int(group_slice[1])
            if begin < 0 or count < 0 or begin + count > S:
                raise ValueError("group_slice (%d, %d) outside the batch of %d masked nodes" % (begin, count, S))
            S_total, S = S, count
        if len(params) != 10 + 2 * L:
            raise ValueError("walk_len=%d but the module has %d distance layers" % (L, (len(params) - 10) // 2))
        ms, mc = _explicit_masks(self._mask_seq, self._mask_cls, H, Hk, math) if training else (None, None)
        p_drop = p if ms is None and mc is None else 0.0
        grad = torch.is_grad_enabled()
        call = PaggCall(self.variant, X.shape[0], X.shape[1], Hk, self.out_size, S, int(num_w), L, S_total, begin, 0,
                        self._cell_kind, det, compact, math, p_seq=p_drop, p_cls=p_drop, seed=seed, mask_seq=ms, mask_cls=mc,
                        step_state=self.step_state, index_rows_local=batch_position is not None, bank_w=fw, bank_b=fb,
                        grad=grad, path_state=bool(_encode))
        call.pick_batch_groups(self.workspace_budget, dev)
        self._last_shape = (call.shape(), dev)
        if not grad:
            ws = call.take_workspace(dev, self._ws_eval)
            fits = ws is self._ws_eval
            key = self._tables_key(X, L)
            compact_now = shape_info(call.shape())[0]
            have_key, have_dense = self._ws_tables if self._ws_tables is not None else (None, False)
            if reuse_tables and fits and have_key == key:
                call.reuse_tables = 1 if (have_dense and not compact_now) else 2
            call.workspace = self._ws_eval = ws
            self._ws_tables = (key, not compact_now) if S > 0 else None
        elif reuse_tables:
            raise RuntimeError("reuse_tables is for no-grad (inference) forwards")
        else:
            call.workspace = call.take_workspace(dev)
            self._ws_tables = None
        if target is not None:
            if not grad:
                raise RuntimeError("forward_loss computes gradients: call it with grad enabled")
            target = torch.as_tensor(target)
            if target.numel() != S:
                raise ValueError("target holds %d classes, the batch has %d masked nodes" % (target.numel(), S))
            call.grad_scale = (1.0 / max(S, 1)) if grad_scale is None else float(grad_scale)
            target = target.reshape(-1)
            if fused is None:
                fused = call.batch_groups > 0
            if fused:
                res = _PaggLossFunction.apply(call, X, ids, codes, sel, target, *params)
            else:
                from . import optim
                out = _PaggFunction.apply(call, X, ids, codes, sel, *params)
                loss = optim.CrossEntropyLoss()(out, target.to(device=dev, dtype=torch.int64))
                if grad_scale is not None:
                    loss = loss * (float(grad_scale) * max(S, 1))
                res = (loss, out)
        elif _encode is not None:
            res = _PaggEncodeFunction.apply(call, X, ids, codes, sel, *params)
        else:
            res = _PaggFunction.apply(call, X, ids, codes, sel, *params)
        if guard and S > 0:
            first = self._range_calls == 0
            self._range_calls += 1
            if first or (self._range_calls % RANGE_POLL_EVERY == 0 and self._range_pending is None):
                self._range_read(call, call.workspace, sync=first)
                if first and self._range_wide:
                    return self._run(X, neis, num_w, walk_len, indices, layer_type, reuse_tables=False, group_slice=group_slice,
                                     target=target, grad_scale=grad_scale, fused=fused, batch_position=batch_position,
                                     seed=seed, _math=_lib.SEQ_MATH_BF16X3, _encode=_encode)
        return res


class PathNet(_Aggregator):
    variant = "hetero"

    def __init__(self, feature_length, hidden_size, out_size, wl, dropout=None, cell=None, **kwargs):
        super().__init__()
        self._common_init(feature_length, hidden_size, out_size, dropout, cell)
        self.fc0 = nn.Linear(feature_length, hidden_size)
        self._make_cell("lstm")
        self.fc2 = nn.Linear(2 * hidden_size, out_size)
        self.nets = nn.ModuleList([nn.Linear(hidden_size, hidden_size) for _ in range(wl)])
        self.attw = nn.Linear(2 * hidden_size, 1)
        self.Lrelu = nn.LeakyReLU()

    def _bank_layers(self):
        return list(self.nets)


class PathNet_homo(PathNet):
    variant = "homo"

    def __init__(self, feature_length, hidden_size, out_size, wl, dropout=None, cell=None, **kwargs):
        super().__init__(feature_length, hidden_size, out_size, wl, dropout=dropout, cell=cell, **kwargs)
        nn.init.xavier_uniform_(self.fc0.weight)
        nn.init.xavier_uniform_(self.fc2.weight)


class PAGG(_Aggregator):
    variant = "pagg"

    def __init__(self, feature_length, hidden_size, out_size, node_num, dropout=0.9, cell=None, **kwargs):
        super().__init__()
        self._common_init(feature_length, hidden_size, out_size, dropout, cell)
        self.node_num = node_num
        self.fc0 = nn.Linear(feature_length, hidden_size)
        self._make_cell("rnn")
        self.fc2 = nn.Linear(2 * hidden_size, out_size)
        self.nei0 = nn.Linear(hidden_size, hidden_size)
        self.nei1 = nn.Linear(hidden_size, hidden_size)
        self.nei2 = nn.Linear(hidden_size, hidden_size)
        self.nei3 = nn.Linear(hidden_size, hidden_size)
        for lin in (self.fc0, self.fc2, self.nei0, self.nei1, self.nei2, self.nei3):
            nn.init.xavier_uniform_(lin.weight)

    def _bank_layers(self):
        return [self.nei0, self.nei1, self.nei2, self.nei3]
```

Baseline: 61.54 million paths/s.

## Use sparse CSR/CSC features for fc0 forward and weight gradient

Adds a sparse feature path. The feature matrix X is scanned once into CSR and CSC form, and the result is cached per tensor version. The fc0 forward becomes an SpMM against a transposed weight, and the fc0 weight gradient becomes a sparse product, so the dense N×F×H GEMMs are skipped for bag-of-words style inputs such as Cora-shaped features. In auto mode it needs N≥2048 and density ≤1/64, and the sparse structure is reused across steps, keyed on the data pointer and version, which is a legitimate preprocessing cache for a constant input. It adds a per-step weight transpose and one-time host-synchronising scans, and it is slower if the features are not actually sparse.

```diff
diff --git a/include/pathnet_hip.h b/include/pathnet_hip.h
--- a/include/pathnet_hip.h
+++ b/include/pathnet_hip.h
@@ -260,6 +260,22 @@
 int pn_pagg_train_step(pn_context *ctx, const pn_pagg_args *args, const int64_t *target, float grad_scale, float *loss,
                        void *stream);
 
+typedef struct pn_sparse_features {
+    int64_t nnz;
+    int32_t *row_off;
+    int32_t *col;
+    float *val;
+    int32_t *col_off;
+    int32_t *row;
+    float *valc;
+} pn_sparse_features;
+int pn_sparse_count(pn_context *ctx, const float *X, int32_t N, int32_t F, int32_t *row_off, int32_t *col_off, void *stream);
+int pn_sparse_fill(pn_context *ctx, const float *X, int32_t N, int32_t F, const pn_sparse_features *features, void *stream);
+int pn_pagg_forward_sparse(pn_context *ctx, const pn_pagg_args *args, const pn_sparse_features *features, void *stream);
+int pn_pagg_backward_sparse(pn_context *ctx, const pn_pagg_args *args, const pn_sparse_features *features, void *stream);
+int pn_pagg_train_step_sparse(pn_context *ctx, const pn_pagg_args *args, const pn_sparse_features *features,
+                              const int64_t *target, float grad_scale, float *loss, void *stream);
+
 int pn_pagg_gather(pn_context *ctx, const pn_pagg_shape *shape, const float *table , const int32_t *ids,
                    const uint8_t *codes, float *rows , void *stream);
 
diff --git a/pathnet_amd/_lib.py b/pathnet_amd/_lib.py
--- a/pathnet_amd/_lib.py
+++ b/pathnet_amd/_lib.py
@@ -62,6 +62,10 @@
                  ("reuse_tables", ctypes.c_int32),
                  ("index_rows_local", ctypes.c_int32), ("step_state", vp),
                  ("out_embed", vp), ("out_path_weight", vp), ("out_path_state", vp), ("g_embed", vp)])
+
+
+class SparseFeatures(ctypes.Structure):
+    _fields_ = [("nnz", ctypes.c_int64), ("row_off", vp), ("col", vp), ("val", vp), ("col_off", vp), ("row", vp), ("valc", vp)]
 
 
 class WalkStatsOut(ctypes.Structure):
@@ -159,6 +163,12 @@
     "pn_linear_backward": (ctypes.c_int, [vp, vp, vp, vp, vp, ctypes.c_int32, ctypes.c_int32, ctypes.c_int32, vp, vp,
                                           vp, vp, ctypes.c_int64, vp]),
     "pn_pagg_train_step": (ctypes.c_int, [vp, ctypes.POINTER(PaggArgs), vp, ctypes.c_float, vp, vp]),
+    "pn_sparse_count": (ctypes.c_int, [vp, vp, ctypes.c_int32, ctypes.c_int32, vp, vp, vp]),
+    "pn_sparse_fill": (ctypes.c_int, [vp, vp, ctypes.c_int32, ctypes.c_int32, ctypes.POINTER(SparseFeatures), vp]),
+    "pn_pagg_forward_sparse": (ctypes.c_int, [vp, ctypes.POINTER(PaggArgs), ctypes.POINTER(SparseFeatures), vp]),
+    "pn_pagg_backward_sparse": (ctypes.c_int, [vp, ctypes.POINTER(PaggArgs), ctypes.POINTER(SparseFeatures), vp]),
+    "pn_pagg_train_step_sparse": (ctypes.c_int, [vp, ctypes.POINTER(PaggArgs), ctypes.POINTER(SparseFeatures), vp,
+                                                 ctypes.c_float, vp, vp]),
     "pn_pagg_debug_offsets": (ctypes.c_int, [ctypes.POINTER(PaggShape), c_i64p]),
     "pn_pagg_range_offset": (ctypes.c_int, [ctypes.POINTER(PaggShape), c_i64p]),
     "pn_pagg_paths_stream": (ctypes.c_int, [vp, ctypes.POINTER(PaggShape), vp, ctypes.POINTER(ctypes.c_void_p)]),
diff --git a/pathnet_amd/csrc/pn_context.hip b/pathnet_amd/csrc/pn_context.hip
--- a/pathnet_amd/csrc/pn_context.hip
+++ b/pathnet_amd/csrc/pn_context.hip
@@ -75,7 +75,8 @@
 const KnobName kKnobs[] = {{"PN_NODE_GEMM3", &pn::Knobs::node_gemm3}, {"PN_EVAL_ZW", &pn::Knobs::eval_zw},
                            {"PN_POOL_STEP", &pn::Knobs::pool_step}, {"PN_EVENT_DEVICE_SCOPE", &pn::Knobs::event_dev},
                            {"PN_NODE_RGRAD", &pn::Knobs::node_rgrad}, {"PN_SAMPLER_STAGE", &pn::Knobs::sampler_stage},
-                           {"PN_SEQ4", &pn::Knobs::seq4}, {"PN_SEQH_TAIL", &pn::Knobs::seqh_tail}};
+                           {"PN_SEQ4", &pn::Knobs::seq4}, {"PN_SEQH_TAIL", &pn::Knobs::seqh_tail},
+                           {"PN_FC0_SPARSE", &pn::Knobs::fc0_sparse}};
 
 }
 
diff --git a/pathnet_amd/csrc/pn_internal.h b/pathnet_amd/csrc/pn_internal.h
--- a/pathnet_amd/csrc/pn_internal.h
+++ b/pathnet_amd/csrc/pn_internal.h
@@ -45,6 +45,7 @@
     int sampler_stage = -1;
     int seq4 = 4;
     int seqh_tail = PN_SEQH_TAIL_DEFAULT;
+    int fc0_sparse = 1;
 };
 const Knobs &knobs_of(const pn_context *ctx);
 
diff --git a/pathnet_amd/csrc/pn_pagg.hip b/pathnet_amd/csrc/pn_pagg.hip
--- a/pathnet_amd/csrc/pn_pagg.hip
+++ b/pathnet_amd/csrc/pn_pagg.hip
@@ -9,6 +9,7 @@
 #include "pn_internal.h"
 #include "pn_kernels.h"
 #include "pn_seq.h"
+#include "pn_sparse.h"
 
 using namespace pn;
 
@@ -1292,6 +1293,7 @@
     size_t flags, rank, list, seg, bsum;
     size_t dx, keys, iota, skey, stmp, cpart, dsel, dds, datt, dgemm;
     size_t okey, osrc;
+    size_t w0t;
     size_t stmp_bytes;
     int wgrad_split, wgrad_tiles;
     size_t total;
@@ -1374,6 +1376,7 @@
         w.dds = take(Pb * 4);
         w.dgemm = take(std::max({det_gemm_floats(C, 2 * H), det_gemm_floats(d.compact ? H : L * H, H), det_gemm_floats(H, F)}) * 4);
     }
+    w.w0t = take(d.H <= 256 ? (size_t)d.F * H * 4 : 0);
     w.total = at;
     return w;
 }
@@ -1404,6 +1407,7 @@
     char *ws;
     const float *Xh;
     float *Z;
+    const pn_sparse_features *sp;
     template <class T>
     T *at(size_t off) const { return reinterpret_cast<T *>(ws + off); }
     int groups(int b) const { return std::min(d.Sb, d.S - b * d.Sb); }
@@ -1411,7 +1415,8 @@
     const int32_t *sel(int b) const { return a->sel + (a->index_rows_local ? (int64_t)b * d.Sb : group0(b)); }
 };
 
-int resolve_call(Call &c, pn_context *ctx, const pn_pagg_args *a, hipStream_t stream, const char *who) {
+int resolve_call(Call &c, pn_context *ctx, const pn_pagg_args *a, hipStream_t stream, const char *who,
+                 const pn_sparse_features *sp = nullptr) {
     if (!a) PN_FAIL(PN_ERR_ARG, "%s: null args", who);
     if (int rc = context_check_device(ctx)) return rc;
     if (int rc = make_dims(a->shape, c.d)) return rc;
@@ -1426,6 +1431,7 @@
     c.ws = reinterpret_cast<char *>(a->workspace);
     c.Xh = a->Xh_in ? a->Xh_in : c.at<const float>(c.w.Xh);
     c.Z = c.at<float>(c.w.Z);
+    c.sp = (sp && !a->Xh_in && c.d.H <= 256 && (int64_t)c.d.N * c.d.F <= SPARSE_MAX_ELEMS && knobs_of(ctx).fc0_sparse != 0) ? sp : nullptr;
     if (a->index_rows_local && c.d.variant == PN_VARIANT_HETERO && (c.d.group_begin != 0 || c.d.S != c.d.S_total))
         PN_FAIL(PN_ERR_ARG, "%s: the hetero class reads paths of the whole batch (PathNet_run.py:196-197): "
                 "index_rows_local needs the whole batch's ids / codes", who);
@@ -1743,7 +1749,11 @@
             g.bias = a->fc0_b;
             g.relu = homo;
             g.clear_word = epi_range ? &c.at<SeqRange>(c.w.range)->x : nullptr;
-            if (gemm3_pays(c.ctx, d.N, H, d.F, G3_FC0)) {
+            if (c.sp) {
+                float *W0T = c.at<float>(c.w.w0t);
+                if (int rc = launch_transpose(stream, a->fc0_w, H, d.F, W0T)) return rc;
+                if (int rc = launch_sparse_fc0_fwd(stream, *c.sp, d.N, H, W0T, g.bias, g.relu, g.clear_word, g.C)) return rc;
+            } else if (gemm3_pays(c.ctx, d.N, H, d.F, G3_FC0)) {
                 if (int rc = launch_gemm3(stream, gemm3_of(g))) return rc;
             } else if (int rc = launch_gemm_split(stream, g, c.at<float>(c.w.gpart)))
                 return rc;
@@ -2203,7 +2213,11 @@
     g.gateA = xgate;
     g.rowsum = a->g_fc0_b;
     g.mode = GEMM_ATOMIC;
-    if (a->g_fc0_w && d.det) {
+    if (a->g_fc0_w && c.sp) {
+        if (int rc = launch_sparse_fc0_wgrad(stream, *c.sp, d.N, d.F, H, dXh, xgate, a->g_fc0_w, d.det ? nullptr : a->g_fc0_b)) return rc;
+        if (a->g_fc0_b && d.det)
+            if (int rc = launch_colsum(stream, dXh, xgate, H, d.N, H, a->g_fc0_b, true)) return rc;
+    } else if (a->g_fc0_w && d.det) {
         if (int rc = launch_gemm_det(stream, g, (d.N + 255) / 256, c.at<float>(c.w.dgemm))) return rc;
     } else if (a->g_fc0_w && d.F % 4 == 0 && rgrad_pays(ctx, d.N, H, d.F)) {
         const RgradParams rp{dXh, xgate, a->X, H, d.F, d.N, H, d.F, a->g_fc0_w, d.F, a->g_fc0_b, nullptr, nullptr};
@@ -2318,10 +2332,14 @@
     return PN_OK;
 }
 
-int pn_pagg_forward(pn_context *ctx, const pn_pagg_args *a, void *stream_) {
+int pn_pagg_forward(pn_context *ctx, const pn_pagg_args *a, void *stream) {
+    return pn_pagg_forward_sparse(ctx, a, nullptr, stream);
+}
+
+int pn_pagg_forward_sparse(pn_context *ctx, const pn_pagg_args *a, const pn_sparse_features *sp, void *stream_) {
     hipStream_t stream = (hipStream_t)stream_;
     Call c;
-    if (int rc = resolve_call(c, ctx, a, stream, "pn_pagg_forward")) return rc;
+    if (int rc = resolve_call(c, ctx, a, stream, "pn_pagg_forward", sp)) return rc;
     const Dims &d = c.d;
     if (int rc = check_forward_args(c, "pn_pagg_forward")) return rc;
     if (d.S == 0) return PN_OK;
@@ -2342,11 +2360,11 @@
 }
 
 static int pagg_backward_impl(pn_context *ctx, const pn_pagg_args *a, void *stream_, const int64_t *target, float grad_scale,
-                              float *loss) {
+                              float *loss, const pn_sparse_features *sp) {
     hipStream_t stream = (hipStream_t)stream_;
     const bool fused = target != nullptr;
     Call c;
-    if (int rc = resolve_call(c, ctx, a, stream, fused ? "pn_pagg_train_step" : "pn_pagg_backward")) return rc;
+    if (int rc = resolve_call(c, ctx, a, stream, fused ? "pn_pagg_train_step" : "pn_pagg_backward", sp)) return rc;
     const Dims &d = c.d;
     if (fused) {
         if (d.S > 0)
@@ -2454,11 +2472,20 @@
 }
 
 int pn_pagg_backward(pn_context *ctx, const pn_pagg_args *a, void *stream) {
-    return pagg_backward_impl(ctx, a, stream, nullptr, 0.0f, nullptr);
+    return pagg_backward_impl(ctx, a, stream, nullptr, 0.0f, nullptr, nullptr);
+}
+
+int pn_pagg_backward_sparse(pn_context *ctx, const pn_pagg_args *a, const pn_sparse_features *sp, void *stream) {
+    return pagg_backward_impl(ctx, a, stream, nullptr, 0.0f, nullptr, sp);
 }
 
 int pn_pagg_train_step(pn_context *ctx, const pn_pagg_args *a, const int64_t *target, float grad_scale, float *loss,
                        void *stream) {
+    return pn_pagg_train_step_sparse(ctx, a, nullptr, target, grad_scale, loss, stream);
+}
+
+int pn_pagg_train_step_sparse(pn_context *ctx, const pn_pagg_args *a, const pn_sparse_features *sp, const int64_t *target,
+                              float grad_scale, float *loss, void *stream) {
     if (!a) PN_FAIL(PN_ERR_ARG, "pn_pagg_train_step: null args");
     if (a->out_embed || a->out_path_weight || a->out_path_state || a->g_embed)
         PN_FAIL(PN_ERR_ARG, "pn_pagg_train_step: out_embed / out_path_weight / out_path_state / g_embed are for pn_pagg_forward / "
@@ -2466,9 +2493,9 @@
     if (!loss || (a->shape.S > 0 && !target)) PN_FAIL(PN_ERR_ARG, "pn_pagg_train_step: null target / loss");
     if (a->shape.S == 0) {
         PN_CHECK_HIP(hipMemsetAsync(loss, 0, sizeof(float), (hipStream_t)stream));
-        return pagg_backward_impl(ctx, a, stream, nullptr, 0.0f, nullptr);
-    }
-    return pagg_backward_impl(ctx, a, stream, target, grad_scale, loss);
+        return pagg_backward_impl(ctx, a, stream, nullptr, 0.0f, nullptr, sp);
+    }
+    return pagg_backward_impl(ctx, a, stream, target, grad_scale, loss, sp);
 }
 
 }
diff --git a/pathnet_amd/csrc/pn_sparse.h b/pathnet_amd/csrc/pn_sparse.h
--- /dev/null
+++ b/pathnet_amd/csrc/pn_sparse.h
@@ -0,0 +1,17 @@
+#pragma once
+#include <hip/hip_runtime.h>
+
+#include <cstdint>
+
+#include "pn_internal.h"
+
+namespace pn {
+
+constexpr int64_t SPARSE_MAX_ELEMS = (int64_t)1 << 28;
+
+int launch_sparse_fc0_fwd(hipStream_t stream, const pn_sparse_features &sp, int N, int H, const float *W0T, const float *bias,
+                          int relu, uint32_t *clear_word, float *Xh);
+int launch_sparse_fc0_wgrad(hipStream_t stream, const pn_sparse_features &sp, int N, int F, int H, const float *dXh,
+                            const float *gate, float *g_w, float *g_b);
+
+}
diff --git a/pathnet_amd/csrc/pn_sparse.hip b/pathnet_amd/csrc/pn_sparse.hip
--- /dev/null
+++ b/pathnet_amd/csrc/pn_sparse.hip
@@ -0,0 +1,332 @@
+#include <hip/hip_runtime.h>
+
+#include "pn_sparse.h"
+
+namespace pn {
+namespace {
+
+__device__ __forceinline__ int wave_bcast(int v, int lane) { return __builtin_amdgcn_readlane(v, lane); }
+__device__ __forceinline__ float wave_bcast(float v, int lane) {
+    return __int_as_float(__builtin_amdgcn_readlane(__float_as_int(v), lane));
+}
+
+__global__ __launch_bounds__(256) void sp_count_rows_kernel(const float *__restrict__ X, int N, int F, int32_t *__restrict__ row_off) {
+    const int lane = threadIdx.x & 63;
+    const int n = blockIdx.x * 4 + (threadIdx.x >> 6);
+    if (n >= N) return;
+    const float *x = X + (int64_t)n * F;
+    int cnt = 0;
+    for (int f = lane; f < F; f += 64) cnt += x[f] != 0.0f ? 1 : 0;
+    for (int o = 32; o > 0; o >>= 1) cnt += __shfl_xor(cnt, o);
+    if (lane == 0) row_off[n + 1] = cnt;
+}
+
+__global__ __launch_bounds__(64) void sp_count_cols_kernel(const float *__restrict__ X, int N, int F, int32_t *__restrict__ col_off) {
+    const int f = blockIdx.x * 64 + threadIdx.x;
+    if (f >= F) return;
+    const float *x = X + f;
+    int cnt = 0;
+#pragma unroll 8
+    for (int n = 0; n < N; n++) cnt += x[(int64_t)n * F] != 0.0f ? 1 : 0;
+    col_off[f + 1] = cnt;
+}
+
+__global__ __launch_bounds__(1024) void sp_scan_kernel(int32_t *__restrict__ off_a, int na, int32_t *__restrict__ off_b, int nb) {
+    __shared__ int wsum[16];
+    int32_t *off = blockIdx.x == 0 ? off_a : off_b;
+    const int n = blockIdx.x == 0 ? na : nb;
+    const int tid = threadIdx.x, lane = tid & 63, wave = tid >> 6;
+    int carry = 0;
+    for (int base = 0; base < n; base += 4096) {
+        const int i = base + tid * 4;
+        int v[4];
+#pragma unroll
+        for (int u = 0; u < 4; u++) v[u] = i + u < n ? off[1 + i + u] : 0;
+        const int t = v[0] + v[1] + v[2] + v[3];
+        int incl = t;
+        for (int o = 1; o < 64; o <<= 1) {
+            const int up = __shfl_up(incl, o);
+            if (lane >= o) incl += up;
+        }
+        if (lane == 63) wsum[wave] = incl;
+        __syncthreads();
+        int before = 0, total = 0;
+        for (int w = 0; w < 16; w++) {
+            const int s = wsum[w];
+            if (w < wave) before += s;
+            total += s;
+        }
+        int run = carry + before + incl - t;
+#pragma unroll
+        for (int u = 0; u < 4; u++) {
+            run += v[u];
+            if (i + u < n) off[1 + i + u] = run;
+        }
+        carry += total;
+        __syncthreads();
+    }
+    if (tid == 0) off[0] = 0;
+}
+
+__global__ __launch_bounds__(256) void sp_fill_rows_kernel(const float *__restrict__ X, int N, int F, const int32_t *__restrict__ row_off,
+                                                            int32_t *__restrict__ col, float *__restrict__ val) {
+    const int lane = threadIdx.x & 63;
+    const int n = blockIdx.x * 4 + (threadIdx.x >> 6);
+    if (n >= N) return;
+    const float *x = X + (int64_t)n * F;
+    int at = row_off[n];
+    const int end = row_off[n + 1];
+    for (int f0 = 0; f0 < F; f0 += 64) {
+        const int f = f0 + lane;
+        const float v = f < F ? x[f] : 0.0f;
+        const bool nz = v != 0.0f;
+        const unsigned long long m = __ballot(nz);
+        const int pos = at + __popcll(m & ((1ull << lane) - 1ull));
+        if (nz && pos < end) {
+            col[pos] = f;
+            val[pos] = v;
+        }
+        at += __popcll(m);
+    }
+}
+
+__global__ __launch_bounds__(64) void sp_fill_cols_kernel(const float *__restrict__ X, int N, int F, const int32_t *__restrict__ col_off,
+                                                           int32_t *__restrict__ row, float *__restrict__ valc) {
+    const int f = blockIdx.x * 64 + threadIdx.x;
+    if (f >= F) return;
+    const float *x = X + f;
+    int at = col_off[f];
+    const int end = col_off[f + 1];
+#pragma unroll 8
+    for (int n = 0; n < N; n++) {
+        const float v = x[(int64_t)n * F];
+        if (v != 0.0f && at < end) {
+            row[at] = n;
+            valc[at] = v;
+            at++;
+        }
+    }
+}
+
+constexpr int SP_GROUP = 8;
+template <int NJ>
+__global__ __launch_bounds__(256) void sparse_fc0_fwd_kernel(const int32_t *__restrict__ row_off, const int32_t *__restrict__ col,
+                                                              const float *__restrict__ val, const float *__restrict__ W0T,
+                                                              const float *__restrict__ bias, int N, int H, int relu,
+                                                              uint32_t *__restrict__ clear_word, float *__restrict__ Xh) {
+    if (clear_word && blockIdx.x == 0 && threadIdx.x == 0) clear_word[0] = clear_word[1] = clear_word[2] = 0u;
+    const int lane = threadIdx.x & 63;
+    const int n = blockIdx.x * 4 + (threadIdx.x >> 6);
+    if (n >= N) return;
+    const int b = __builtin_amdgcn_readfirstlane(row_off[n]), e = __builtin_amdgcn_readfirstlane(row_off[n + 1]);
+    float acc[NJ];
+#pragma unroll
+    for (int j = 0; j < NJ; j++) acc[j] = 0.0f;
+    for (int c0 = b; c0 < e; c0 += 64) {
+        const int cnt = min(64, e - c0);
+        int cl = 0;
+        float vl = 0.0f;
+        if (lane < cnt) {
+            cl = col[c0 + lane];
+            vl = val[c0 + lane];
+        }
+        for (int k = 0; k < cnt; k += SP_GROUP) {
+            float w[SP_GROUP][NJ], v[SP_GROUP];
+#pragma unroll
+            for (int u = 0; u < SP_GROUP; u++) {
+                const int kk = min(k + u, cnt - 1);
+                const float *wr = W0T + (size_t)wave_bcast(cl, kk) * H;
+                v[u] = wave_bcast(vl, kk);
+#pragma unroll
+                for (int j = 0; j < NJ; j++) w[u][j] = j * 64 + lane < H ? wr[j * 64 + lane] : 0.0f;
+            }
+#pragma unroll
+            for (int u = 0; u < SP_GROUP; u++)
+                if (k + u < cnt) {
+#pragma unroll
+                    for (int j = 0; j < NJ; j++) acc[j] = fmaf(v[u], w[u][j], acc[j]);
+                }
+        }
+    }
+#pragma unroll
+    for (int j = 0; j < NJ; j++) {
+        const int h = j * 64 + lane;
+        if (h < H) {
+            float y = acc[j] + bias[h];
+            if (relu) y = fmaxf(y, 0.0f);
+            Xh[(size_t)n * H + h] = y;
+        }
+    }
+}
+
+constexpr int SP_BIAS_ROWS = 64;
+template <int NJ>
+__device__ __forceinline__ void sparse_bias_block(float (*part)[NJ * 64], int block, const float *__restrict__ dXh,
+                                                  const float *__restrict__ gate, int N, int H, float *__restrict__ g_b) {
+    const int lane = threadIdx.x & 63, wave = threadIdx.x >> 6;
+    const int r0 = block * SP_BIAS_ROWS + wave * (SP_BIAS_ROWS / 4);
+    float d[SP_BIAS_ROWS / 4][NJ];
+#pragma unroll
+    for (int u = 0; u < SP_BIAS_ROWS / 4; u++) {
+        const size_t at = (size_t)min(r0 + u, N - 1) * H;
+#pragma unroll
+        for (int j = 0; j < NJ; j++) {
+            const int h = j * 64 + lane;
+            d[u][j] = h < H ? dXh[at + h] : 0.0f;
+            if (gate && h < H && !(gate[at + h] > 0.0f)) d[u][j] = 0.0f;
+        }
+    }
+#pragma unroll
+    for (int j = 0; j < NJ; j++) {
+        float s = 0.0f;
+#pragma unroll
+        for (int u = 0; u < SP_BIAS_ROWS / 4; u++)
+            if (r0 + u < N) s += d[u][j];
+        part[wave][j * 64 + lane] = s;
+    }
+    __syncthreads();
+    for (int h = threadIdx.x; h < H; h += 256) atomicAdd(g_b + h, ((part[0][h] + part[1][h]) + part[2][h]) + part[3][h]);
+}
+
+template <int NJ>
+__global__ __launch_bounds__(256) void sparse_fc0_wgrad_kernel(const int32_t *__restrict__ col_off, const int32_t *__restrict__ row,
+                                                                      const float *__restrict__ valc, const float *__restrict__ dXh,
+                                                                      const float *__restrict__ gate, int N, int F, int H,
+                                                                      int feature_blocks, float *__restrict__ g_w,
+                                                                      float *__restrict__ g_b) {
+    __shared__ float part[4][NJ * 64];
+    const int lane = threadIdx.x & 63, wave = threadIdx.x >> 6;
+    if ((int)blockIdx.x >= feature_blocks) {
+        sparse_bias_block<NJ>(part, (int)blockIdx.x - feature_blocks, dXh, gate, N, H, g_b);
+        return;
+    }
+    const int f = blockIdx.x;
+    const int b = __builtin_amdgcn_readfirstlane(col_off[f]), e = __builtin_amdgcn_readfirstlane(col_off[f + 1]);
+    const int mine = (e - b - wave + 3) / 4;
+    float acc[NJ];
+#pragma unroll
+    for (int j = 0; j < NJ; j++) acc[j] = 0.0f;
+    for (int i0 = 0; i0 < mine; i0 += 64) {
+        const int cnt = min(64, mine - i0);
+        int rl = 0;
+        float vl = 0.0f;
+        if (lane < cnt) {
+            const int at = b + wave + 4 * (i0 + lane);
+            rl = row[at];
+            vl = valc[at];
+        }
+        for (int k = 0; k < cnt; k += SP_GROUP) {
+            float d[SP_GROUP][NJ], v[SP_GROUP];
+#pragma unroll
+            for (int u = 0; u < SP_GROUP; u++) {
+                const int kk = min(k + u, cnt - 1);
+                const size_t at = (size_t)wave_bcast(rl, kk) * H;
+                v[u] = wave_bcast(vl, kk);
+#pragma unroll
+                for (int j = 0; j < NJ; j++) {
+                    const int h = j * 64 + lane;
+                    d[u][j] = h < H ? dXh[at + h] : 0.0f;
+                    if (gate && h < H && !(gate[at + h] > 0.0f)) d[u][j] = 0.0f;
+                }
+            }
+#pragma unroll
+            for (int u = 0; u < SP_GROUP; u++)
+                if (k + u < cnt) {
+#pragma unroll
+                    for (int j = 0; j < NJ; j++) acc[j] = fmaf(v[u], d[u][j], acc[j]);
+                }
+        }
+    }
+#pragma unroll
+    for (int j = 0; j < NJ; j++) part[wave][j * 64 + lane] = acc[j];
+    __syncthreads();
+    for (int h = threadIdx.x; h < H; h += 256) g_w[(size_t)h * F + f] = ((part[0][h] + part[1][h]) + part[2][h]) + part[3][h];
+}
+
+int check_features(const pn_sparse_features &sp, int H, const char *who) {
+    if (H < 32 || H > 256 || H % 32 != 0) PN_FAIL(PN_ERR_ARG, "%s: hidden size %d (multiples of 32 up to 256)", who, H);
+    if (sp.nnz < 0 || !sp.row_off || !sp.col_off || (sp.nnz > 0 && (!sp.col || !sp.val || !sp.row || !sp.valc)))
+        PN_FAIL(PN_ERR_ARG, "%s: incomplete sparse features", who);
+    return PN_OK;
+}
+
+int check_matrix(const float *X, int32_t N, int32_t F, const char *who) {
+    if (!X || N < 1 || F < 1) PN_FAIL(PN_ERR_ARG, "%s: bad matrix", who);
+    if ((int64_t)N * F > SPARSE_MAX_ELEMS)
+        PN_FAIL(PN_ERR_ARG, "%s: %lld elements, sparse features are prepared for at most 2^28", who, (long long)N * F);
+    return PN_OK;
+}
+
+}
+
+int launch_sparse_fc0_fwd(hipStream_t stream, const pn_sparse_features &sp, int N, int H, const float *W0T, const float *bias,
+                          int relu, uint32_t *clear_word, float *Xh) {
+    if (int rc = check_features(sp, H, "sparse fc0 forward")) return rc;
+    const dim3 grid((unsigned)((N + 3) / 4)), block(256);
+#define PN_SP_FWD(NJ)                                                                                                       \
+    hipLaunchKernelGGL(sparse_fc0_fwd_kernel<NJ>, grid, block, 0, stream, sp.row_off, sp.col, sp.val, W0T, bias, N, H, relu, \
+                       clear_word, Xh)
+    switch ((H + 63) / 64) {
+        case 1: PN_SP_FWD(1); break;
+        case 2: PN_SP_FWD(2); break;
+        case 3: PN_SP_FWD(3); break;
+        default: PN_SP_FWD(4); break;
+    }
+#undef PN_SP_FWD
+    PN_CHECK_HIP(hipGetLastError());
+    return PN_OK;
+}
+
+int launch_sparse_fc0_wgrad(hipStream_t stream, const pn_sparse_features &sp, int N, int F, int H, const float *dXh,
+                            const float *gate, float *g_w, float *g_b) {
+    if (int rc = check_features(sp, H, "sparse fc0 weight gradient")) return rc;
+    const int feature_blocks = F, bias_blocks = g_b ? (N + SP_BIAS_ROWS - 1) / SP_BIAS_ROWS : 0;
+    const dim3 grid((unsigned)(feature_blocks + bias_blocks)), block(256);
+#define PN_SP_WGRAD(NJ)                                                                                                        \
+    hipLaunchKernelGGL(sparse_fc0_wgrad_kernel<NJ>, grid, block, 0, stream, sp.col_off, sp.row, sp.valc, dXh, gate, N, F, H, \
+                       feature_blocks, g_w, g_b)
+    switch ((H + 63) / 64) {
+        case 1: PN_SP_WGRAD(1); break;
+        case 2: PN_SP_WGRAD(2); break;
+        case 3: PN_SP_WGRAD(3); break;
+        default: PN_SP_WGRAD(4); break;
+    }
+#undef PN_SP_WGRAD
+    PN_CHECK_HIP(hipGetLastError());
+    return PN_OK;
+}
+
+}
+
+using namespace pn;
+
+extern "C" {
+
+int pn_sparse_count(pn_context *ctx, const float *X, int32_t N, int32_t F, int32_t *row_off, int32_t *col_off, void *stream_) {
+    hipStream_t stream = (hipStream_t)stream_;
+    if (int rc = check_matrix(X, N, F, "pn_sparse_count")) return rc;
+    if (!row_off || !col_off) PN_FAIL(PN_ERR_ARG, "pn_sparse_count: null offsets");
+    if (int rc = context_check_device(ctx)) return rc;
+    hipLaunchKernelGGL(sp_count_rows_kernel, dim3((unsigned)((N + 3) / 4)), dim3(256), 0, stream, X, N, F, row_off);
+    hipLaunchKernelGGL(sp_count_cols_kernel, dim3((unsigned)((F + 63) / 64)), dim3(64), 0, stream, X, N, F, col_off);
+    hipLaunchKernelGGL(sp_scan_kernel, dim3(2), dim3(1024), 0, stream, row_off, N, col_off, F);
+    PN_CHECK_HIP(hipGetLastError());
+    return PN_OK;
+}
+
+int pn_sparse_fill(pn_context *ctx, const float *X, int32_t N, int32_t F, const pn_sparse_features *sp, void *stream_) {
+    hipStream_t stream = (hipStream_t)stream_;
+    if (int rc = check_matrix(X, N, F, "pn_sparse_fill")) return rc;
+    if (!sp) PN_FAIL(PN_ERR_ARG, "pn_sparse_fill: null features");
+    if (int rc = check_features(*sp, 32, "pn_sparse_fill")) return rc;
+    if (int rc = context_check_device(ctx)) return rc;
+    if (sp->nnz == 0) return PN_OK;
+    hipLaunchKernelGGL(sp_fill_rows_kernel, dim3((unsigned)((N + 3) / 4)), dim3(256), 0, stream, X, N, F, sp->row_off,
+                       sp->col, sp->val);
+    hipLaunchKernelGGL(sp_fill_cols_kernel, dim3((unsigned)((F + 63) / 64)), dim3(64), 0, stream, X, N, F, sp->col_off,
+                       sp->row, sp->valc);
+    PN_CHECK_HIP(hipGetLastError());
+    return PN_OK;
+}
+
+}
diff --git a/pathnet_amd/modules.py b/pathnet_amd/modules.py
--- a/pathnet_amd/modules.py
+++ b/pathnet_amd/modules.py
@@ -1,6 +1,7 @@
 import collections
 import ctypes
 import os
+import weakref
 
 import numpy as np
 import torch
@@ -54,12 +55,12 @@
                     "deterministic", "compact", "seq_math")
     __slots__ = SHAPE_FIELDS + ("p_seq", "p_cls", "seed", "mask_seq", "mask_cls", "step_state", "index_rows_local", "bank_w",
                                 "bank_b", "grad", "reuse_tables", "grad_scale", "path_state", "sparse_plan", "workspace",
-                                "_shape", "_ws_bytes")
+                                "features", "_shape", "_ws_bytes")
 
     def __init__(self, variant, N, F, H, C, S, W, L, S_total=0, group_begin=0, batch_groups=0, cell=None, deterministic=False,
                  compact=None, seq_math=None, *, p_seq=0.0, p_cls=0.0, seed=0, mask_seq=None, mask_cls=None, step_state=None,
                  index_rows_local=False, bank_w=None, bank_b=None, grad=True, reuse_tables=0, grad_scale=1.0,
-                 path_state=False, sparse_plan=None, workspace=None):
+                 path_state=False, sparse_plan=None, workspace=None, features=None):
         self.variant, self.N, self.F, self.H, self.C, self.S, self.W, self.L = variant, N, F, H, C, S, W, L
         self.S_total, self.group_begin, self.batch_groups, self.cell = S_total, group_begin, batch_groups, cell
         self.deterministic = bool(deterministic)
@@ -69,6 +70,7 @@
         self.step_state, self.index_rows_local, self.bank_w, self.bank_b = step_state, index_rows_local, bank_w, bank_b
         self.grad, self.reuse_tables, self.grad_scale, self.path_state = grad, reuse_tables, grad_scale, path_state
         self.sparse_plan, self.workspace = sparse_plan, workspace
+        self.features = features
         self._shape = self._ws_bytes = None
 
     def get(self, name, default=None):
@@ -105,6 +107,9 @@
         if have is not None and have.numel() >= need and have.device == dev:
             return have
         return torch.empty(max(need, 1), dtype=torch.uint8, device=dev)
+
+    def features_ref(self):
+        return ctypes.byref(self.features.c) if self.features is not None else None
 
     def args(self, ids, codes, sel, p, X=None, Xh=None):
         a = _lib.PaggArgs()
@@ -141,6 +146,45 @@
         gX = torch.empty_like(X) if X is not None else None
         a.g_X = gX.data_ptr() if gX is not None else None
         return grads, gX, buf
+
+
+SPARSE_MAX_ELEMS = 1 << 28
+SPARSE_CACHE_ENTRIES = 4
+SPARSE_DENSE_KEYS = 16
+SPARSE_SEEN_KEYS = 8
+SPARSE_MISS_LIMIT = 2
+
+
+class PreparedFeatures:
+    __slots__ = ("X", "nnz", "row_off", "col_off", "col", "val", "row", "valc", "c", "pinned")
+
+    def __init__(self, X):
+        N, F = X.shape
+        dev = X.device
+        self.X = X
+        with torch.cuda.device(dev):
+            self.row_off = torch.empty(N + 1, dtype=torch.int32, device=dev)
+            self.col_off = torch.empty(F + 1, dtype=torch.int32, device=dev)
+            _lib.check(_lib.load().pn_sparse_count(_lib.context(dev), X.data_ptr(), N, F, self.row_off.data_ptr(),
+                                                   self.col_off.data_ptr(), _lib.stream_ptr(dev)))
+            self.nnz = int(self.row_off[N].item())
+        self.col = self.val = self.row = self.valc = self.c = None
+        self.pinned = False
+
+    def density(self):
+        return self.nnz / float(self.X.shape[0] * self.X.shape[1])
+
+    def fill(self):
+        N, F = self.X.shape
+        dev = self.X.device
+        with torch.cuda.device(dev):
+            self.col, self.row = (torch.zeros(self.nnz, dtype=torch.int32, device=dev) for _ in range(2))
+            self.val, self.valc = (torch.zeros(self.nnz, dtype=torch.float32, device=dev) for _ in range(2))
+            self.c = _lib.SparseFeatures(self.nnz, self.row_off.data_ptr(), self.col.data_ptr(), self.val.data_ptr(),
+                                         self.col_off.data_ptr(), self.row.data_ptr(), self.valc.data_ptr())
+            _lib.check(_lib.load().pn_sparse_fill(_lib.context(dev), self.X.data_ptr(), N, F, ctypes.byref(self.c),
+                                                  _lib.stream_ptr(dev)))
+        return self
 
 
 def _shape(variant, N, F, H, C, S, W, L, S_total=0, group_begin=0, batch_groups=0, cell=None, deterministic=False,
@@ -229,7 +273,8 @@
                 a.out_embed, a.out_path_weight = encode_out[0].data_ptr(), encode_out[1].data_ptr()
                 a.out_path_state = encode_out[2].data_ptr() if encode_out[2] is not None else None
             if call.S > 0:
-                _lib.check(_lib.load().pn_pagg_forward(_lib.context(dev), ctypes.byref(a), _lib.stream_ptr(dev)))
+                _lib.check(_lib.load().pn_pagg_forward_sparse(_lib.context(dev), ctypes.byref(a), call.features_ref(),
+                                                              _lib.stream_ptr(dev)))
         ctx.call, ctx.ws = call, ws
         ctx.present = [t is not None for t in params]
         ctx.save_for_backward(X, ids, codes, sel, *[t for t in params if t is not None])
@@ -261,7 +306,8 @@
             a.g_out = g_out.data_ptr() if g_out is not None else None
             a.g_embed = g_embed.data_ptr() if g_embed is not None else None
             if call.S > 0:
-                _lib.check(_lib.load().pn_pagg_backward(_lib.context(dev), ctypes.byref(a), _lib.stream_ptr(dev)))
+                _lib.check(_lib.load().pn_pagg_backward_sparse(_lib.context(dev), ctypes.byref(a), call.features_ref(),
+                                                               _lib.stream_ptr(dev)))
             else:
                 for g in list(grads.values()) + [gX] * (gX is not None):
                     g.zero_()
@@ -301,8 +347,9 @@
             grads, gX, flat = call.grad_buffers(a, p, X if ctx.needs_input_grad[1] else None, flat=True)
             target = target.to(device=dev, dtype=torch.int64).contiguous()
             if call.S > 0:
-                _lib.check(_lib.load().pn_pagg_train_step(_lib.context(dev), ctypes.byref(a), target.data_ptr(),
-                                                          float(call.grad_scale), loss.data_ptr(), _lib.stream_ptr(dev)))
+                _lib.check(_lib.load().pn_pagg_train_step_sparse(_lib.context(dev), ctypes.byref(a), call.features_ref(),
+                                                                 target.data_ptr(), float(call.grad_scale), loss.data_ptr(),
+                                                                 _lib.stream_ptr(dev)))
             else:
                 flat.zero_()
                 if gX is not None:
@@ -403,6 +450,17 @@
         self._range_calls = 0
         self._range_pending = None
         self.range_spread_bits = None
+        self.sparse_features = "auto"
+        self.sparse_min_nodes = 2048
+        self.sparse_max_density = 1.0 / 64
+        self._sparse_cache = collections.OrderedDict()
+        self._sparse_dense = collections.OrderedDict()
+        self._sparse_seen = collections.OrderedDict()
+        self.sparse_scans = 0
+        self._sparse_misses = 0
+        self._sparse_scan_open = False
+        self.fc0_route = None
+        self.fc0_route_calls = {"sparse": 0, "dense": 0}
         self._mask_seq = None
         self._mask_cls = None
         self._bank_flat = (None, None)
@@ -420,6 +478,56 @@
         lins = [self.fc0] + list(self._bank_layers())
         return (X.data_ptr(), tuple(X.shape), int(X._version), int(L),
                 tuple(int(t._version) for l in lins for t in (l.weight, l.bias)))
+
+    def _features_for(self, X, Hk):
+        mode = self.sparse_features
+        if mode not in ("auto", "never", "always"):
+            raise ValueError("sparse_features: auto, never or always")
+        N, F = X.shape
+        if mode == "never" or Hk > 256 or N * F == 0 or N * F > SPARSE_MAX_ELEMS:
+            return None
+        key = (X.data_ptr(), (N, F), int(X._version), X.device)
+        cache, capturing = self._sparse_cache, torch.cuda.is_current_stream_capturing()
+        feat = cache.get(key)
+        if feat is not None:
+            cache.move_to_end(key)
+            feat.pinned = feat.pinned or capturing
+            self._sparse_misses, self._sparse_scan_open = 0, False
+            return feat
+        if mode == "auto" and key in self._sparse_dense:
+            self._sparse_misses, self._sparse_scan_open = 0, False
+            return None
+        if capturing or (mode == "auto" and N < self.sparse_min_nodes):
+            return None
+        if mode == "auto" and self._sparse_scan_open:
+            self._sparse_misses += 1
+            self._sparse_scan_open = False
+        if mode == "auto" and self._sparse_misses >= SPARSE_MISS_LIMIT:
+            seen = self._sparse_seen.pop(key, None)
+            if seen is None or seen() is not X:
+                self._sparse_seen[key] = weakref.ref(X)
+                while len(self._sparse_seen) > SPARSE_SEEN_KEYS:
+                    self._sparse_seen.popitem(last=False)
+                return None
+        if len(cache) >= SPARSE_CACHE_ENTRIES:
+            old = next((k for k, f in cache.items() if not f.pinned), None)
+            if old is None:
+                return self._remember_dense(key)
+        feat = PreparedFeatures(X)
+        self.sparse_scans += 1
+        self._sparse_scan_open = mode == "auto"
+        if mode == "auto" and feat.density() > self.sparse_max_density:
+            return self._remember_dense(key)
+        if len(cache) >= SPARSE_CACHE_ENTRIES:
+            del cache[old]
+        cache[key] = feat.fill()
+        return feat
+
+    def _remember_dense(self, key):
+        self._sparse_dense[key] = True
+        while len(self._sparse_dense) > SPARSE_DENSE_KEYS:
+            self._sparse_dense.popitem(last=False)
+        return None
 
     def _make_cell(self, default):
         kind = self.cell or default
@@ -575,6 +683,7 @@
         dev = X.device
         if dev.type != "cuda":
             raise RuntimeError("pathnet_amd aggregators run on the GPU only (X is on %s); no CPU fallback" % dev)
+        X_given = X
         X = X.contiguous().float()
         ids, codes, sel, S = _as_index_tensors(neis, layer_type, indices, num_w, walk_len, dev, n_nodes=X.shape[0])
         H, L = self.hidden_size, int(walk_len)
@@ -614,6 +723,10 @@
                         self._cell_kind, det, compact, math, p_seq=p_drop, p_cls=p_drop, seed=seed, mask_seq=ms, mask_cls=mc,
                         step_state=self.step_state, index_rows_local=batch_position is not None, bank_w=fw, bank_b=fb,
                         grad=grad, path_state=bool(_encode))
+        whole = batch_position is None and group_slice is None
+        call.features = self._features_for(X, Hk) if (X is X_given and S > 0 and whole) else None
+        self.fc0_route = "sparse" if call.features is not None else "dense"
+        self.fc0_route_calls[self.fc0_route] += 1
         call.pick_batch_groups(self.workspace_budget, dev)
         self._last_shape = (call.shape(), dev)
         if not grad:
```

Result: faster. 62.73 million paths/s, median of 6 (+1.9%).
